# vnminin/phylomap

Measured on NVIDIA B200. Metric: sampled branch-site histories/sec (4-state, 10k-tip tree), higher is better.
Workload: dtype f32

## Files before the change

phylomap_b200/csrc/pm_host.cu:

```cuda
#include <cuda_runtime.h>

#include <algorithm>
#include <chrono>
#include <cmath>
#include <cstdarg>
#include <cstdio>
#include <cstdlib>
#include <cstring>
#include <map>
#include <memory>
#include <mutex>
#include <string>
#include <type_traits>
#include <vector>

#include "../../include/phylomap_b200.h"
#include "pm_launch.cuh"
#include "pm_setup_kernels.cuh"
#include "pm_loglik.cuh"
#include "pm_exp.cuh"
#include "pm_nccl.hpp"
#include "pm_rates.hpp"
#include "pm_tree.hpp"

// ... 316 lines not shown
  p.gx = (S + 127) / 128;
  long long ny = (148LL * 16 * 6 + p.gx - 1) / p.gx;
  ny = std::max(1LL, std::min<long long>(ny, (E + 15) / 16));
  ny = std::min<long long>(ny, 65535);
  ny = std::max<long long>(ny, (E + 2047) / 2048);
  ny = std::max<long long>(ny, (E + ((1LL << 32) - 1) / S - 1) / std::max<long long>(1, ((1LL << 32) - 1) / S));
  const double G = (double)(1 << rec_shift);
  for (;;) {
    p.chunk = (int)((E + ny - 1) / ny);
    ny = (E + p.chunk - 1) / p.chunk;
    long long cap_max = 0;
    p.cap_off.assign(ny + 1, 0);
    for (long long c = 0; c < ny; c++) {
      const int b0 = (int)c * p.chunk, b1 = std::min(E, b0 + p.chunk);
      double len = 0;
      long long init_records = 0;
      for (int e = b0; e < b1; e++) {
        len += (double)elen[e];
        const long long m0 = moff[e + 1] - moff[e];
        if (exact || m0 >= 2) init_records += m0;
      }
      long long cap;
      if (no_paths) cap = 4;
      else if (path_capacity > 0) cap = (long long)path_capacity * (b1 - b0) * (long long)G;
      else if (exact) {
        const int jumps = poisson_cap(1.5 * Omega * len + 1.0, 1e-18);
        cap = std::max<long long>((long long)(b1 - b0) + jumps, init_records);
      } else {
        std::vector<double> lams;
        long long init3 = 0;
        for (int e = b0; e < b1; e++) {
          lams.push_back(1.5 * Omega * (double)elen[e]);
          const long long m0 = moff[e + 1] - moff[e];
          if (m0 >= 3) init3 += m0;
        }
        double lam_sum = 0, lam_max = 0;
        for (double l : lams) { lam_sum += l; lam_max = std::max(lam_max, l); }
        const long long simple = (long long)poisson_cap(G * lam_sum, 1e-18) + 2LL * (b1 - b0) * (long long)G;
        long long stat = simple;
        if (lam_max < 200.0) stat = std::min(stat, chernoff_records_cap(lams, 1e-18, G));
        cap = std::max<long long>(stat, init3 * (long long)G) + 4;
      }
      if (cap > (1 << 28)) { if (rec_shift) cap = 1 << 28; else fail(PM_ERR_CAPACITY, "path capacity of a branch chunk too large"); }
      cap = (cap + 3) & ~3;
      cap_max = std::max(cap_max, cap);
      p.cap_off[c + 1] = p.cap_off[c] + (int)cap;
    }
    if (exact || no_paths || cap_max <= 65535) break;
    if (rec_shift) { p.fits = false; break; }
    if (p.chunk <= 1 || ny >= 65535) fail(PM_ERR_CAPACITY, "a branch needs more than 65 535 path records per site");
    ny = std::min<long long>(std::min<long long>(2 * ny, E), 65535);
  }
  p.ny = ny;
  return p;
}

struct CladeCode {
  pm::host::CladeSchedule cs;
  std::vector<int> e16, top;
  std::vector<int> d16;
  std::vector<long long> tips;
};
CladeCode encode_clade_schedule(const pm::host::Schedule& sch, long long S, long long TS, long long rowPL, bool redraw_tips) {
  const int T = sch.T;
  CladeCode c;
  pm::host::CladeSchedule& cs = c.cs;
  const int clade_max = (T - 1 < 512) ? std::max(8, (T - 1) / 8) : std::max(8, std::min(512, (T - 1) / 64));
  pm::host::build_clade_schedule(sch, 8, clade_max, cs);
  const int n1 = cs.warp_off.back();
  c.e16.assign((size_t)PM_CLADE_ENTRY_INTS * (n1 + 17), 0);
  auto put64 = [](int* dst, long long v) { dst[0] = (int)(unsigned)(v & 0xffffffffLL); dst[1] = (int)(v >> 32); };
  for (int i = 0; i < n1; i++) {
    const int* en = &cs.entries[(size_t)8 * i];
    int* o = &c.e16[(size_t)PM_CLADE_ENTRY_INTS * i];
    const int pn = en[0], a = en[1], ea = en[2], b = en[3], eb = en[4];
    int fl = en[5] & 3;
    const int x = (en[5] & 4) ? a : (en[5] & 8) ? b : -1;
    if (a < T) fl |= 16;
    if (b < T) fl |= 32;
    put64(o + 0, (long long)(pn - T) * rowPL);
    put64(o + 2, x >= 0 ? (long long)(x - T) * rowPL : -1LL);
    put64(o + 4, (long long)ea * S * 4);
    put64(o + 6, (long long)eb * S * 4);
    put64(o + 8, a < T ? (long long)a * TS : -1LL);
    put64(o + 10, b < T ? (long long)b * TS : -1LL);
    o[12] = fl;
  }
  c.top.assign(cs.entries.begin() + (size_t)8 * n1, cs.entries.end());
  for (int& v : cs.top_off) v -= n1;
  const int n2 = cs.down_warp_off.back();
  c.d16.assign((size_t)16 * (n2 + 17), 0);
  for (int i = 0; i < n2; i++) {
    const int* en = &cs.down_seq[(size_t)4 * i];
    int* o = &c.d16[(size_t)16 * i];
    put64(o + 0, (long long)(en[0] - T) * rowPL);
    put64(o + 2, (long long)en[2] * S * 4);
    put64(o + 4, (long long)en[0] * S);
    put64(o + 6, en[3] ? -1LL : (long long)en[1] * S);
  }
  if (redraw_tips)
    for (int v = 0; v < T; v++) {
      const int e = sch.parent_edge[v];
      c.tips.push_back((long long)sch.e_parent[e] * S); c.tips.push_back((long long)e * S * 4);
    }
  return c;
}

struct SmallOrder {
  std::vector<int> down;
  std::vector<int> border;
};
template <typename Real>
SmallOrder small_draw_order(const pm::host::Schedule& sch, const pm::host::CladeSchedule& cs, const std::vector<Real>& elen) {
  const int T = sch.T, E = (int)elen.size();
  SmallOrder so;
  std::vector<uint32_t> key(2 * (size_t)T - 1, 0u);
  for (int i = 0; i < (int)cs.down_top.size() / 4; i++) key[cs.down_top[(size_t)4 * i]] = 0x80000000u | (uint32_t)i;
  for (int i = 0; i < cs.down_warp_off.back(); i++) key[cs.down_seq[(size_t)4 * i]] = (uint32_t)i;
  for (int v = 0; v < T; v++) key[v] = 0x40000000u | (uint32_t)v;
  const int nd = (int)sch.down_entries.size() / 3;
  so.down.assign((size_t)4 * std::max(nd, 1), 0);
  for (int i = 0; i < nd; i++) {
    const int* en = &sch.down_entries[(size_t)3 * i];
    so.down[(size_t)4 * i] = en[0]; so.down[(size_t)4 * i + 1] = en[1]; so.down[(size_t)4 * i + 2] = en[2]; so.down[(size_t)4 * i + 3] = (int)key[en[0]];
  }
  std::vector<int> sorted(E);
  for (int e = 0; e < E; e++) sorted[e] = e;
  std::stable_sort(sorted.begin(), sorted.end(), [&](int x, int y) { return elen[x] > elen[y]; });
  if (E <= 256) {
    so.border.assign(256, -1);
    for (int k = 0; k < E; k++) so.border[(size_t)(k % 8) * 32 + k / 8] = sorted[k];
  } else so.border = sorted;
  return so;
}

struct WorkItems {
  std::vector<long long> off;
  std::vector<int> g;
  std::vector<int> hint;
};
template <typename Real>
WorkItems build_work_items(const std::vector<Real>& elen, double Omega, long long S) {
  const int E = (int)elen.size();
  const long long Wl = (S + 31) / 32;
  WorkItems w;
  w.off.assign(E + 1, 0);
  w.g.resize(E);
  for (int e = 0; e < E; e++) {
    const double lam = Omega * (double)elen[e];
    const double h = std::max(1e-6, 1.0 - std::exp(-lam) * (1.0 + lam));
    long long g = (long long)std::ceil(96.0 / (32.0 * h));
    g = std::max(1LL, std::min<long long>(std::min<long long>(g, 32), Wl));
    w.g[e] = (int)g;
    w.off[e + 1] = w.off[e] + (Wl + g - 1) / g;
  }
  w.hint.resize((size_t)(w.off[E] >> 6) + 1);
  for (long long i = 0, e = 0; i < (long long)w.hint.size(); i++) {
    while (e + 1 < E && w.off[e + 1] <= (i << 6)) e++;
    w.hint[i] = (int)e;
  }
  return w;
}

template <typename Real>
struct TreeDev {
  pm::host::Schedule sch;
  long long S = 0, TS = 0;
  DevBuf cl_entries, cl_warp_off, cl_top_entries, cl_top_off, cd_top, cd_top_off, cd_entries, cd_warp_off, cd_tips;
  DevBuf up_entries, up_off, down_entries, down_off, e_parent, e_child, e_len, maps_off, maps_len, cap_off;
  DevBuf tipcode, node_state, meta, PL, rec_len[2], rec_st[2], dw_partial, hard_ballot, wk_off, wk_g, wk_hint, wk_item, rec_cursor, shape;
  long long wk_total = 0, dw_rows = 0;
  int hard_blocks = 0;
  int pl_slots = 0;
  int slots_per_sm = 0;
  DevBuf slot_busy;
  long long pl_sites = 0;
  int rec_shift = 0;
  bool small_ok = false;
  bool small_two = false;
  int small_chunks = 0;
  DevBuf small_down, small_part, small_cnt, small_root, small_prof, small_border;
  DevBuf tip_stage;
  int small_cap = 0;
  int small_order_n = 0;
  long long rec_groups = 0;
  DevBuf e_len_d, TP, ll_partial;
  std::vector<int> cap_off_h;
  pm::ChainParams<Real> P;
  dim3 paths_grid;
  int chunk = 0;
  long long nblocks = 0;
};

template <typename Real>
struct ChainT : pm_chain {
  Variant V;
  int n = 0, ntrees = 0, N_total = 0, iters_done = 0, W = 0, WR = 0, ncols = 0;
  pm::host::NcclApi::Comm nccl = nullptr;
  int NS = 0;
  bool exact = false;
  double* Q = nullptr;
  double* B = nullptr;
  std::vector<double> pid, prior;
  double Omega = 0;
  pm_options opt;
  cudaStream_t stream = nullptr;
  bool own_stream = false;
  std::vector<std::unique_ptr<TreeDev<Real>>> trees;
  int jcap = 0;
  DevBuf model, cnt, root_out, err_flag, rows, tab_off, tab_u, q_dev;
  double* q_h = nullptr;
  std::vector<double> own_B;
  std::vector<double> eig_L, eig_R, eig_d;
  DevBuf eig_dev;
  Real* model_h = nullptr;
  double* rows_h = nullptr;
  double* rows_h_dev = nullptr;
  unsigned* err_h = nullptr;
  std::vector<double> scale_prev, rate_prev;
  pm::host::MersenneR mt{0};
  std::unique_ptr<pm::host::ReplaySource> replay;
  size_t smem_prune = 0, smem_nodes = 0, smem_paths = 0;
  int rows_cap = 0;
  int debug_kernel = 0;
  struct Timed { cudaEvent_t a, b; int k; };
  std::vector<Timed> timed;
  DevBuf ctl, phase_ns;
  uint32_t* ctl_h = nullptr;
  cudaGraphExec_t sweep_graph = nullptr;
  void* graph_rows = nullptr;
  bool capturing = false;
  int launches_per_sweep = 0;
  Switches sw;

  ~ChainT() override {
    cudaSetDevice(opt.device);
    cudaDeviceSynchronize();
    for (auto& t : timed) { cudaEventDestroy(t.a); cudaEventDestroy(t.b); }
    if (model_h) cudaFreeHost(model_h);
    if (rows_h) cudaFreeHost(rows_h);
    if (err_h) cudaFreeHost(err_h);
    if (q_h) cudaFreeHost(q_h);
    if (ctl_h) cudaFreeHost(ctl_h);
    for (auto& t : trees) if (t && t->small_prof.p) {
      long long h[12];
      if (cudaMemcpy(h, t->small_prof.p, sizeof h, cudaMemcpyDeviceToHost) == cudaSuccess)
        fprintf(stderr, "[phylomap_b200] k_small_chain block 0 (%d + %d levels), cycles over %d sweeps: prune %lld, node draws %lld, paths %lld, row %lld; paths per warp:"
                        " %lld %lld %lld %lld %lld %lld %lld %lld\n", (int)t->sch.up_off.size() - 1, (int)t->sch.down_off.size() - 1, iters_done, h[0], h[1], h[2], h[3], h[4], h[5], h[6], h[7], h[8], h[9], h[10], h[11]);
    }
    if (sweep_graph) cudaGraphExecDestroy(sweep_graph);
    if (own_stream && stream) cudaStreamDestroy(stream);
  }

  pm::host::UniformSource& host_rng() { return replay ? static_cast<pm::host::UniformSource&>(*replay) : mt; }

  size_t model_elems() const { return (size_t)2 * n * n + 5 * n; }
  size_t model_stride() const { return (model_elems() + 3) & ~(size_t)3; }

  void stage_model(bool first) {
    std::vector<double> Bd((size_t)n * n), Bs((size_t)n * n);
    for (int i = 0; i < n; i++)
      for (int j = 0; j < n; j++) {
        const double v = B[i + (size_t)j * n];
        Bd[(size_t)i * n + j] = v;
        Bs[(size_t)i * n + j] = (V.sparse && !(v > 1e-7)) ? 0.0 : v;
      }
    std::vector<double> scale_new(n);
    for (int s = 0; s < n; s++) scale_new[s] = 1.0 / (Omega + Q[s + (size_t)s * n]);
    std::vector<double> rate_new(n);
    for (int s = 0; s < n; s++) rate_new[s] = Omega + Q[s + (size_t)s * n];
    if (first) { scale_prev = scale_new; rate_prev = rate_new; }
    Real* m = model_h;
    for (size_t i = 0; i < (size_t)n * n; i++) { m[i] = (Real)Bd[i]; m[(size_t)n * n + i] = (Real)Bs[i]; }
    Real* v = m + 2 * (size_t)n * n;
    for (int s = 0; s < n; s++) {
      v[s] = (Real)pid[s]; v[n + s] = (Real)scale_prev[s]; v[2 * n + s] = (Real)scale_new[s];
      v[3 * n + s] = (Real)rate_prev[s]; v[4 * n + s] = (Real)rate_new[s];
    }
    scale_prev = scale_new; rate_prev = rate_new;
    Real* pw = m + model_stride();
    std::vector<double> cur((size_t)n * n, 0.0), nxt((size_t)n * n);
    for (int i = 0; i < n; i++) cur[(size_t)i * n + i] = 1.0;
    for (int j = 0; j < jcap; j++) {
      for (size_t i = 0; i < (size_t)n * n; i++) pw[(size_t)j * n * n + i] = (Real)cur[i];
      if (j + 1 < jcap) {
        for (int r = 0; r < n; r++)
          for (int c = 0; c < n; c++) {
            double acc = 0;
            for (int l = 0; l < n; l++) acc = acc + Bs[(size_t)r * n + l] * cur[(size_t)l * n + c];
            nxt[(size_t)r * n + c] = acc;
          }
        cur.swap(nxt);
      }
    }
    CK(cudaMemcpyAsync(model.p, m, (model_stride() + (size_t)jcap * n * n) * sizeof(Real), cudaMemcpyHostToDevice, stream));
  }

  template <typename F>
  auto with_ns(F&& f) const {
    if (NS == 2) return f(std::integral_constant<int, 2>{});
    if (NS == 4) return f(std::integral_constant<int, 4>{});
    return f(std::integral_constant<int, 0>{});
  }
  template <typename F>
  auto with_ns_exact(F&& f) const {
    if constexpr (std::is_same_v<Real, double>)
      if (exact) return with_ns([&](auto ns) { return f(ns, std::true_type{}); });
    return with_ns([&](auto ns) { return f(ns, std::false_type{}); });
  }

  template <int NSc, bool EX>
  void launch_sweep_t(TreeDev<Real>& t, uint32_t iter, double* row) {
    if (!EX && use_small(t)) { launch_small(t, iter, 1, row); launches_per_sweep = t.S == 1 ? 1 : 2; return; }
    const uint32_t* ctl_d = capturing ? ctl.as<uint32_t>() : nullptr;
    {
      pm::ChainParams<Real> P = t.P;
      P.ctl = ctl_d;
      const int gx = (int)((t.S + 31) / 32);
      if (t.pl_slots) {
        begin_timed(4);
        pm::Sweep<Real, NSc, EX>::prune_nodes(P, gx, smem_nodes, stream, iter, 0, 3, t.slots_per_sm ? t.slot_busy.template as<int>() : nullptr,
                                              t.slots_per_sm, timing ? phase_ns.as<unsigned long long>() : nullptr);
        end_timed();
      } else {
        begin_timed(0);
        pm::Sweep<Real, NSc, EX>::prune(P, gx, smem_prune, stream);
        end_timed();
        begin_timed(1);
        pm::Sweep<Real, NSc, EX>::nodes(P, gx, smem_nodes, stream, iter);
        end_timed();
      }
    }
    begin_timed(2);
    if (!EX) CK(cudaMemsetAsync(t.rec_cursor.p, 0, t.rec_cursor.bytes, stream));
    {
      pm::ChainParams<Real> P = t.P;
      P.ctl = ctl_d;
      pm::Sweep<Real, NSc, EX>::paths(P, t.paths_grid, smem_paths, stream, iter, (iter == 0 && !capturing) ? 1 : 0, t.chunk, t.hard_blocks);
    }
    end_timed();
    begin_timed(3);
    pm::k_reduce<<<1, 256, 0, stream>>>(t.dw_partial.template as<double>(), t.dw_rows, n, cnt.as<unsigned long long>(),
                                        root_out.as<int>(), row, 0, err_flag.as<unsigned>(), W, capturing ? ctl.as<uint32_t>() : nullptr, WR);
    end_timed();
    launches_per_sweep = (t.pl_slots ? 1 : 2) + (exact ? 2 : (iter == 0 && !capturing) ? 3 : 4);
    if (!capturing) launches += launches_per_sweep;
  }
  bool use_small(const TreeDev<Real>& t) const { return t.small_ok && !timing && !sw.debug_sync && !capturing; }
  void launch_small(TreeDev<Real>& t, uint32_t iter0, int nsweeps, double* rows_d) {
    const long long S = t.S;
    pm::SmallOut o;
    o.down = reinterpret_cast<const int4*>(t.small_down.p); o.down_off = t.down_off.template as<int>();
    o.n_down_levels = (int)t.sch.down_off.size() - 1; o.n_chunks = t.small_chunks;
    o.br_order = t.small_border.template as<int>(); o.n_order = t.small_order_n;
    o.part = nullptr; o.cnt = nullptr; o.root = nullptr; o.rows = nullptr; o.row_stride = WR; o.err_slot = W;
    o.prof = nullptr;
    if (sw.small_prof) {
      if (!t.small_prof.p) { t.small_prof.alloc(12 * sizeof(long long)); CK(cudaMemsetAsync(t.small_prof.p, 0, t.small_prof.bytes, stream)); }
      o.prof = t.small_prof.template as<long long>();
    }
    auto launch = [&](uint32_t it0, int nb) {
      with_ns([&](auto ns) { pm::Sweep<Real, decltype(ns)::value, false>::small_chain(t.P, (int)S, stream, it0, nb, o, t.small_two); });
    };
    if (S == 1) {
      o.rows = rows_d;
      launch(iter0, nsweeps);
      launches += 1;
      return;
    }
    const int batch = (int)std::max<long long>(1, std::min<long long>(nsweeps, (64LL << 20) / (S * n * (long long)sizeof(double))));
    if (t.small_cap < batch) {
      t.small_part.alloc((size_t)batch * S * n * sizeof(double));
      t.small_cnt.alloc((size_t)batch * n * n * sizeof(unsigned long long));
      t.small_root.alloc((size_t)batch * sizeof(int));
      t.small_cap = batch;
      CK(cudaMemsetAsync(t.small_cnt.p, 0, t.small_cnt.bytes, stream));
      CK(cudaMemsetAsync(t.small_root.p, 0, t.small_root.bytes, stream));
    }
    o.part = t.small_part.template as<double>(); o.cnt = t.small_cnt.template as<unsigned long long>(); o.root = t.small_root.template as<int>();
    for (int b0 = 0; b0 < nsweeps; b0 += batch) {
      const int nb = std::min(batch, nsweeps - b0);
      launch(iter0 + (uint32_t)b0, nb);
      pm::k_small_reduce<<<nb, 128, 0, stream>>>(o.part, o.cnt, o.root, S, n, rows_d + (size_t)b0 * WR, WR, err_flag.as<unsigned>(), W);
      launches += 2;
    }
  }
  void launch_loglik(TreeDev<Real>& t, double* row) {
    for (int i = 0; i < n; i++) for (int j = 0; j < n; j++) q_h[(size_t)i * n + j] = Q[i + (size_t)j * n];
    CK(cudaMemcpyAsync(q_dev.p, q_h, (size_t)n * n * sizeof(double), cudaMemcpyHostToDevice, stream));
    const int E = t.sch.E;
    pm::k_transprob<Real><<<(E + 127) / 128, 128, 0, stream>>>(q_dev.as<double>(), t.e_len_d.template as<double>(), E, n,
                                                              t.TP.template as<Real>());
    const int gx = (int)((t.S + 31) / 32);
    with_ns([&](auto ns) {
      pm::k_loglik<Real, decltype(ns)::value><<<gx, 256, 0, stream>>>(t.P, t.TP.template as<Real>(), t.ll_partial.template as<double>());
    });
    pm::k_reduce_ll<<<1, 256, 0, stream>>>(t.ll_partial.template as<double>(), gx, row + n + n * n + 1);
    launches += 3;
  }

  template <int NSc, bool EX>
  void launch_prune_t(TreeDev<Real>& t, long long only_site) {
    const long long nb = (t.S + 31) / 32;
    if (t.pl_slots) {
      if (only_site >= 0) pm::Sweep<Real, NSc, EX>::prune_nodes(t.P, 1, smem_nodes, stream, 0u, only_site / 32, 1, nullptr, 0, nullptr);
      else pm::Sweep<Real, NSc, EX>::prune_nodes(t.P, (int)nb, smem_nodes, stream, 0u, 0, 1, t.slots_per_sm ? t.slot_busy.template as<int>() : nullptr,
                                                 t.slots_per_sm, nullptr);
    } else pm::Sweep<Real, NSc, EX>::prune(t.P, (int)nb, smem_prune, stream);
    launches++;
  }

  void launch_sweep(TreeDev<Real>& t, uint32_t iter, double* row) {
    with_ns_exact([&](auto ns, auto ex) { launch_sweep_t<decltype(ns)::value, decltype(ex)::value>(t, iter, row); });
  }
  void launch_prune(TreeDev<Real>& t, long long only_site = -1) {
    with_ns_exact([&](auto ns, auto ex) { launch_prune_t<decltype(ns)::value, decltype(ex)::value>(t, only_site); });
  }

  void begin_timed(int k) {
    debug_kernel = k;
    if (!timing) return;
    Timed t; t.k = k;
    CK(cudaEventCreate(&t.a)); CK(cudaEventCreate(&t.b));
    CK(cudaEventRecord(t.a, stream));
    timed.push_back(t);
  }
  void end_timed() {
    if (timing) CK(cudaEventRecord(timed.back().b, stream));
    if (sw.debug_sync) {
      try { check_device_errors(); }
      catch (Fail& f) { f.msg += " [raised by sweep kernel #" + std::to_string(debug_kernel) + ": 0 prune, 1 nodes, 2 paths, 3 reduce]"; throw; }
    }
  }
  void collect_timed() {
    double fused = 0;
    for (auto& t : timed) {
      float ms = 0;
      cudaEventElapsedTime(&ms, t.a, t.b);
      if (t.k == 4) fused += ms; else kernel_ms[t.k] += ms;
      cudaEventDestroy(t.a); cudaEventDestroy(t.b);
    }
    timed.clear();
    if (fused > 0) {
      unsigned long long ns[2] = {0, 0};
      cudaMemcpy(ns, phase_ns.p, sizeof ns, cudaMemcpyDeviceToHost);
      cudaMemset(phase_ns.p, 0, sizeof ns);
      const double tot = (double)ns[0] + (double)ns[1];
      const double share = tot > 0 ? (double)ns[0] / tot : 0.5;
      kernel_ms[0] += fused * share;
      kernel_ms[1] += fused * (1.0 - share);
    }
  }

  void check_device_errors() {
    CK(cudaMemcpyAsync(err_h, err_flag.p, sizeof(unsigned), cudaMemcpyDeviceToHost, stream));
    CK(cudaStreamSynchronize(stream));
    const unsigned f = *err_h;
    if (!f) return;
    if (f & PM_DE_BAD_STATE) fail(PM_ERR_ARG, "tip states must lie in 1..n");
    if (f & PM_DE_SAMPLE_NA) fail(PM_ERR_SAMPLE, "NAs not allowed in probability");
    if (f & PM_DE_SAMPLE_NEG) fail(PM_ERR_SAMPLE, "Negative probabilities not allowed");
    if (f & PM_DE_SAMPLE_ZERO)
      fail(PM_ERR_SAMPLE, opt.precision == PM_F32 ? "Not enough positive probabilities (FP32 partial likelihoods span ~1e-45: on large trees with "
                                                      "one-piece branches this can be an underflow; precision f64 has the reference's range)"
                                                    : "Not enough positive probabilities");
    if (f & PM_DE_REPLAY) fail(PM_ERR_REPLAY, "replay table exhausted");
    if (f & PM_DE_JUMP_LIMIT)
      fail(PM_ERR_CAPACITY, "a branch carries more than 63 state changes at one site: the deterministic mode holds at most 64 runs "
                            "per path (the production arithmetic has no such limit)");
    if (f & PM_DE_PATH_CAP) fail(PM_ERR_CAPACITY, "the run records of a branch chunk overflowed; raise pm_options.path_capacity");
    if (f & PM_DE_M_OVERFLOW) fail(PM_ERR_CAPACITY, "more than 65535 pieces on one branch");
    fail(PM_ERR_CUDA, "inconsistent chain state (device flag %u)", f);
  }

  void create(int variant, const pm_tree* tr, int ntr, int n_, double* Q_, const double* pid_, double* B_, double Om,
              const double* prior_, int nprior, int Ntot, const pm_options* o) {
    V = variant_of(variant);
    n = n_; ntrees = ntr; N_total = Ntot; Q = Q_; B = B_; Omega = Om;
    opt = *o;
    sw = read_switches();
    PhaseTrace trace{sw.trace};
    std::vector<pm::host::Schedule> schedules = validate(variant, tr, pid_, prior_, nprior);
    trace.mark("validation + schedules");
    const int sms = open_device();
    trace.mark("device queries + stream");
    err_flag.alloc(sizeof(unsigned));
    CK(cudaMemsetAsync(err_flag.p, 0, err_flag.bytes, stream));
    cudaStream_t aux = nullptr;
    cudaEvent_t ev_a = nullptr, ev_b = nullptr;
    struct AuxGuard {
      cudaStream_t& s; cudaEvent_t& a; cudaEvent_t& b;
      ~AuxGuard() { if (s) { cudaStreamSynchronize(s); cudaStreamDestroy(s); } if (a) cudaEventDestroy(a); if (b) cudaEventDestroy(b); }
    } aux_guard{aux, ev_a, ev_b};
    CK(cudaStreamCreateWithFlags(&aux, cudaStreamNonBlocking));
    CK(cudaEventCreateWithFlags(&ev_a, cudaEventDisableTiming));
    CK(cudaEventCreateWithFlags(&ev_b, cudaEventDisableTiming));
    CK(cudaEventRecord(ev_a, stream));
    CK(cudaStreamWaitEvent(aux, ev_a, 0));
    double tmax = 0;
    for (int ti = 0; ti < ntr; ti++) trees.push_back(create_tree(tr[ti], ti, std::move(schedules[ti]), sms, aux, tmax, trace));

    alloc_model_and_host_buffers(tmax);
    if (opt.rng == PM_RNG_TABLE) upload_replay_table();
    mt.reseed((uint32_t)opt.seed);
    trace.mark("pinned buffers, replay table");
    const int np_fast = exact ? 0 : ((NS == 2 || NS == 4) ? std::min(PM_SMEM_POW, jcap) : 0);
    smem_prune = ((size_t)n * n + (size_t)np_fast * n * n) * sizeof(Real);
    smem_nodes = ((size_t)n * n + 3 * n + (size_t)np_fast * n * n) * sizeof(Real);
    smem_paths = (size_t)4 * n * sizeof(double) + ((size_t)n * n + ((n * n) & 1)) * sizeof(unsigned) +
                 ((size_t)2 * n * n + 5 * n + (size_t)np_fast * n * n) * sizeof(Real);

    for (int ti = 0; ti < ntr; ti++) {
      TreeDev<Real>& t = *trees[ti];
      fill_params(t, ti);
      const pm::ChainParams<Real>& P = t.P;
      if (!V.exp && !V.llonly)
        pm::k_init_meta<Real><<<dim3((unsigned)((t.S + 255) / 256), (unsigned)std::min(P.E, 65535)), 256, 0, stream>>>(P.maps_off, P.maps_len, t.S, P.E, P.meta,
                                                                                                                         P.e_len, exact ? nullptr : P.shape);
      trace.mark("set-up kernels issued");
      CK(cudaGetLastError());
    }
    CK(cudaEventRecord(ev_b, aux));
    CK(cudaStreamWaitEvent(stream, ev_b, 0));
    stage_model(true);
    if (V.exp) {
      std::vector<double> eg;
      eg.insert(eg.end(), eig_L.begin(), eig_L.end());
      eg.insert(eg.end(), eig_R.begin(), eig_R.end());
      eg.insert(eg.end(), eig_d.begin(), eig_d.end());
      upload(eig_dev, eg, stream);
      TreeDev<Real>& t = *trees[0];
      const int E = t.sch.E;
      const double* g = eig_dev.as<double>();
      pm::k_transprob_eig<Real><<<(E + 127) / 128, 128, 0, stream>>>(g, g + (size_t)n * n, g + (size_t)2 * n * n,
                                                                    t.e_len_d.template as<double>(), E, n, t.TP.template as<Real>());
      CK(cudaGetLastError());
    }
    check_device_errors();
    for (auto& t : trees) t->tip_stage.alloc(0);
    trace.mark("tip states: H2D + transpose, init kernels, sync");
  }

  std::vector<pm::host::Schedule> validate(int variant, const pm_tree* tr, const double* pid_, const double* prior_, int nprior) {
    const int ntr = ntrees;
    if (n < 2 || n > PM_NMAX) fail(PM_ERR_ARG, "number of states must be in 2..%d", PM_NMAX);
    if (!V.multi && ntr != 1) fail(PM_ERR_ARG, "this sampler takes exactly one tree");
    if (ntr < 1) fail(PM_ERR_ARG, "no trees");
    if (N_total < 0) fail(PM_ERR_ARG, "N must be non-negative");
    if (V.hidden && (n < 4 || (n & 1))) fail(PM_ERR_ARG, "hidden-rate samplers need an even number of states >= 4");
    if (V.two_state && n != 2) fail(PM_ERR_ARG, "this sampler is 2-state only");
    if (V.dic && n > PM_DIC_NMAX) fail(PM_ERR_ARG, "the DIC samplers support at most %d states", PM_DIC_NMAX);
    const int need_prior = V.two_state ? 4 : variant == PM_V_KSMT ? 8 : V.hidden ? 6 : 0;
    if (nprior < need_prior || (need_prior && !prior_)) fail(PM_ERR_ARG, "prior needs %d values", need_prior);
    if (need_prior) prior.assign(prior_, prior_ + nprior);
    pid.assign(pid_, pid_ + n);
    exact = opt.mode == PM_MODE_DETERMINISTIC;
    if (exact && opt.precision != PM_F64) fail(PM_ERR_ARG, "deterministic mode computes in FP64");
    if (exact && V.exp) fail(PM_ERR_ARG, "the direct sampler (maketreelistEXP) runs in production arithmetic only");
    if (opt.rng == PM_RNG_TABLE && (!opt.tab_off || !opt.tab_u)) fail(PM_ERR_ARG, "replay table missing");
    if (opt.rng == PM_RNG_TABLE && !exact) fail(PM_ERR_ARG, "the replay table feeds the deterministic mode only");
    if (opt.rng == PM_RNG_TABLE && (opt.site_offset != 0 || opt.allreduce || opt.nccl_world > 1)) fail(PM_ERR_ARG, "replay runs are single-process");
    if (opt.allreduce && !opt.cuda_stream)
      fail(PM_ERR_ARG, "an allreduce callback needs pm_options.cuda_stream: the collective must be ordered on the stream the chain launches on");
    if (opt.allreduce && opt.nccl_world > 1) fail(PM_ERR_ARG, "give either an allreduce callback or an NCCL clique, not both");
    if (opt.nccl_world > 1 && (!opt.nccl_id || opt.nccl_rank < 0 || opt.nccl_rank >= opt.nccl_world)) fail(PM_ERR_ARG, "bad NCCL clique (nccl_id / nccl_rank / nccl_world)");
    NS = (n == 2) ? 2 : (n == 4) ? 4 : 0;
    W = n + n * n + 1 + (V.dic ? 1 : 0);
    WR = W + 1;
    ncols = ncols_of(variant, n);

    if (!(Omega > 0)) fail(PM_ERR_ARG, "Omega must be positive");
    std::vector<pm::host::Schedule> schedules(ntr);
    for (int ti = 0; ti < ntr; ti++) {
      const pm_tree& x = tr[ti];
      if (x.n_tips != tr[0].n_tips || x.n_edges != tr[0].n_edges) fail(PM_ERR_ARG, "all trees must have the same number of tips");
      if (x.n_sites < 1 || x.n_sites != tr[0].n_sites) fail(PM_ERR_ARG, "n_sites must be >= 1 and equal across trees");
      if (x.n_sites >= (1LL << 31)) fail(PM_ERR_ARG, "at most 2^31 - 1 sites per process");
      if (!x.edge || !x.nen || !x.nodelist || !x.maps_off || !x.maps_len) fail(PM_ERR_ARG, "tree %d: missing field", ti);
      if (!x.states && !x.states_u8) fail(PM_ERR_ARG, "tree %d: states missing", ti);
      try {
        pm::host::build_schedule(x.n_tips, x.n_edges, x.edge, x.nen, x.nodelist, x.root, V.redraw_tips, schedules[ti]);
      } catch (const std::string& msg) { fail(PM_ERR_ARG, "tree %d: %s", ti, msg.c_str()); }
      if (x.maps_off[0] != 0) fail(PM_ERR_ARG, "tree %d: maps_off[0] must be 0", ti);
      for (int e = 0; e < x.n_edges; e++) {
        const long long a = x.maps_off[e], b = x.maps_off[e + 1];
        if (b <= a) fail(PM_ERR_ARG, "tree %d: branch %d has no segments", ti, e + 1);
        if (b - a > 65535) fail(PM_ERR_ARG, "tree %d: branch %d has more than 65535 segments", ti, e + 1);
        for (long long p = a; p < b; p++) {
          if (!(x.maps_len[p] >= 0)) fail(PM_ERR_ARG, "tree %d: negative or NA segment length", ti);
          if (x.maps_state && (x.maps_state[p] < 1 || x.maps_state[p] > n)) fail(PM_ERR_ARG, "tree %d: mapnames out of range", ti);
        }
      }
    }
    return schedules;
  }

  int open_device() {
    int ndev = 0;
    if (cudaGetDeviceCount(&ndev) != cudaSuccess || ndev <= 0) fail(PM_ERR_CUDA, "no CUDA device (there is no CPU fallback)");
    if (opt.device < 0 || opt.device >= ndev) fail(PM_ERR_CUDA, "device %d not present", opt.device);
    CK(cudaSetDevice(opt.device));
    int major = 0, minor = 0, sms = 0;
    CK(cudaDeviceGetAttribute(&major, cudaDevAttrComputeCapabilityMajor, opt.device));
    CK(cudaDeviceGetAttribute(&minor, cudaDevAttrComputeCapabilityMinor, opt.device));
    CK(cudaDeviceGetAttribute(&sms, cudaDevAttrMultiProcessorCount, opt.device));
    if (major != 10) fail(PM_ERR_CUDA, "device %d is sm_%d%d; this library is built for sm_100a only", opt.device, major, minor);
    if (opt.cuda_stream) stream = (cudaStream_t)opt.cuda_stream;
    else { CK(cudaStreamCreateWithFlags(&stream, cudaStreamNonBlocking)); own_stream = true; }
    return sms;
  }

  std::unique_ptr<TreeDev<Real>> create_tree(const pm_tree& x, int ti, pm::host::Schedule&& sch, int sms, cudaStream_t aux,
                                             double& tmax, PhaseTrace& trace) {
    std::unique_ptr<TreeDev<Real>> tp(new TreeDev<Real>());
    TreeDev<Real>& t = *tp;
    t.sch = std::move(sch);
    t.S = x.n_sites;
    t.TS = (t.S + 15) / 16 * 16;
    const int E = x.n_edges, T = x.n_tips;
    const long long S = t.S;
    const bool no_paths = V.exp || V.llonly;
    upload_tips(t, x, aux);
    std::vector<long long> moff(x.maps_off, x.maps_off + E + 1);
    std::vector<Real> elen(E);
    for (int e = 0; e < E; e++) {
      double tot = 0;
      for (long long p = moff[e]; p < moff[e + 1]; p++) tot = tot + x.maps_len[p];
      elen[e] = (Real)tot;
      tmax = std::max(tmax, tot);
    }
    std::vector<double> mlen(x.maps_len, x.maps_len + moff[E]);

    const size_t small_smem = with_ns([&](auto ns) { return pm::Sweep<Real, decltype(ns)::value, false>::small_smem(T); });
    const SmallChoice small = choose_small_kernel(!exact && (NS == 2 || NS == 4) && !no_paths && opt.rng != PM_RNG_TABLE, elen,
                                                  Omega, T, S, sms, small_smem, sw);
    t.small_ok = small.ok;
    t.small_two = small.two;
    const bool pooled_ok = !t.small_ok && !exact && !no_paths && sw.rec_pool;
    RecordPlan rp = plan_records(pooled_ok ? 5 : 0, elen, moff, S, Omega, exact, no_paths, opt.path_capacity);
    if (!rp.fits) rp = plan_records(0, elen, moff, S, Omega, exact, no_paths, opt.path_capacity);
    t.rec_shift = rp.rec_shift;
    t.rec_groups = (S + (1LL << t.rec_shift) - 1) >> t.rec_shift;
    t.chunk = rp.chunk;
    t.paths_grid = dim3((unsigned)rp.gx, (unsigned)rp.ny, 1);
    t.nblocks = rp.gx * rp.ny;
    t.small_chunks = (int)rp.ny;
    t.cap_off_h = std::move(rp.cap_off);
    trace.mark("record capacities");

    plan_partials_slots(t, sms);
    upload(t.up_entries, t.sch.up_entries, stream);
    upload(t.up_off, t.sch.up_off, stream);
    if (!exact && (NS == 2 || NS == 4)) {
      CladeCode cc = encode_clade_schedule(t.sch, S, t.TS, (long long)t.pl_sites * n * (long long)sizeof(Real), V.redraw_tips);
      upload(t.cl_entries, cc.e16, stream);
      upload(t.cl_warp_off, cc.cs.warp_off, stream);
      upload(t.cl_top_entries, cc.top, stream);
      upload(t.cl_top_off, cc.cs.top_off, stream);
      upload(t.cd_entries, cc.d16, stream);
      upload(t.cd_warp_off, cc.cs.down_warp_off, stream);
      upload(t.cd_top, cc.cs.down_top, stream);
      upload(t.cd_top_off, cc.cs.down_top_off, stream);
      upload(t.cd_tips, cc.tips, stream);
      t.P.n_cl_top_levels = (int)cc.cs.top_off.size() - 1;
      t.P.n_cd_top_levels = (int)cc.cs.down_top_off.size() - 1;
      t.P.n_cd_tips = (int)cc.tips.size() / 2;
      if (t.small_ok) {
        const SmallOrder so = small_draw_order(t.sch, cc.cs, elen);
        upload(t.small_down, so.down, stream);
        upload(t.small_border, so.border, stream);
        t.small_order_n = (int)so.border.size();
      }
    }
    upload(t.down_entries, t.sch.down_entries, stream);
    upload(t.down_off, t.sch.down_off, stream);
    upload(t.e_parent, t.sch.e_parent, stream);
    upload(t.e_child, t.sch.e_child, stream);
    upload(t.e_len, elen, stream);
    if (V.dic || V.exp) {
      std::vector<double> eld(E);
      for (int e = 0; e < E; e++) eld[e] = x.edge_length ? x.edge_length[e] : (double)elen[e];
      if (x.edge_length) for (int e = 0; e < E; e++) if (!(eld[e] >= 0)) fail(PM_ERR_ARG, "tree %d: negative or NA edge.length", ti);
      upload(t.e_len_d, eld, stream);
      t.TP.alloc((size_t)E * n * n * sizeof(Real));
      t.ll_partial.alloc((size_t)((S + 31) / 32) * sizeof(double));
    }
    trace.mark("clade schedules + uploads");
    alloc_path_state(t, moff, mlen, elen, sms);
    trace.mark("device buffers");
    return tp;
  }

  void upload_tips(TreeDev<Real>& t, const pm_tree& x, cudaStream_t aux) {
    const int T = x.n_tips;
    t.tipcode.alloc((size_t)T * t.TS);
    CK(cudaMemsetAsync(t.tipcode.p, 0, t.tipcode.bytes, aux));
    t.node_state.alloc((size_t)(2 * T - 1) * t.S);
    CK(cudaMemsetAsync(t.node_state.p, 0, t.node_state.bytes, aux));
    const size_t esz = x.states_u8 ? 1 : 4;
    long long rows_per = std::max<long long>(32, (256LL << 20) / ((long long)T * (long long)esz));
    rows_per = std::min<long long>(rows_per, std::min<long long>(t.S, 32LL * 65535));
    t.tip_stage.alloc((size_t)rows_per * T * esz);
    for (long long s0 = 0; s0 < t.S; s0 += rows_per) {
      const int ns = (int)std::min<long long>(rows_per, t.S - s0);
      const void* src = x.states_u8 ? (const void*)(x.states_u8 + s0 * T) : (const void*)(x.states + s0 * T);
      CK(cudaMemcpyAsync(t.tip_stage.p, src, (size_t)ns * T * esz, cudaMemcpyHostToDevice, aux));
      dim3 g((T + 31) / 32, (ns + 31) / 32), b(32, 8);
      if (x.states_u8)
        pm::k_init_tips<uint8_t><<<g, b, 0, aux>>>(t.tip_stage.template as<uint8_t>(), ns, s0, t.S, t.TS, T, n, V.parity_tips,
                                                     t.tipcode.template as<uint8_t>(), t.node_state.template as<uint8_t>(), err_flag.as<unsigned>());
      else
        pm::k_init_tips<int32_t><<<g, b, 0, aux>>>(t.tip_stage.template as<int32_t>(), ns, s0, t.S, t.TS, T, n, V.parity_tips,
                                                     t.tipcode.template as<uint8_t>(), t.node_state.template as<uint8_t>(), err_flag.as<unsigned>());
    }
    CK(cudaGetLastError());
  }

  void plan_partials_slots(TreeDev<Real>& t, int sms) {
    t.pl_slots = 0;
    t.pl_sites = t.S;
    if (exact || !(NS == 2 || NS == 4) || V.dic || V.exp || V.llonly || !sw.fused) return;
    const size_t smem_lo = ((size_t)n * n + 3 * n) * sizeof(Real);
    const int per_sm = with_ns([&](auto ns) { return pm::Sweep<Real, decltype(ns)::value, false>::fused_blocks_per_sm(smem_lo); });
    if (per_sm < 1) fail(PM_ERR_CUDA, "cudaOccupancyMaxActiveBlocksPerMultiprocessor failed for the fused prune + node-draw kernel");
    t.slots_per_sm = per_sm;
    t.pl_slots = sm_id_range(opt.device, sms) * per_sm;
    t.pl_sites = 32LL * t.pl_slots;
    if (t.pl_sites >= ((t.S + 31) / 32) * 32) {
      t.pl_slots = (int)((t.S + 31) / 32); t.pl_sites = 32LL * t.pl_slots; t.slots_per_sm = 0;
    } else {
      t.slot_busy.alloc((size_t)t.pl_slots * sizeof(int));
      CK(cudaMemsetAsync(t.slot_busy.p, 0, t.slot_busy.bytes, stream));
    }
  }

  void alloc_path_state(TreeDev<Real>& t, const std::vector<long long>& moff, const std::vector<double>& mlen,
                        const std::vector<Real>& elen, int sms) {
    const int E = t.sch.E, T = t.sch.T;
    const long long S = t.S, R = t.cap_off_h.back();
    const bool no_paths = V.exp || V.llonly;
    upload(t.maps_off, moff, stream);
    upload(t.maps_len, mlen, stream);
    upload(t.cap_off, t.cap_off_h, stream);
    if (!no_paths) t.meta.alloc((size_t)E * S * sizeof(uint32_t));
    t.PL.alloc((size_t)(T - 1) * t.pl_sites * n * sizeof(Real));
    for (int b = 0; b < 2 && !no_paths; b++) {
      t.rec_len[b].alloc((size_t)R * t.rec_groups * sizeof(Real));
      t.rec_st[b].alloc((size_t)R * t.rec_groups);
    }
    if (!exact && !no_paths) {
      const long long Wl = (S + 31) / 32;
      t.hard_ballot.alloc((size_t)E * Wl * sizeof(uint32_t));
      const WorkItems w = build_work_items(elen, Omega, S);
      t.wk_total = w.off.back();
      upload(t.wk_hint, w.hint, stream);
      upload(t.wk_off, w.off, stream);
      upload(t.wk_g, w.g, stream);
      t.wk_item.alloc((size_t)std::max<long long>(t.wk_total, 1) * sizeof(unsigned long long));
      pm::k_build_items<<<(unsigned)((t.wk_total + 255) / 256), 256, 0, stream>>>(t.wk_off.template as<long long>(), t.wk_g.template as<int>(), E, Wl,
                                                                                 t.wk_total, t.wk_item.template as<unsigned long long>());
      t.rec_cursor.alloc((size_t)t.small_chunks * t.rec_groups * sizeof(int));
      t.shape.alloc((size_t)E * S * sizeof(uint16_t));
      t.hard_blocks = (int)std::max<long long>(1, std::min<long long>(sms * 4LL, (t.wk_total + 3) / 4));
    }
    t.dw_rows = t.nblocks + 3 * t.hard_blocks;
    t.dw_partial.alloc((size_t)t.dw_rows * n * sizeof(double));
    CK(cudaMemsetAsync(t.dw_partial.p, 0, t.dw_partial.bytes, stream));
    dev_bytes += t.tipcode.bytes + t.node_state.bytes + t.meta.bytes + t.PL.bytes + 2 * (t.rec_len[0].bytes + t.rec_st[0].bytes) +
                 t.dw_partial.bytes + t.hard_ballot.bytes + t.rec_cursor.bytes + t.shape.bytes + t.wk_item.bytes;
  }

  void alloc_model_and_host_buffers(double tmax) {
    jcap = opt.power_capacity > 0 ? opt.power_capacity : 64;
    if (V.exp) jcap = 302;
    else if (opt.power_capacity <= 0) {
      const double lam = Omega * tmax;
      const double want = lam + 10 * std::sqrt(lam) + 24;
      jcap = (int)std::min(16384.0, std::max(64.0, want));
    }
    if (jcap < 2) jcap = 2;
    model.alloc((model_stride() + (size_t)jcap * n * n) * sizeof(Real));
    CK(cudaMallocHost((void**)&model_h, (model_stride() + (size_t)jcap * n * n) * sizeof(Real)));
    memset(model_h, 0, (model_stride() + (size_t)jcap * n * n) * sizeof(Real));
    CK(cudaMallocHost((void**)&rows_h, (size_t)ntrees * WR * sizeof(double)));
    if (cudaHostGetDevicePointer((void**)&rows_h_dev, rows_h, 0) != cudaSuccess) { rows_h_dev = nullptr; (void)cudaGetLastError(); }
    if (opt.nccl_world > 1) nccl = clique(opt.nccl_id, opt.nccl_world, opt.nccl_rank);
    CK(cudaMallocHost((void**)&err_h, sizeof(unsigned)));
    CK(cudaMallocHost((void**)&ctl_h, 2 * sizeof(uint32_t)));
    ctl.alloc(2 * sizeof(uint32_t));
    phase_ns.alloc(2 * sizeof(unsigned long long));
    CK(cudaMemsetAsync(phase_ns.p, 0, phase_ns.bytes, stream));
    if (V.dic) { CK(cudaMallocHost((void**)&q_h, (size_t)n * n * sizeof(double))); q_dev.alloc((size_t)n * n * sizeof(double)); }
    cnt.alloc((size_t)n * n * sizeof(unsigned long long));
    root_out.alloc(sizeof(int));
    CK(cudaMemsetAsync(cnt.p, 0, cnt.bytes, stream));
    CK(cudaMemsetAsync(root_out.p, 0, root_out.bytes, stream));
  }

  int replay_slots_per_iter() const { return (2 * trees[0]->sch.T - 1) + 2 * trees[0]->sch.E; }
  void upload_replay_table() {
    const long long nslots = (long long)ntrees * trees[0]->S * N_total * replay_slots_per_iter();
    std::vector<long long> off(nslots + 1);
    for (long long i = 0; i <= nslots; i++) off[i] = opt.tab_off[i];
    std::vector<double> u(opt.tab_u, opt.tab_u + off[nslots]);
    upload(tab_off, off, stream);
    upload(tab_u, u, stream);
    if (opt.host_tab) replay.reset(new pm::host::ReplaySource(opt.host_tab, opt.host_tab_n));
  }

  void fill_params(TreeDev<Real>& t, int ti) {
    pm::ChainParams<Real>& P = t.P;
    const int T = t.sch.T, E = t.sch.E, spi = replay_slots_per_iter();
    P.n = n; P.T = T; P.E = E; P.S = t.S;
    P.cap_off = t.cap_off.template as<int>();
    P.hard_ballot = t.hard_ballot.template as<uint32_t>(); P.W = (int)((t.S + 31) / 32);
    P.wk_off = t.wk_off.template as<long long>(); P.wk_g = t.wk_g.template as<int>(); P.wk_total = t.wk_total;
    P.wk_hint = t.wk_hint.template as<int>(); P.wk_item = t.wk_item.template as<unsigned long long>();
    P.rec_cursor = t.rec_cursor.template as<int>(); P.chunk = t.chunk; P.easy_blocks = t.nblocks;
    P.shape = t.shape.template as<uint16_t>();
    P.model = model.as<Real>(); P.ppow = model.as<Real>() + model_stride(); P.jcap = jcap;
    P.up_entries = t.up_entries.template as<int>(); P.up_off = t.up_off.template as<int>();
    P.n_up_levels = (int)t.sch.up_off.size() - 1;
    P.cl_entries = t.cl_entries.template as<int>(); P.cl_warp_off = t.cl_warp_off.template as<int>();
    P.cl_top_entries = t.cl_top_entries.template as<int>(); P.cl_top_off = t.cl_top_off.template as<int>();
    P.cd_top = t.cd_top.template as<int>(); P.cd_top_off = t.cd_top_off.template as<int>();
    P.cd_entries = t.cd_entries.template as<int>(); P.cd_warp_off = t.cd_warp_off.template as<int>();
    P.cd_tips = t.cd_tips.template as<long long>();
    P.down_entries = t.down_entries.template as<int>(); P.down_off = t.down_off.template as<int>();
    P.n_down_levels = (int)t.sch.down_off.size() - 1;
    P.e_parent = t.e_parent.template as<int>(); P.e_child = t.e_child.template as<int>();
    P.e_len = t.e_len.template as<Real>();
    P.maps_off = t.maps_off.template as<long long>(); P.maps_len = t.maps_len.template as<double>();
    P.root = t.sch.root;
    P.tipcode = t.tipcode.template as<uint8_t>(); P.TS = t.TS; P.node_state = t.node_state.template as<uint8_t>();
    P.meta = t.meta.template as<uint32_t>(); P.PL = t.PL.template as<Real>();
    P.tile_base = 0; P.pl_S = t.pl_sites; P.rec_shift = t.rec_shift; P.rec_groups = t.rec_groups; P.ctl = nullptr;
    for (int b = 0; b < 2; b++) { P.rec_len[b] = t.rec_len[b].template as<Real>(); P.rec_st[b] = t.rec_st[b].template as<uint8_t>(); }
    P.normalize = V.normalize || !exact; P.full_counts = V.full_counts; P.parity_tips = V.parity_tips;
    P.dw_partial = t.dw_partial.template as<double>(); P.cnt = cnt.as<unsigned long long>();
    P.root_out = root_out.as<int>(); P.err_flag = err_flag.as<unsigned>();
    const uint64_t key = opt.seed + (uint64_t)ti * 0x9E3779B97F4A7C15ull;
    P.rng.k0 = (uint32_t)key; P.rng.k1 = (uint32_t)(key >> 32);
    for (int r = 0; r < 10; r++) { P.rng.rk[2 * r] = P.rng.k0 + (uint32_t)r * 0x9E3779B9u; P.rng.rk[2 * r + 1] = P.rng.k1 + (uint32_t)r * 0xBB67AE85u; }
    P.rng.site0 = (uint32_t)opt.site_offset;
    P.rng.tab_off = opt.rng == PM_RNG_TABLE ? (const int64_t*)tab_off.p : nullptr;
    P.rng.tab_u = opt.rng == PM_RNG_TABLE ? tab_u.as<double>() : nullptr;
    P.rng.tab_site_stride = (int64_t)N_total * spi;
    P.rng.tab_base = (int64_t)ti * t.S * N_total * spi;
    P.rng.slots_per_iter = spi; P.rng.n_nodes = 2 * T - 1;
  }

  void reduce_over_ranks(double* buf, int count) {
    if (nccl) {
      auto& api = pm::host::NcclApi::get();
      const int rc = api.AllReduce(buf, buf, (size_t)count, pm::host::NcclApi::kDouble, pm::host::NcclApi::kSum, nccl, stream);
      if (rc != 0) fail(PM_ERR_CUDA, "ncclAllReduce failed: %s", api.error(rc).c_str());
    } else if (opt.allreduce) {
      if (opt.allreduce(opt.allreduce_ctx, buf, count) != 0) fail(PM_ERR_CUDA, "allreduce callback failed");
    }
  }
  void check_row_errors(const double* rows_host, int nrows) {
    bool any = false;
    for (int i = 0; i < nrows; i++) any = any || rows_host[(size_t)i * WR + W] != 0.0;
    if (!any) return;
    check_device_errors();
    fail(PM_ERR_CUDA, "another rank reported a device error in this sweep; all ranks stop together");
  }

  void ensure_rows(int count) {
    const int need = std::max(count, 1) * ntrees;
    if (need <= rows_cap) return;
    rows.alloc((size_t)need * WR * sizeof(double));
    rows_cap = need;
  }

  void write_fixed_row(const double* r, double* out, int64_t ld, int i) {
    for (int s = 0; s < n; s++) out[i + (int64_t)s * ld] = r[s];
    for (int a = 0; a < n; a++)
      for (int b = 0; b < n; b++) {
        if (a == b) continue;
        const int col = n + a * (n - 1) + b - (a < b ? 1 : 0);
        out[i + (int64_t)col * ld] = r[n + a * n + b];
      }
  }

  void launch_exp_iteration(TreeDev<Real>& t, uint32_t iter, double* row) {
    const int gx = (int)((t.S + 31) / 32);
    Real* TP = t.TP.template as<Real>();
    double* llp = t.ll_partial.template as<double>();
    const size_t smem_b = (size_t)4 * n * sizeof(double) + ((size_t)n * n + ((n * n) & 1)) * sizeof(unsigned) + (size_t)n * n * sizeof(Real);
    const double* el = t.e_len_d.template as<double>();
    with_ns([&](auto ns) {
      constexpr int NSc = decltype(ns)::value;
      begin_timed(0);
      pm::k_loglik<Real, NSc><<<gx, 256, 0, stream>>>(t.P, TP, llp);
      end_timed();
      begin_timed(1);
      pm::k_exp_nodes<Real, NSc><<<gx, 256, 0, stream>>>(t.P, TP, iter);
      end_timed();
      begin_timed(2);
      pm::k_exp_branches<Real, NSc><<<t.paths_grid, 128, smem_b, stream>>>(t.P, TP, el, (Real)Omega, iter, t.chunk);
      end_timed();
    });
    begin_timed(3);
    pm::k_reduce<<<1, 256, 0, stream>>>(t.dw_partial.template as<double>(), t.dw_rows, n, cnt.as<unsigned long long>(),
                                        root_out.as<int>(), row, 0, err_flag.as<unsigned>(), W);
    end_timed();
    launches += 4;
  }

  void run(int count, double* out, int64_t ld) override {
    if (count < 0 || iters_done + count > N_total) fail(PM_ERR_ARG, "cannot run %d more iterations (%d of %d done)", count, iters_done, N_total);
    if (count == 0) return;
    if (ld < count) fail(PM_ERR_ARG, "leading dimension smaller than the number of rows");
    CK(cudaSetDevice(opt.device));
    if (!V.rates) {
      ensure_rows(count);
      TreeDev<Real>& t = *trees[0];
      const bool small = (double)t.S * t.sch.E <= (double)(1 << 22);
      const bool one_launch = !V.exp && !exact && use_small(t);
      const bool use_graph = !one_launch && !V.exp && !timing && !sw.debug_sync && count > 1 && (sw.graph == 1 || (sw.graph != 0 && small));
      if (one_launch) launch_small(t, (uint32_t)iters_done, count, rows.as<double>());
      for (int i = 0; i < count && !one_launch; i++) {
        if (V.exp) launch_exp_iteration(t, (uint32_t)(iters_done + i), rows.as<double>() + (size_t)i * WR);
        else if (use_graph && i > 0) {
          if (i == 1) {
            if (sweep_graph && graph_rows != rows.p) { cudaGraphExecDestroy(sweep_graph); sweep_graph = nullptr; }
            if (!sweep_graph) {
              cudaGraph_t g = nullptr;
              CK(cudaStreamBeginCapture(stream, cudaStreamCaptureModeRelaxed));
              capturing = true;
              try { launch_sweep(t, 1u, rows.as<double>()); } catch (...) { capturing = false; cudaStreamEndCapture(stream, &g); if (g) cudaGraphDestroy(g); throw; }
              capturing = false;
              CK(cudaStreamEndCapture(stream, &g));
              const cudaError_t ge = cudaGraphInstantiate(&sweep_graph, g, 0);
              cudaGraphDestroy(g);
              if (ge != cudaSuccess) fail(PM_ERR_CUDA, "cudaGraphInstantiate failed: %s", cudaGetErrorString(ge));
              graph_rows = rows.p;
            }
            ctl_h[0] = (uint32_t)(iters_done + 1); ctl_h[1] = 1u;
            CK(cudaMemcpyAsync(ctl.p, ctl_h, 2 * sizeof(uint32_t), cudaMemcpyHostToDevice, stream));
          }
          CK(cudaGraphLaunch(sweep_graph, stream));
          launches += launches_per_sweep;
        }
        else launch_sweep(t, (uint32_t)(iters_done + i), rows.as<double>() + (size_t)i * WR);
        if (opt.progress) { printf("%i \r", iters_done + i); }
      }
      CK(cudaGetLastError());
      reduce_over_ranks(rows.as<double>(), count * WR);
      std::vector<double> h((size_t)count * WR);
      CK(cudaMemcpyAsync(h.data(), rows.p, h.size() * sizeof(double), cudaMemcpyDeviceToHost, stream));
      CK(cudaStreamSynchronize(stream));
      check_row_errors(h.data(), count);
      collect_timed();
      for (int i = 0; i < count; i++) write_fixed_row(&h[(size_t)i * WR], out, ld, i);
      iters_done += count;
      return;
    }

    ensure_rows(1);
    pm::host::RateModel rm{n, Q, B, Omega, prior.data()};
    const size_t nparam = V.hidden ? (size_t)2 + 3 * (n / 2 - 1) : 2;
    if (rate_proposed.size() != nparam) { rate_proposed.assign(nparam, 0); rate_accepted.assign(nparam, 0); }
    rm.proposed = rate_proposed.data(); rm.accepted = rate_accepted.data();
    pm::host::UniformSource& g = host_rng();
    std::vector<double> row(ncols);
    std::vector<std::vector<double>> jodt(ntrees, std::vector<double>(ncols, 0.0));
    for (int i = 0; i < count; i++) {
      const int it = iters_done;
      if (V.multi && it == 0) (void)g.next();
      bool host_rows = rows_h_dev != nullptr && !nccl && !opt.allreduce && !V.dic;
      for (int j = 0; j < ntrees; j++) host_rows = host_rows && use_small(*trees[j]);
      double* const row0 = host_rows ? rows_h_dev : rows.as<double>();
      for (int j = 0; j < ntrees; j++) launch_sweep(*trees[j], (uint32_t)it, row0 + (size_t)j * WR);
      if (V.dic) launch_loglik(*trees[0], rows.as<double>());
      CK(cudaGetLastError());
      cudaEvent_t ca = nullptr, cb = nullptr;
      if (timing) { CK(cudaEventCreate(&ca)); CK(cudaEventCreate(&cb)); CK(cudaEventRecord(ca, stream)); }
      reduce_over_ranks(rows.as<double>(), ntrees * WR);
      if (timing) CK(cudaEventRecord(cb, stream));
      if (!host_rows) CK(cudaMemcpyAsync(rows_h, rows.p, (size_t)ntrees * WR * sizeof(double), cudaMemcpyDeviceToHost, stream));
      CK(cudaStreamSynchronize(stream));
      if (timing) { float ms = 0; cudaEventElapsedTime(&ms, ca, cb); comm_ms += ms; cudaEventDestroy(ca); cudaEventDestroy(cb); }
      const auto host_t0 = std::chrono::steady_clock::now();
      check_row_errors(rows_h, ntrees);
      for (int j = 0; j < ntrees; j++) {
        std::fill(jodt[j].begin(), jodt[j].end(), 0.0);
        const double* r = rows_h + (size_t)j * WR;
        for (int c = 0; c < n + n * n; c++) jodt[j][c] = r[c];
        if (V.hidden) rm.record_hidden(jodt[j].data()); else rm.record_two_state(jodt[j].data());
        if (V.dic) { jodt[j][ncols - 2] = r[n + n * n]; jodt[j][ncols - 1] = r[n + n * n + 1]; }
        else jodt[j][ncols - 1] = r[n + n * n];
      }
      int pick = 0;
      if (V.multi) {
        const double u = g.next();
        double cum = 0;
        for (pick = 0; pick < ntrees; pick++) { cum += 1.0 / ntrees; if (u < cum) break; }
        if (pick >= ntrees) pick = ntrees - 1;
        jodt[pick][ncols - 1] = pick;
      }
      const double* st = jodt[pick].data();
      for (int c = 0; c < ncols; c++) out[i + (int64_t)c * ld] = st[c];
      if (V.hidden) rm.hidden_rates(st, g, V.multi); else rm.two_state(st, g, V.multi);
      if (g.exhausted()) fail(PM_ERR_REPLAY, "host replay table exhausted");
      iters_done++;
      stage_model(false);
      if (timing) host_update_ms += std::chrono::duration<double, std::milli>(std::chrono::steady_clock::now() - host_t0).count();
      if (opt.progress) { printf("%i \r", it); }
    }
    CK(cudaStreamSynchronize(stream));
    collect_timed();
  }

  float time_prune(int tree, int reps) override {
    if (tree < 0 || tree >= ntrees || reps < 1) fail(PM_ERR_ARG, "bad arguments");
    CK(cudaSetDevice(opt.device));
    cudaEvent_t a, b;
    CK(cudaEventCreate(&a)); CK(cudaEventCreate(&b));
    launch_prune(*trees[tree]);
    CK(cudaEventRecord(a, stream));
    for (int r = 0; r < reps; r++) launch_prune(*trees[tree]);
    CK(cudaEventRecord(b, stream));
    CK(cudaEventSynchronize(b));
    float ms = 0;
    CK(cudaEventElapsedTime(&ms, a, b));
    cudaEventDestroy(a); cudaEventDestroy(b);
    CK(cudaGetLastError());
    return ms / reps;
  }

  void node_states(int tree, int32_t* out) override {
    TreeDev<Real>& t = *trees.at(tree);
    const int NN = 2 * t.sch.T - 1;
    std::vector<uint8_t> h((size_t)NN * t.S);
    CK(cudaMemcpy(h.data(), t.node_state.p, h.size(), cudaMemcpyDeviceToHost));
    for (long long s = 0; s < t.S; s++) for (int v = 0; v < NN; v++) out[s * NN + v] = h[(size_t)v * t.S + s];
  }
  void piece_counts(int tree, int32_t* out) override {
    TreeDev<Real>& t = *trees.at(tree);
    const int E = t.sch.E;
    std::vector<uint32_t> h((size_t)E * t.S);
    CK(cudaMemcpy(h.data(), t.meta.p, h.size() * 4, cudaMemcpyDeviceToHost));
    for (long long s = 0; s < t.S; s++) for (int e = 0; e < E; e++) out[s * E + e] = (int)(h[(size_t)e * t.S + s] & 0xffffu);
  }
  int path(int tree, int64_t site, int e, double* len, int32_t* st, int cap) override {
    TreeDev<Real>& t = *trees.at(tree);
    if (site < 0 || site >= t.S || e < 0 || e >= t.sch.E) fail(PM_ERR_ARG, "bad site / branch");
    uint32_t m = 0;
    CK(cudaMemcpy(&m, t.meta.template as<uint32_t>() + (size_t)e * t.S + site, 4, cudaMemcpyDeviceToHost));
    if (iters_done == 0) fail(PM_ERR_ARG, "no sweep done yet");
    const int c = e / t.chunk, b0 = c * t.chunk;
    const int cap_c = t.cap_off_h[c + 1] - t.cap_off_h[c];
    const int buf = (iters_done - 1) & 1;
    auto records = [&](long long pos, int count) {
      const size_t base = (size_t)t.cap_off_h[c] * t.rec_groups + (size_t)(site >> t.rec_shift) * cap_c + pos;
      for (int k = 0; k < count && k < cap; k++) {
        Real L; uint8_t s;
        CK(cudaMemcpy(&L, t.rec_len[buf].template as<Real>() + base + k, sizeof(Real), cudaMemcpyDeviceToHost));
        CK(cudaMemcpy(&s, t.rec_st[buf].template as<uint8_t>() + base + k, 1, cudaMemcpyDeviceToHost));
        len[k] = (double)L; st[k] = s;
      }
    };
    if (exact) {
      const int nj = (m >> 16) & 0xff;
      long long pos = 0;
      for (int e2 = b0; e2 < e; e2++) {
        uint32_t m2 = 0;
        CK(cudaMemcpy(&m2, t.meta.template as<uint32_t>() + (size_t)e2 * t.S + site, 4, cudaMemcpyDeviceToHost));
        pos += ((m2 >> 16) & 0xff) + 1;
      }
      records(pos, nj + 1);
      return nj + 1;
    }
    uint16_t shp = 0;
    CK(cudaMemcpy(&shp, t.shape.template as<uint16_t>() + (size_t)e * t.S + site, 2, cudaMemcpyDeviceToHost));
    int nj = shp & 0x3f;
    const int s0 = (shp >> 6) & 0x1f, s1 = (shp >> 11) & 0x1f;
    const uint32_t q = m >> 16;
    Real Le;
    CK(cudaMemcpy(&Le, t.e_len.template as<Real>() + e, sizeof(Real), cudaMemcpyDeviceToHost));
    if (nj == 0) {
      if (cap > 0) { len[0] = (double)Le; st[0] = s0; }
      return 1;
    }
    if (nj == 1) {
      const Real p1 = (Real)q * (Le * (Real)(1.0 / 65536.0));
      if (cap > 0) { len[0] = (double)p1; st[0] = s0; }
      if (cap > 1) { len[1] = (double)(Le - p1); st[1] = s1; }
      return 2;
    }
    long long pos = (long long)q;
    if (nj == 63) {
      Real cntv;
      CK(cudaMemcpy(&cntv, t.rec_len[buf].template as<Real>() + (size_t)t.cap_off_h[c] * t.rec_groups + (size_t)(site >> t.rec_shift) * cap_c + pos, sizeof(Real),
                    cudaMemcpyDeviceToHost));
      nj = (int)cntv - 1;
      pos += 1;
    }
    records(pos, nj + 1);
    return nj + 1;
  }
  static constexpr uint32_t PM_STATE_FORMAT = 6;
  struct StateHeader {
    char magic[8];
    int32_t variant, n, ntrees, precision, mode, T, E, iters_done, jcap, reserved;
    int64_t S, site_offset, total_bytes;
    uint64_t seed;
  };
  std::vector<DevBuf*> state_buffers() {
    std::vector<DevBuf*> v{&model};
    for (auto& t : trees) {
      v.push_back(&t->node_state); v.push_back(&t->meta); v.push_back(&t->shape);
      for (int b = 0; b < 2; b++) { v.push_back(&t->rec_len[b]); v.push_back(&t->rec_st[b]); }
    }
    return v;
  }
  size_t host_state_bytes() const { return sizeof(StateHeader) + 625 * sizeof(uint32_t) + ((size_t)2 * n * n + 2 * n) * sizeof(double); }
  int64_t state_bytes() override {
    size_t tot = host_state_bytes();
    for (DevBuf* b : state_buffers()) tot += (b->bytes + 15) & ~(size_t)15;
    return (int64_t)tot;
  }
  StateHeader make_header() {
    StateHeader h;
    memset(&h, 0, sizeof h);
    memcpy(h.magic, "PMB200S", 8);
    h.variant = V.id; h.n = n; h.ntrees = ntrees; h.precision = opt.precision; h.mode = opt.mode;
    h.T = trees[0]->sch.T; h.E = trees[0]->sch.E; h.iters_done = iters_done; h.jcap = jcap;
    h.S = trees[0]->S; h.site_offset = opt.site_offset; h.total_bytes = state_bytes(); h.seed = opt.seed;
    uint32_t hsh = 2166136261u;
    auto mix = [&](uint32_t v) { hsh = (hsh ^ v) * 16777619u; };
    mix(PM_STATE_FORMAT); mix(PM_META(1, 2)); mix((uint32_t)PM_SHAPE(1, 2, 3)); mix(PM_LAMBDA_INV); mix(PM_LOCAL_PATH_MAX); mix(PM_SMEM_POW);
    for (auto& t : trees) { mix((uint32_t)t->chunk); mix((uint32_t)t->rec_shift); for (int c : t->cap_off_h) mix((uint32_t)c); }
    h.reserved = (int32_t)((PM_STATE_FORMAT << 24) | (hsh & 0xffffffu));
    return h;
  }
  void export_state(void* buf, int64_t bytes) override {
    if (opt.rng == PM_RNG_TABLE) fail(PM_ERR_ARG, "replay-table runs cannot be checkpointed");
    if (!buf || bytes < state_bytes()) fail(PM_ERR_ARG, "state buffer too small (%lld bytes needed)", (long long)state_bytes());
    CK(cudaSetDevice(opt.device));
    CK(cudaStreamSynchronize(stream));
    unsigned char* p = (unsigned char*)buf;
    const StateHeader h = make_header();
    memcpy(p, &h, sizeof h); p += sizeof h;
    uint32_t w[625]; mt.save(w);
    memcpy(p, w, sizeof w); p += sizeof w;
    memcpy(p, Q, (size_t)n * n * sizeof(double)); p += (size_t)n * n * sizeof(double);
    memcpy(p, B, (size_t)n * n * sizeof(double)); p += (size_t)n * n * sizeof(double);
    memcpy(p, scale_prev.data(), n * sizeof(double)); p += n * sizeof(double);
    memcpy(p, rate_prev.data(), n * sizeof(double)); p += n * sizeof(double);
    for (DevBuf* b : state_buffers()) {
      if (b->bytes) CK(cudaMemcpyAsync(p, b->p, b->bytes, cudaMemcpyDeviceToHost, stream));
      p += (b->bytes + 15) & ~(size_t)15;
    }
    CK(cudaStreamSynchronize(stream));
  }
  void import_state(const void* buf, int64_t bytes) override {
    if (opt.rng == PM_RNG_TABLE) fail(PM_ERR_ARG, "replay-table runs cannot be checkpointed");
    if (!buf || bytes < (int64_t)sizeof(StateHeader)) fail(PM_ERR_ARG, "not a chain state");
    const unsigned char* p = (const unsigned char*)buf;
    StateHeader h; memcpy(&h, p, sizeof h); p += sizeof h;
    const StateHeader me = make_header();
    if (memcmp(h.magic, me.magic, 8) != 0) fail(PM_ERR_ARG, "not a chain state");
    if (h.variant != me.variant || h.n != me.n || h.ntrees != me.ntrees || h.precision != me.precision || h.mode != me.mode ||
        h.T != me.T || h.E != me.E || h.S != me.S || h.site_offset != me.site_offset || h.jcap != me.jcap || h.seed != me.seed ||
        h.total_bytes != me.total_bytes)
      fail(PM_ERR_ARG, "the state was exported by a chain of a different shape, sampler, precision, seed or site block");
    if (h.reserved != me.reserved)
      fail(PM_ERR_ARG, "the state was exported under another state format or buffer layout (format %d here, %d in the blob)",
           (int)PM_STATE_FORMAT, (int)((uint32_t)h.reserved >> 24));
    if (bytes < h.total_bytes) fail(PM_ERR_ARG, "truncated chain state");
    if (h.iters_done < 0 || h.iters_done > N_total) fail(PM_ERR_ARG, "the state has %d iterations done, this chain was created for %d", h.iters_done, N_total);
    CK(cudaSetDevice(opt.device));
    CK(cudaStreamSynchronize(stream));
    uint32_t w[625]; memcpy(w, p, sizeof w); p += sizeof w;
    if (w[624] > 624u) fail(PM_ERR_ARG, "corrupt chain state");
    mt.load(w);
    memcpy(Q, p, (size_t)n * n * sizeof(double)); p += (size_t)n * n * sizeof(double);
    memcpy(B, p, (size_t)n * n * sizeof(double)); p += (size_t)n * n * sizeof(double);
    memcpy(scale_prev.data(), p, n * sizeof(double)); p += n * sizeof(double);
    memcpy(rate_prev.data(), p, n * sizeof(double)); p += n * sizeof(double);
    for (DevBuf* b : state_buffers()) {
      if (b->bytes) CK(cudaMemcpyAsync(b->p, p, b->bytes, cudaMemcpyHostToDevice, stream));
      p += (b->bytes + 15) & ~(size_t)15;
    }
    CK(cudaStreamSynchronize(stream));
    iters_done = h.iters_done;
  }

  double loglik() override {
    if (!V.dic) fail(PM_ERR_ARG, "this chain was not created with a log-likelihood column");
    CK(cudaSetDevice(opt.device));
    ensure_rows(1);
    double* row = rows.as<double>();
    launch_loglik(*trees[0], row);
    CK(cudaGetLastError());
    double* cell = row + n + n * n + 1;
    reduce_over_ranks(cell, 1);
    CK(cudaMemcpyAsync(rows_h, cell, sizeof(double), cudaMemcpyDeviceToHost, stream));
    check_device_errors();
    return rows_h[0];
  }
  void partials(int tree, int64_t site, double* out) override {
    TreeDev<Real>& t = *trees.at(tree);
    const int T = t.sch.T;
    if (site < 0 || site >= t.S) fail(PM_ERR_ARG, "bad site");
    CK(cudaSetDevice(opt.device));
    launch_prune(t, site);
    CK(cudaStreamSynchronize(stream));
    const long long col = t.pl_slots ? site % 32 : site;
    std::fill(out, out + (size_t)(2 * T - 1) * n, 0.0);
    std::vector<Real> v(n);
    for (int i = 0; i < T - 1; i++) {
      CK(cudaMemcpy(v.data(), t.PL.template as<Real>() + ((size_t)i * t.pl_sites + col) * n, n * sizeof(Real), cudaMemcpyDeviceToHost));
      for (int j = 0; j < n; j++) out[(size_t)(T + i) * n + j] = (double)v[j];
    }
  }
};

struct EigenIn { const double* lefts; const double* rights; const double* d; };

template <typename Real>
void prepare_exp(ChainT<Real>& c, int n, const double* Q, const EigenIn& eg, double*& B, double& Omega) {
  double mn = Q[0];
  for (int i = 1; i < n; i++) mn = std::min(mn, Q[i + (size_t)i * n]);
  Omega = -mn;
  c.own_B.assign((size_t)n * n, 0.0);
  for (int i = 0; i < n; i++) for (int j = 0; j < n; j++) c.own_B[i + (size_t)j * n] = (i == j ? 1.0 : 0.0) + Q[i + (size_t)j * n] / Omega;
  B = c.own_B.data();
  c.eig_L.resize((size_t)n * n); c.eig_R.resize((size_t)n * n); c.eig_d.resize(n);
  for (int i = 0; i < n; i++) {
    c.eig_d[i] = eg.d[i + (size_t)i * n];
    for (int j = 0; j < n; j++) { c.eig_L[(size_t)i * n + j] = eg.lefts[i + (size_t)j * n]; c.eig_R[(size_t)i * n + j] = eg.rights[i + (size_t)j * n]; }
  }
}

pm_chain* make_chain(int variant, const pm_tree* trees, int ntrees, int n, double* Q, const double* pid, double* B,
                     double Omega, const double* prior, int nprior, int N_total, const pm_options* opt,
                     const EigenIn* eg = nullptr, bool internal = false) {
  pm_options def;
  if (!opt) { pm_default_options(&def); opt = &def; }
  if (!trees || !Q || !pid || (!B && variant != PM_V_EXP)) fail(PM_ERR_ARG, "null argument");
  if (variant == PM_V_EXP && (!eg || !eg->lefts || !eg->rights || !eg->d)) fail(PM_ERR_ARG, "the direct sampler needs the eigendecomposition of Q");
  if (variant == PM_V_EXP && (n < 2 || n > PM_NMAX)) fail(PM_ERR_ARG, "number of states must be in 2..%d", PM_NMAX);
  if ((variant < PM_V_PLAIN || variant > PM_V_EXP) && !internal) fail(PM_ERR_ARG, "unknown variant");
  if (opt->precision == PM_F32) {
    std::unique_ptr<ChainT<float>> c(new ChainT<float>());
    if (variant == PM_V_EXP) prepare_exp(*c, n, Q, *eg, B, Omega);
    c->create(variant, trees, ntrees, n, Q, pid, B, Omega, prior, nprior, N_total, opt);
    return c.release();
  }
  std::unique_ptr<ChainT<double>> c(new ChainT<double>());
  if (variant == PM_V_EXP) prepare_exp(*c, n, Q, *eg, B, Omega);
  c->create(variant, trees, ntrees, n, Q, pid, B, Omega, prior, nprior, N_total, opt);
  return c.release();
}

void run_site_block(int variant, const pm_tree* x, int n, double* Q, const double* pid, double* B, double Omega, int N,
                    const pm_options* opt, const EigenIn* eg, long long s0, long long count, double* out) {
  pm_tree t = *x;
  t.n_sites = count;
  if (x->states_u8) t.states_u8 = x->states_u8 + s0 * (long long)x->n_tips;
  if (x->states) t.states = x->states + s0 * (long long)x->n_tips;
  pm_options o = *opt;
  o.site_offset = opt->site_offset + s0;
  std::unique_ptr<pm_chain> c(make_chain(variant, &t, 1, n, Q, pid, B, Omega, nullptr, 0, N, &o, eg));
  c->run(N, out, N);
}

int one_call(int variant, const pm_tree* trees, int ntrees, int n, double* Q, const double* pid, double* B, double Omega,
             int N, const double* prior, int nprior, const pm_options* opt, double* out, char* err, size_t errlen,
             const EigenIn* eg = nullptr) {
  return guarded(err, errlen, [&] {
    if (!out && N > 0) fail(PM_ERR_ARG, "null output");
    pm_options def;
    if (!opt) { pm_default_options(&def); opt = &def; }
    const bool fixed_q = variant == PM_V_PLAIN || variant == PM_V_SPARSE || variant == PM_V_BIGTREE || variant == PM_V_EXP;
    const bool single_process = !opt->allreduce && opt->nccl_world <= 1;
    long long tile = read_switches().site_tile;
    if (!fixed_q || !trees || ntrees != 1 || opt->rng == PM_RNG_TABLE || trees[0].n_sites < 2) tile = 0;
    const long long S = trees ? trees[0].n_sites : 0;
    for (;;) {
      const long long ts = (tile > 0 && tile < S) ? tile : S;
      try {
        if (ts >= S) {
          std::unique_ptr<pm_chain> c(make_chain(variant, trees, ntrees, n, Q, pid, B, Omega, prior, nprior, N, opt, eg));
          c->run(N, out, N);
        } else {
          const int nc = ncols_of(variant, n);
          std::vector<double> part((size_t)N * nc), acc((size_t)N * nc, 0.0);
          for (long long s0 = 0; s0 < S; s0 += ts) {
            run_site_block(variant, trees, n, Q, pid, B, Omega, N, opt, eg, s0, std::min(ts, S - s0), part.data());
            for (size_t i = 0; i < acc.size(); i++) acc[i] += part[i];
          }
          std::copy(acc.begin(), acc.end(), out);
        }
        return;
      } catch (const Fail& f) {
        const bool oom = f.code == PM_ERR_CUDA && f.msg.find("cudaMalloc") != std::string::npos;
        if (!oom || !fixed_q || !single_process || ts < 64 || ntrees != 1 || opt->rng == PM_RNG_TABLE) throw;
        cudaGetLastError();
        pool().release();
        tile = (ts + 1) / 2;
      }
    }
  });
}

}

extern "C" {

void pm_default_options(pm_options* o) {
  memset(o, 0, sizeof *o);
  o->precision = PM_F64;
  o->mode = PM_MODE_PRODUCTION;
  o->rng = PM_RNG_PHILOX;
  o->seed = 1;
}

int32_t pm_ncols(int32_t variant, int32_t n) { return ncols_of(variant, n); }

int pm_maketreelistMCMC(const pm_tree* x, int32_t n, double* Q, const double* pid, double* B, double Omega, int32_t N,
                        const pm_options* opt, double* out, char* err, size_t errlen) {
  return one_call(PM_V_PLAIN, x, 1, n, Q, pid, B, Omega, N, nullptr, 0, opt, out, err, errlen);
}
int pm_SPARSEmaketreelistMCMC(const pm_tree* x, int32_t n, double* Q, const double* pid, double* B, double Omega,
                              int32_t N, const pm_options* opt, double* out, char* err, size_t errlen) {
  return one_call(PM_V_SPARSE, x, 1, n, Q, pid, B, Omega, N, nullptr, 0, opt, out, err, errlen);
}
int pm_maketreelistMCMC_bigtree(const pm_tree* x, int32_t n, double* Q, const double* pid, double* B, double Omega,
                                int32_t N, const pm_options* opt, double* out, char* err, size_t errlen) {
  return one_call(PM_V_BIGTREE, x, 1, n, Q, pid, B, Omega, N, nullptr, 0, opt, out, err, errlen);
}
int pm_maketreelistMCMCbf(const pm_tree* x, int32_t n, double* Q, const double* pid, double* B, double Omega, int32_t N,
                          const double* prior, int32_t nprior, const pm_options* opt, double* out, char* err,
                          size_t errlen) {
  return one_call(PM_V_BF, x, 1, n, Q, pid, B, Omega, N, prior, nprior, opt, out, err, errlen);
}
int pm_maketreelistMCMCks(const pm_tree* x, int32_t n, double* Q, const double* pid, double* B, double Omega, int32_t N,
                          const double* prior, int32_t nprior, const pm_options* opt, double* out, char* err,
                          size_t errlen) {
  return one_call(PM_V_KS, x, 1, n, Q, pid, B, Omega, N, prior, nprior, opt, out, err, errlen);
}
int pm_maketreelistMCMCmt(const pm_tree* trees, int32_t ntrees, int32_t n, double* Q, const double* pid, double* B,
                          double Omega, int32_t N, const double* prior, int32_t nprior, const pm_options* opt,
                          double* out, char* err, size_t errlen) {
  return one_call(PM_V_MT, trees, ntrees, n, Q, pid, B, Omega, N, prior, nprior, opt, out, err, errlen);
}
int pm_maketreelistMCMCksmt(const pm_tree* trees, int32_t ntrees, int32_t n, double* Q, const double* pid, double* B,
                            double Omega, int32_t N, const double* prior, int32_t nprior, const pm_options* opt,
                            double* out, char* err, size_t errlen) {
  return one_call(PM_V_KSMT, trees, ntrees, n, Q, pid, B, Omega, N, prior, nprior, opt, out, err, errlen);
}

int pm_maketreelistEXP(const pm_tree* x, int32_t n, double* Q, const double* pid, int32_t N, const double* lefts,
                       const double* rights, const double* d, const pm_options* opt, double* out, char* err, size_t errlen) {
  EigenIn eg{lefts, rights, d};
  return one_call(PM_V_EXP, x, 1, n, Q, pid, nullptr, 0.0, N, nullptr, 0, opt, out, err, errlen, &eg);
}

int pm_maketreelistMCMC2sDICt(const pm_tree* x, int32_t n, double* Q, const double* pid, double* B, double Omega, int32_t N,
                              const double* prior, int32_t nprior, const pm_options* opt, double* out, char* err,
                              size_t errlen) {
  return one_call(PM_V_DIC2S, x, 1, n, Q, pid, B, Omega, N, prior, nprior, opt, out, err, errlen);
}
int pm_maketreelistMCMCksDICt(const pm_tree* x, int32_t n, double* Q, const double* pid, double* B, double Omega, int32_t N,
                              const double* prior, int32_t nprior, const pm_options* opt, double* out, char* err,
                              size_t errlen) {
  return one_call(PM_V_DICKS, x, 1, n, Q, pid, B, Omega, N, prior, nprior, opt, out, err, errlen);
}

int pm_loglik(const pm_tree* x, int32_t n, const double* Q, const double* pid, int32_t parity_tips, const pm_options* opt,
              double* out, char* err, size_t errlen) {
  return guarded(err, errlen, [&] {
    if (!x || !Q || !pid || !out) fail(PM_ERR_ARG, "null argument");
    if (n < 2 || n > PM_DIC_NMAX) fail(PM_ERR_ARG, "number of states must be in 2..%d", PM_DIC_NMAX);
    if (parity_tips && (n & 1)) fail(PM_ERR_ARG, "parity tip partials need an even number of states");
    std::vector<double> q(Q, Q + (size_t)n * n), b((size_t)n * n, 0.0);
    double om = 0;
    for (int i = 0; i < n; i++) om = std::max(om, 2 * std::fabs(q[i + (size_t)i * n]));
    if (!(om > 0)) om = 1;
    for (int i = 0; i < n; i++) for (int j = 0; j < n; j++) b[i + (size_t)j * n] = (i == j ? 1.0 : 0.0) + q[i + (size_t)j * n] / om;
    std::unique_ptr<pm_chain> c(make_chain(parity_tips ? V_LOGLIK_PARITY : V_LOGLIK, x, 1, n, q.data(), pid, b.data(), om, nullptr, 0, 0,
                                           opt, nullptr, true));
    *out = c->loglik();
  });
}

int pm_debug_clade_schedule(const int32_t* edge, int32_t n_edges, int32_t n_tips, const int32_t* nen, const int32_t* nodelist,
                            int32_t root, int32_t nwarps, int32_t clade_max, int64_t* stats, char* err, size_t errlen) {
  return guarded(err, errlen, [&] {
    if (!edge || !nen || !nodelist || !stats || nwarps < 1) fail(PM_ERR_ARG, "bad argument");
    pm::host::Schedule sch;
    try { pm::host::build_schedule(n_tips, n_edges, edge, nen, nodelist, root, false, sch); }
    catch (const std::string& msg) { fail(PM_ERR_ARG, "%s", msg.c_str()); }
    pm::host::CladeSchedule cs;
    pm::host::build_clade_schedule(sch, nwarps, clade_max, cs);
    const int T = n_tips, NN = 2 * T - 1;
    std::vector<int> owner(NN, -2), posn(NN, -1);
    const int n1 = cs.warp_off[nwarps];
    long long lo = 1LL << 60, hi = 0, nprev = 0;
    for (int w = 0; w < nwarps; w++) {
      lo = std::min<long long>(lo, cs.warp_off[w + 1] - cs.warp_off[w]);
      hi = std::max<long long>(hi, cs.warp_off[w + 1] - cs.warp_off[w]);
      int prev = -1;
      for (int i = cs.warp_off[w]; i < cs.warp_off[w + 1]; i++) {
        const int* en = &cs.entries[(size_t)8 * i];
        const int v = en[0], fl = en[5];
        if (v < T || v >= NN || owner[v] != -2) fail(PM_ERR_ARG, "node %d scheduled twice or out of range", v);
        const int kids[2] = {en[1], en[3]};
        for (int c = 0; c < 2; c++) {
          const int k = kids[c], isprev = fl & (c ? 2 : 1), isload = fl & (c ? 8 : 4);
          if (k < T) { if (isprev || isload) fail(PM_ERR_ARG, "tip child of %d flagged", v); continue; }
          if (owner[k] != w) fail(PM_ERR_ARG, "child %d of %d is not an earlier node of the same warp", k, v);
          if (isprev ? (k != prev) : (!isload || posn[k] >= i - 1)) fail(PM_ERR_ARG, "flags of node %d", v);
          if (isprev) nprev++;
        }
        if ((fl & 4) && (fl & 8)) fail(PM_ERR_ARG, "node %d would load both children", v);
        owner[v] = w; posn[v] = i; prev = v;
      }
    }
    const int ntop = (int)cs.entries.size() / 8 - n1;
    for (size_t l = 0; l + 1 < cs.top_off.size(); l++)
      for (int i = cs.top_off[l]; i < cs.top_off[l + 1]; i++) {
        const int* en = &cs.entries[(size_t)8 * i];
        const int v = en[0];
        if (v < T || v >= NN || owner[v] != -2) fail(PM_ERR_ARG, "top node %d scheduled twice", v);
        const int kids[2] = {en[1], en[3]};
        for (int k : kids) if (k >= T && (owner[k] == -2 || (owner[k] == -1 && posn[k] >= cs.top_off[l]))) fail(PM_ERR_ARG, "top node %d before its child %d", v, k);
        owner[v] = -1; posn[v] = i;
      }
    for (int v = T; v < NN; v++) if (owner[v] == -2) fail(PM_ERR_ARG, "node %d never scheduled", v);
    std::vector<int> seen(NN, 0);
    seen[sch.root] = 1;
    for (size_t l = 0; l + 1 < cs.down_top_off.size(); l++) {
      for (int i = cs.down_top_off[l]; i < cs.down_top_off[l + 1]; i++) {
        const int* en = &cs.down_top[(size_t)4 * i];
        if (seen[en[0]] || !seen[en[1]] || seen[en[1]] > (int)l + 1) fail(PM_ERR_ARG, "top-down order of node %d", en[0]);
      }
      for (int i = cs.down_top_off[l]; i < cs.down_top_off[l + 1]; i++) seen[cs.down_top[(size_t)4 * i]] = (int)l + 2;
    }
    for (int w = 0; w < nwarps; w++) {
      int prev = -1;
      for (int i = cs.down_warp_off[w]; i < cs.down_warp_off[w + 1]; i++) {
        const int* en = &cs.down_seq[(size_t)4 * i];
        if (seen[en[0]] || !seen[en[1]]) fail(PM_ERR_ARG, "pre-order of node %d", en[0]);
        if (en[3] && en[1] != prev) fail(PM_ERR_ARG, "parent-is-previous flag of node %d", en[0]);
        if (sch.e_child[en[2]] != en[0] || sch.e_parent[en[2]] != en[1]) fail(PM_ERR_ARG, "edge of node %d", en[0]);
        seen[en[0]] = 1 << 20; prev = en[0];
      }
    }
    for (int v = T; v < NN; v++) if (!seen[v]) fail(PM_ERR_ARG, "node %d never drawn", v);
    stats[0] = n1; stats[1] = ntop; stats[2] = (long long)cs.top_off.size() - 1; stats[3] = lo; stats[4] = hi; stats[5] = nprev;
    stats[6] = cs.down_warp_off[nwarps]; stats[7] = (long long)cs.down_top.size() / 4;
  });
}

int pm_tree_order(const int32_t* edge, int32_t n_edges, int32_t n_tips, int32_t* nen, int32_t* nodelist, int32_t* root,
                  char* err, size_t errlen) {
  return guarded(err, errlen, [&] {
    if (!edge || !nen || !nodelist || !root) fail(PM_ERR_ARG, "null argument");
    pm::host::tree_order(edge, n_edges, n_tips, nen, nodelist, root);
  });
}

int pm_chain_create(int32_t variant, const pm_tree* trees, int32_t ntrees, int32_t n, double* Q, const double* pid,
                    double* B, double Omega, const double* prior, int32_t nprior, int32_t N_total, const pm_options* opt,
                    pm_chain** out, char* err, size_t errlen) {
  return guarded(err, errlen, [&] {
    if (!out) fail(PM_ERR_ARG, "null output");
    *out = make_chain(variant, trees, ntrees, n, Q, pid, B, Omega, prior, nprior, N_total, opt);
  });
}
int pm_chain_run(pm_chain* c, int32_t count, double* out, int64_t ld, char* err, size_t errlen) {
  return guarded(err, errlen, [&] {
    if (!c || (!out && count > 0)) fail(PM_ERR_ARG, "null argument");
    c->run(count, out, ld);
  });
}
int64_t pm_chain_state_bytes(pm_chain* c) { return c ? c->state_bytes() : 0; }
int pm_chain_export_state(pm_chain* c, void* buf, int64_t bytes, char* err, size_t errlen) {
  return guarded(err, errlen, [&] {
    if (!c) fail(PM_ERR_ARG, "null argument");
    c->export_state(buf, bytes);
  });
}
int pm_chain_import_state(pm_chain* c, const void* buf, int64_t bytes, char* err, size_t errlen) {
  return guarded(err, errlen, [&] {
    if (!c) fail(PM_ERR_ARG, "null argument");
    c->import_state(buf, bytes);
  });
}
int pm_chain_time_prune(pm_chain* c, int32_t tree, int32_t reps, float* ms_per_pass, char* err, size_t errlen) {
  return guarded(err, errlen, [&] {
    if (!c || !ms_per_pass) fail(PM_ERR_ARG, "null argument");
    *ms_per_pass = c->time_prune(tree, reps);
  });
}
void pm_chain_kernel_times(pm_chain* c, double ms[4], int64_t* launches) {
  for (int i = 0; i < 4; i++) ms[i] = c->kernel_ms[i];
  if (launches) *launches = c->launches;
}
void pm_chain_enable_timing(pm_chain* c, int32_t on) { c->timing = on != 0; }
void pm_chain_overheads(pm_chain* c, double ms[2]) { ms[0] = c->comm_ms; ms[1] = c->host_update_ms; }
int pm_chain_get_node_states(pm_chain* c, int32_t tree, int32_t* out) {
  return guarded(nullptr, 0, [&] { c->node_states(tree, out); });
}
int pm_chain_get_piece_counts(pm_chain* c, int32_t tree, int32_t* out) {
  return guarded(nullptr, 0, [&] { c->piece_counts(tree, out); });
}
int pm_chain_get_path(pm_chain* c, int32_t tree, int64_t site, int32_t e, double* len, int32_t* st, int32_t cap) {
  int r = -1;
// ... 53 lines not shown
```

phylomap_b200/csrc/pm_kernels.cuh:

```cuda
#pragma once
#include <type_traits>
#include "pm_device.cuh"

namespace pm {

template <typename Real>
struct ChainParams {
  int n, T, E;
  const int* cap_off;
  long long S;
  const Real* model;
  const Real* ppow;
  int jcap;
  const int* up_entries; const int* up_off; int n_up_levels;
  int* rec_cursor;
  const int* cl_entries; const int* cl_warp_off; const int* cl_top_entries; const int* cl_top_off; int n_cl_top_levels;
  const int* cd_top; const int* cd_top_off; int n_cd_top_levels; const int* cd_entries; const int* cd_warp_off;
  const long long* cd_tips; int n_cd_tips;
  const int* down_entries; const int* down_off; int n_down_levels;
  const int* e_parent; const int* e_child; const Real* e_len;
  const long long* maps_off; const double* maps_len;
  int root;
  const uint8_t* tipcode; long long TS;
  uint8_t* node_state; uint32_t* meta; Real* PL;
  long long tile_base, pl_S;
  int rec_shift; long long rec_groups;
  const uint32_t* ctl;
  uint32_t* hard_ballot; int W;
  const long long* wk_off; const int* wk_g; long long wk_total;
  const int* wk_hint;
  const unsigned long long* wk_item;
  int chunk;
  long long easy_blocks;
  uint16_t* shape;
  Real* rec_len[2]; uint8_t* rec_st[2];
  int normalize, full_counts, parity_tips;
  double* dw_partial; unsigned long long* cnt; int* root_out;
  unsigned* err_flag;
  RngDesc rng;
};

template <typename Real, int NC>
__device__ __forceinline__ void tip_partial(int code, int n, bool parity, Real* v) {
#pragma unroll
  for (int j = 0; j < n; j++) v[j] = parity ? (Real)((j & 1) != code) : (Real)(j == code);
}

template <typename Real, int NC, bool EXACT>
__device__ __forceinline__ void apply_power(const ChainParams<Real>& P, const Real* sBs, const Real* sPow, int npow_s, int n,
                                            int k, Real* v) {
  if (k <= 0) return;
  if (!EXACT) {
    if (k < npow_s) { matvec<Real, NC, false>(sPow + k * n * n, n, v); return; }
    if (k < P.jcap) { matvec<Real, NC, false>(P.ppow + (size_t)k * n * n, n, v); return; }
  }
  for (int r = 0; r < k; r++) matvec<Real, NC, EXACT>(sBs, n, v);
}

template <typename Real>
__device__ __forceinline__ void load_model_smem(const ChainParams<Real>& P, int n, Real* sB, Real* sBs, Real* sVec ,
                                                Real* sPow, int npow_s) {
  for (int i = threadIdx.x; i < n * n; i += blockDim.x) { if (sB) sB[i] = P.model[i]; sBs[i] = P.model[n * n + i]; }
  if (sVec) for (int i = threadIdx.x; i < 3 * n; i += blockDim.x) sVec[i] = P.model[2 * n * n + i];
  for (int i = threadIdx.x; i < npow_s * n * n; i += blockDim.x) sPow[i] = P.ppow[i];
}

template <int NS, bool EXACT> __host__ __device__ constexpr int smem_pow_count() { return (!EXACT && NS > 0 && NS <= 4) ? PM_SMEM_POW : 0; }

template <typename Real, int NS, bool EXACT>
__global__ void __launch_bounds__(256) k_prune(ChainParams<Real> P) {
  constexpr int NC = NS > 0 ? NS : PM_NMAX;
  const int n = NS > 0 ? NS : P.n;
  extern __shared__ __align__(16) unsigned char smem_raw[];
  Real* sBs = reinterpret_cast<Real*>(smem_raw);
  Real* sPow = sBs + n * n;
  const int npow_s = min(smem_pow_count<NS, EXACT>(), P.jcap);
  load_model_smem<Real>(P, n, nullptr, sBs, nullptr, sPow, npow_s);
  __syncthreads();
  const int lane = threadIdx.x & 31, warp = threadIdx.x >> 5, nw = blockDim.x >> 5;
  const long long S = P.S;
  const long long site = (long long)blockIdx.x * 32 + lane;
  const bool active = site < S;
  const bool parity = P.parity_tips != 0;
  for (int l = 0; l < P.n_up_levels; l++) {
    const int beg = __ldg(P.up_off + l), end = __ldg(P.up_off + l + 1);
    for (int idx = beg + warp; idx < end; idx += nw) {
      const int* en = P.up_entries + 5 * idx;
      const int pn = __ldg(en), a = __ldg(en + 1), ea = __ldg(en + 2), b = __ldg(en + 3), eb = __ldg(en + 4);
      if (active) {
        const int ka = (int)(P.meta[(long long)ea * S + site] & 0xffffu) - 1;
        const int kb = (int)(P.meta[(long long)eb * S + site] & 0xffffu) - 1;
        Real va[NC], vb[NC];
        if (a < P.T) tip_partial<Real, NC>(P.tipcode[(long long)a * P.TS + site], n, parity, va);
        else VecIO<Real, NS>::load(P.PL + ((long long)(a - P.T) * S + site) * n, n, va);
        if (b < P.T) tip_partial<Real, NC>(P.tipcode[(long long)b * P.TS + site], n, parity, vb);
        else VecIO<Real, NS>::load(P.PL + ((long long)(b - P.T) * S + site) * n, n, vb);
        apply_power<Real, NC, EXACT>(P, sBs, sPow, npow_s, n, kb, vb);
        apply_power<Real, NC, EXACT>(P, sBs, sPow, npow_s, n, ka, va);
        Real out[NC];
#pragma unroll
        for (int j = 0; j < n; j++) out[j] = Ar<Real, EXACT>::mul(vb[j], va[j]);
        if (P.normalize) {
          if (EXACT) {
            Real a1 = 0, a2 = 0;
#pragma unroll
            for (int j = 0; j < n; j++) { if (j & 1) a2 = Ar<Real, true>::add(a2, out[j]); else a1 = Ar<Real, true>::add(a1, out[j]); }
            const Real s = Ar<Real, true>::add(a1, a2);
#pragma unroll
            for (int j = 0; j < n; j++) out[j] = Ar<Real, true>::div(out[j], s);
          } else {
            Real s = 0;
#pragma unroll
            for (int j = 0; j < n; j++) s += out[j];
            const Real inv = s > (Real)0 ? (Real)1 / s : (Real)0;
#pragma unroll
            for (int j = 0; j < n; j++) out[j] *= inv;
          }
        }
        VecIO<Real, NS>::store(P.PL + ((long long)(pn - P.T) * S + site) * n, n, out);
      }
    }
    __syncthreads();
  }
}

template <typename Real, int NS>
__device__ __forceinline__ void pow_times(const ChainParams<Real>& P, const Real* sPow, int npow_s, int k, Real* v) {
  if (k < npow_s) {
    const Real* M = sPow + k * NS * NS;
    Real y[NS];
#pragma unroll
    for (int i = 0; i < NS; i++) {
      Real acc = 0;
#pragma unroll
      for (int j = 0; j < NS; j++) acc += M[i * NS + j] * v[j];
      y[i] = acc;
    }
#pragma unroll
    for (int i = 0; i < NS; i++) v[i] = y[i];
  } else if (k < P.jcap) {
    matvec<Real, NS, false>(P.ppow + (size_t)k * NS * NS, NS, v);
  } else {
    for (int r = 0; r < k; r++) matvec<Real, NS, false>(sPow + NS * NS, NS, v);
  }
}

template <typename Real> __device__ __forceinline__ Real fast_rcp(Real x) { return (Real)1 / x; }
template <> __device__ __forceinline__ float fast_rcp<float>(float x) {
  float r; asm("rcp.approx.ftz.f32 %0, %1;" : "=f"(r) : "f"(x)); return r;
}

template <typename Real, int NS>
struct PruneNode {
  int pn; uint32_t ma, mb;
  int ca, cb;
  Real va[NS], vb[NS];
};

__device__ __forceinline__ void cp_async4(unsigned dst, const void* gsrc, bool pred) {
  const int sz = pred ? 4 : 0;
  asm volatile("cp.async.ca.shared.global [%0], [%1], 4, %2;" ::"r"(dst), "l"(gsrc), "r"(sz) : "memory");
}
__device__ __forceinline__ void cp_async4(unsigned dst, const void* gsrc) {
  asm volatile("cp.async.ca.shared.global [%0], [%1], 4;" ::"r"(dst), "l"(gsrc) : "memory");
}
__device__ __forceinline__ void cp_async16(unsigned dst, const void* gsrc) {
  asm volatile("cp.async.ca.shared.global [%0], [%1], 16;" ::"r"(dst), "l"(gsrc) : "memory");
}
__device__ __forceinline__ void cp_async_commit() { asm volatile("cp.async.commit_group;" ::: "memory"); }
template <int N> __device__ __forceinline__ void cp_async_wait() { asm volatile("cp.async.wait_group %0;" ::"n"(N) : "memory"); }
__device__ __forceinline__ int lds_u16(unsigned a) { unsigned short v; asm volatile("ld.shared.u16 %0, [%1];" : "=h"(v) : "r"(a)); return (int)v; }
__device__ __forceinline__ int lds_u8(unsigned a) { unsigned v; asm volatile("ld.shared.u8 %0, [%1];" : "=r"(v) : "r"(a)); return (int)v; }
__device__ __forceinline__ int4 lds_v4(unsigned a) {
  int4 v; asm volatile("ld.shared.v4.s32 {%0,%1,%2,%3}, [%4];" : "=r"(v.x), "=r"(v.y), "=r"(v.z), "=r"(v.w) : "r"(a)); return v;
}
template <typename Real, int NS> __device__ __forceinline__ void lds_vec(unsigned a, Real* v);
template <> __device__ __forceinline__ void lds_vec<float, 4>(unsigned a, float* v) {
  asm volatile("ld.shared.v4.f32 {%0,%1,%2,%3}, [%4];" : "=f"(v[0]), "=f"(v[1]), "=f"(v[2]), "=f"(v[3]) : "r"(a));
}
template <> __device__ __forceinline__ void lds_vec<float, 2>(unsigned a, float* v) {
  asm volatile("ld.shared.v2.f32 {%0,%1}, [%2];" : "=f"(v[0]), "=f"(v[1]) : "r"(a));
}
template <> __device__ __forceinline__ void lds_vec<double, 2>(unsigned a, double* v) {
  asm volatile("ld.shared.v2.f64 {%0,%1}, [%2];" : "=d"(v[0]), "=d"(v[1]) : "r"(a));
}
template <> __device__ __forceinline__ void lds_vec<double, 4>(unsigned a, double* v) {
  asm volatile("ld.shared.v2.f64 {%0,%1}, [%2];" : "=d"(v[0]), "=d"(v[1]) : "r"(a));
  asm volatile("ld.shared.v2.f64 {%0,%1}, [%2];" : "=d"(v[2]), "=d"(v[3]) : "r"(a + 16));
}
__device__ __forceinline__ int lds_s32(unsigned a) { int v; asm volatile("ld.shared.s32 %0, [%1];" : "=r"(v) : "r"(a)); return v; }

#define PM_CLADE_SLOT 384
#define PM_CLADE_ENTRY_INTS 16

template <typename Real, int NS, int DEPTH>
__device__ __forceinline__ void prune_clade_block(const ChainParams<Real>& P, const long long site0, const long long pl0) {
  extern __shared__ __align__(16) unsigned char smem_raw[];
  Real* sPow = reinterpret_cast<Real*>(smem_raw + PM_CLADE_SLOT * 8 * DEPTH);
  Real* sPowT = sPow + PM_SMEM_POW * NS * NS;
  const int npow_s = min(PM_SMEM_POW, P.jcap);
  for (int i = threadIdx.x; i < npow_s * NS * NS; i += blockDim.x) {
    const Real v = P.ppow[i];
    sPow[i] = v;
    const int k = i / (NS * NS), r = (i / NS) % NS, c = i % NS;
    sPowT[k * NS * NS + c * NS + r] = v;
  }
  __syncthreads();
  const int lane = threadIdx.x & 31, warp = threadIdx.x >> 5, nw = blockDim.x >> 5;
  const long long S = P.S;
  const long long site_raw = site0 + lane;
  const bool active = site_raw < S;
  const long long site = active ? site_raw : S - 1;
  const bool parity = P.parity_tips != 0;
  const int T = P.T;
  const uint32_t* __restrict__ meta = P.meta + site;
  const uint8_t* __restrict__ tip = P.tipcode + site;
  Real* PLs = P.PL + (pl0 + (site - site0)) * NS;
  const long long rowPL = P.pl_S * NS;

  auto contribution = [&](int k, int code, Real* v) {
    if (code >= 0 && !parity && k < npow_s) {
      VecIO<Real, NS>::load(sPowT + k * NS * NS + code * NS, NS, v);
    } else {
      if (code >= 0) tip_partial<Real, NS>(code, NS, parity, v);
      pow_times<Real, NS>(P, sPow, npow_s, k, v);
    }
  };
  auto product = [&](const Real* va, const Real* vb, Real* out) {
    Real sum = 0;
#pragma unroll
    for (int j = 0; j < NS; j++) { out[j] = vb[j] * va[j]; sum += out[j]; }
    if (sizeof(Real) == 4 && !(sum > (Real)1e-30)) {
      double d[NS], ds = 0;
#pragma unroll
      for (int j = 0; j < NS; j++) { d[j] = (double)vb[j] * (double)va[j]; ds += d[j]; }
      const double di = ds > 0 ? 1.0 / ds : 0.0;
#pragma unroll
      for (int j = 0; j < NS; j++) out[j] = (Real)(d[j] * di);
      return;
    }
    const Real inv = sum > (Real)0 ? fast_rcp<Real>(sum) : (Real)0;
#pragma unroll
    for (int j = 0; j < NS; j++) out[j] *= inv;
  };

  {
    const int i0 = __ldg(P.cl_warp_off + warp), i1 = __ldg(P.cl_warp_off + warp + 1);
    unsigned ring = (unsigned)__cvta_generic_to_shared(smem_raw) + warp * (DEPTH * PM_CLADE_SLOT);
    asm volatile("" : "+r"(ring));
    char* const plb = reinterpret_cast<char*>(PLs);
    const char* const mtb = reinterpret_cast<const char*>(meta);
    const char* const tpb = reinterpret_cast<const char*>(P.tipcode) + site0 + 4 * (lane & 7);
    const bool tip_in = site0 + 4 * (lane & 7) < S;
    const int4* ep = reinterpret_cast<const int4*>(P.cl_entries) + 4 * (long long)i0;
    unsigned long long plb_u = reinterpret_cast<unsigned long long>(plb), mtb_u = reinterpret_cast<unsigned long long>(mtb),
                       tpb_u = reinterpret_cast<unsigned long long>(tpb);
    int act = active ? 1 : 0;
    asm volatile("" : "+l"(plb_u), "+l"(mtb_u), "+l"(tpb_u), "+r"(act));
    auto off64 = [](int lo, int hi) { return (long long)(((unsigned long long)(unsigned)hi << 32) | (unsigned)lo); };
    const bool role_b = (lane >> 3) == 1, role_nxt = lane >= 21, role_ent = lane >= 16;
    unsigned long long cbase = role_ent ? (unsigned long long)(role_nxt ? (long long)DEPTH * 64 + 16 + 4 * (lane - 21)
                                                                        : (lane == 20 ? 48 : 4 * (lane - 16)))
                                        : tpb_u;
    unsigned dst_off = lane >= 29 ? 340 + 4 * (lane - 29) : role_nxt ? 352 + 4 * (lane - 21) : 256 + 4 * lane;
    int lrole = ((lane < 29 && (role_ent || tip_in)) ? 1 : 0) | (role_nxt ? 2 : 0) | (role_b ? 4 : 0) | (role_ent ? 8 : 0);
    unsigned lane4 = 4 * lane;
    unsigned fast_pow = ((!parity || NS == 4) && npow_s == PM_SMEM_POW) ? (unsigned)PM_SMEM_POW : 0u;
    int lane_v = lane;
    asm volatile("" : "+l"(cbase), "+r"(dst_off), "+r"(lrole), "+r"(lane4), "+r"(fast_pow), "+r"(lane_v));
    auto issue = [&](unsigned slot, const int4* e, const int4& q1, const int4& q2, bool more) {
      cp_async4(slot + lane4, reinterpret_cast<const char*>(mtb_u) + off64(q1.x, q1.y));
      cp_async4(slot + 128 + lane4, reinterpret_cast<const char*>(mtb_u) + off64(q1.z, q1.w));
      const long long tipoff = (lrole & 4) ? off64(q2.z, q2.w) : off64(q2.x, q2.y);
      const long long X = (lrole & 8) ? reinterpret_cast<long long>(e) : tipoff;
      const bool on = (lrole & 1) && X >= 0 && (more || !(lrole & 2));
      cp_async4(slot + dst_off, reinterpret_cast<const char*>(cbase + (unsigned long long)(X >= 0 ? X : 0LL)), on);
    };
#pragma unroll 1
    for (int u = 0; u < DEPTH; u++) {
      if (i0 + u < i1) { issue(ring + u * PM_CLADE_SLOT, ep, __ldg(ep + 1), __ldg(ep + 2), i0 + u + DEPTH < i1); ep += 4; }
      cp_async_commit();
    }
    Real prev[NS], xA[NS], xB[NS];
#pragma unroll
    for (int j = 0; j < NS; j++) { prev[j] = 0; xA[j] = 0; xB[j] = 0; }
    long long pnA = 0, pnB = 0;
    int flA = 0, flB = 0;
    if (i0 < i1) {
      cp_async_wait<DEPTH - 1>();
      __syncwarp();
      const int4 h = lds_v4(ring + 320);
      pnA = off64(h.x, h.y);
      flA = lds_s32(ring + 336);
    }
    unsigned slot = ring;
    unsigned ring_end = ring + DEPTH * PM_CLADE_SLOT;
    asm volatile("" : "+r"(ring_end));
    auto tip_column = [&](int k, int code, Real* v) {
      if (!parity) { VecIO<Real, NS>::load(sPowT + (k * NS + code) * NS, NS, v); return; }
      Real c0[NS], c1[NS];
      const int j0 = 1 - code;
      VecIO<Real, NS>::load(sPowT + (k * NS + j0) * NS, NS, c0);
      VecIO<Real, NS>::load(sPowT + (k * NS + (j0 + 2 < NS ? j0 + 2 : j0)) * NS, NS, c1);
#pragma unroll
      for (int j = 0; j < NS; j++) v[j] = c0[j] + c1[j];
    };
    auto step = [&](int idx, long long pn_off, int fl, const Real* xcur, long long& pn_off_n, int& fl_n, Real* xnext) {
      const unsigned slot_n = (slot + PM_CLADE_SLOT == ring_end) ? ring : slot + PM_CLADE_SLOT;
      cp_async_wait<DEPTH - 2>();
      __syncwarp();
      if (idx + 1 < i1) {
        const int4 h = lds_v4(slot_n + 320);
        fl_n = lds_s32(slot_n + 336);
        pn_off_n = off64(h.x, h.y);
        if (h.w >= 0) VecIO<Real, NS>::load(reinterpret_cast<const Real*>(plb_u + (unsigned long long)off64(h.z, h.w)), NS, xnext);
      }
      const int ma = lds_u16(slot + lane4), mb = lds_u16(slot + 128 + lane4);
      Real va[NS], vb[NS];
      const bool fast = __all_sync(0xffffffffu, ((unsigned)(ma - 1) | (unsigned)(mb - 1)) < fast_pow);
      if (fast) {
        if (fl & 16) tip_column(ma - 1, lds_u8(slot + 256 + lane_v), va);
        else {
          const Real* Ma = sPow + (ma - 1) * NS * NS;
          Real src[NS];
#pragma unroll
          for (int j = 0; j < NS; j++) src[j] = (fl & 1) ? prev[j] : xcur[j];
#pragma unroll
          for (int r = 0; r < NS; r++) {
            Real row[NS];
            VecIO<Real, NS>::load(Ma + r * NS, NS, row);
            Real acc = 0;
#pragma unroll
            for (int c = 0; c < NS; c++) acc += row[c] * src[c];
            va[r] = acc;
          }
        }
        if (fl & 32) tip_column(mb - 1, lds_u8(slot + 288 + lane_v), vb);
        else {
          const Real* Mb = sPow + (mb - 1) * NS * NS;
          Real src[NS];
#pragma unroll
          for (int j = 0; j < NS; j++) src[j] = (fl & 2) ? prev[j] : xcur[j];
#pragma unroll
          for (int r = 0; r < NS; r++) {
            Real row[NS];
            VecIO<Real, NS>::load(Mb + r * NS, NS, row);
            Real acc = 0;
#pragma unroll
            for (int c = 0; c < NS; c++) acc += row[c] * src[c];
            vb[r] = acc;
          }
        }
      } else {
        const int ca = (fl & 16) ? lds_u8(slot + 256 + lane_v) : -1, cb = (fl & 32) ? lds_u8(slot + 288 + lane_v) : -1;
#pragma unroll
        for (int j = 0; j < NS; j++) {
          va[j] = (fl & 1) ? prev[j] : xcur[j];
          vb[j] = (fl & 2) ? prev[j] : xcur[j];
        }
        contribution(mb - 1, cb, vb);
        contribution(ma - 1, ca, va);
      }
      product(va, vb, prev);
      if (act) VecIO<Real, NS>::store(reinterpret_cast<Real*>(plb_u + (unsigned long long)pn_off), NS, prev);
      __syncwarp();
      if (idx + DEPTH < i1) {
        const int4 q1 = lds_v4(slot + 352), q2 = lds_v4(slot + 368);
        __syncwarp();
        issue(slot, ep, q1, q2, idx + 2 * DEPTH < i1);
        ep += 4;
      }
      cp_async_commit();
      slot = slot_n;
    };
#pragma unroll 1
    for (int idx = i0; idx < i1; idx += 2) {
      step(idx, pnA, flA, xA, pnB, flB, xB);
      if (idx + 1 < i1) step(idx + 1, pnB, flB, xB, pnA, flA, xA);
    }
    cp_async_wait<0>();
  }
  __syncthreads();

  const int4* __restrict__ ent = reinterpret_cast<const int4*>(P.cl_top_entries);
  auto load = [&](PruneNode<Real, NS>& nd, int id) {
    const int4 e0 = __ldg(ent + 2 * id), e1 = __ldg(ent + 2 * id + 1);
    nd.pn = e0.x;
    nd.ma = meta[(long long)e0.z * S];
    nd.mb = meta[(long long)e1.x * S];
    nd.ca = -1; nd.cb = -1;
    if (e0.y < T) nd.ca = tip[(long long)e0.y * P.TS];
    else VecIO<Real, NS>::load(PLs + (long long)(e0.y - T) * rowPL, NS, nd.va);
    if (e0.w < T) nd.cb = tip[(long long)e0.w * P.TS];
    else VecIO<Real, NS>::load(PLs + (long long)(e0.w - T) * rowPL, NS, nd.vb);
  };
  auto compute = [&](PruneNode<Real, NS>& nd) {
    contribution((int)(nd.mb & 0xffffu) - 1, nd.cb, nd.vb);
    contribution((int)(nd.ma & 0xffffu) - 1, nd.ca, nd.va);
    Real out[NS];
    product(nd.va, nd.vb, out);
    if (active) VecIO<Real, NS>::store(PLs + (long long)(nd.pn - T) * rowPL, NS, out);
  };
  PruneNode<Real, NS> A, B;
  for (int l = 0; l < P.n_cl_top_levels; l++) {
    const int beg = __ldg(P.cl_top_off + l), end = __ldg(P.cl_top_off + l + 1);
    int idx = beg + warp;
    if (idx < end) load(A, idx);
    while (idx < end) {
      if (idx + nw < end) load(B, idx + nw);
      compute(A);
      idx += nw;
      if (idx >= end) break;
      if (idx + nw < end) load(A, idx + nw);
      compute(B);
      idx += nw;
    }
    __syncthreads();
  }
}

template <typename Real, int NS, int DEPTH, int MINB>
__global__ void __launch_bounds__(256, MINB) k_prune_clade(ChainParams<Real> P) {
  prune_clade_block<Real, NS, DEPTH>(P, P.tile_base + (long long)blockIdx.x * 32, (long long)blockIdx.x * 32);
}

template <typename Real, int NS, bool EXACT>
__global__ void __launch_bounds__(256) k_nodes(ChainParams<Real> P, uint32_t iter) {
  if (P.ctl) iter = P.ctl[0];
  constexpr int NC = NS > 0 ? NS : PM_NMAX;
  typedef typename StreamSel<Real, EXACT>::type Stream;
  const int n = NS > 0 ? NS : P.n;
  extern __shared__ __align__(16) unsigned char smem_raw[];
  Real* sBs = reinterpret_cast<Real*>(smem_raw);
  Real* sVec = sBs + n * n;
  Real* sPow = sVec + 3 * n;
  const int npow_s = min(smem_pow_count<NS, EXACT>(), P.jcap);
  load_model_smem<Real>(P, n, nullptr, sBs, sVec, sPow, npow_s);
  __syncthreads();
  const int lane = threadIdx.x & 31, warp = threadIdx.x >> 5, nw = blockDim.x >> 5;
  const long long S = P.S;
  const long long site = (long long)blockIdx.x * 32 + lane;
  const bool active = site < S;
  const bool parity = P.parity_tips != 0;
  if (warp == 0 && active) {
    Real w[NC], pl[NC];
    VecIO<Real, NS>::load(P.PL + ((long long)(P.root - P.T) * S + site) * n, n, pl);
#pragma unroll
    for (int j = 0; j < n; j++) w[j] = Ar<Real, EXACT>::mul(sVec[j], pl[j]);
    Stream g; g.open(P.rng, (uint32_t)site, iter, K_NODE, (uint32_t)P.root, P.err_flag);
    const int s = categorical<Real, NC, EXACT>(w, n, g.next(), P.err_flag);
    P.node_state[(long long)P.root * S + site] = (uint8_t)s;
    if (P.rng.site0 + (uint32_t)site == 0u) *P.root_out = s;
  }
  __syncthreads();
  for (int l = 0; l < P.n_down_levels; l++) {
    const int beg = __ldg(P.down_off + l), end = __ldg(P.down_off + l + 1);
    for (int idx = beg + warp; idx < end; idx += nw) {
      const int* en = P.down_entries + 3 * idx;
      const int v = __ldg(en), pn = __ldg(en + 1), e = __ldg(en + 2);
      if (active) {
        const int ps = P.node_state[(long long)pn * S + site];
        const int k = (int)(P.meta[(long long)e * S + site] & 0xffffu) - 1;
        Real w[NC], pl[NC];
        bool done = false;
        if (!EXACT && k > 0) {
          const Real* M = (k < npow_s) ? (sPow + k * n * n) : (k < P.jcap ? P.ppow + (size_t)k * n * n : nullptr);
          if (M) {
#pragma unroll
            for (int j = 0; j < n; j++) w[j] = M[ps * n + j];
            done = true;
          }
        }
        if (!done) {
#pragma unroll
          for (int j = 0; j < n; j++) w[j] = (Real)(j == ps);
          for (int r = 0; r < k; r++) matvec_t<Real, NC, EXACT>(sBs, n, w);
        }
        if (v < P.T) tip_partial<Real, NC>(P.tipcode[(long long)v * P.TS + site], n, parity, pl);
        else VecIO<Real, NS>::load(P.PL + ((long long)(v - P.T) * S + site) * n, n, pl);
#pragma unroll
        for (int j = 0; j < n; j++) w[j] = Ar<Real, EXACT>::mul(w[j], pl[j]);
        Stream g; g.open(P.rng, (uint32_t)site, iter, K_NODE, (uint32_t)v, P.err_flag);
        const int s = categorical<Real, NC, EXACT>(w, n, g.next(), P.err_flag);
        P.node_state[(long long)v * S + site] = (uint8_t)s;
      }
    }
    __syncthreads();
  }
}

template <typename Real> __device__ __forceinline__ Real u01_from_word(uint32_t x);
template <> __device__ __forceinline__ float u01_from_word<float>(uint32_t x) { return ((float)(x >> 8) + 0.5f) * (1.0f / 16777216.0f); }
template <> __device__ __forceinline__ double u01_from_word<double>(uint32_t x) { return ((double)x + 0.5) * (1.0 / 4294967296.0); }

template <typename Real, int NS, bool EXACT>
__global__ void __launch_bounds__(128) k_paths(ChainParams<Real> P, uint32_t iter, int first, int chunk) {
  if (P.ctl) { iter = P.ctl[0]; first = iter == 0u; }
  constexpr int NC = NS > 0 ? NS : PM_NMAX;
  typedef typename StreamSel<Real, EXACT>::type Stream;
  typedef ExpDev<Real, EXACT> Exp;
  typedef Ar<Real, EXACT> A;
  typedef Ar<Real, true> AX;
  typedef typename std::conditional<EXACT, double, Real>::type Acc;
  const int n = NS > 0 ? NS : P.n;
  extern __shared__ __align__(16) unsigned char smem_raw[];
  double* s_dw = reinterpret_cast<double*>(smem_raw);
  unsigned* s_cnt = reinterpret_cast<unsigned*>(s_dw + 4 * n);
  Real* sB = reinterpret_cast<Real*>(s_cnt + n * n + ((n * n) & 1));
  Real* sBs = sB + n * n;
  Real* sVec = sBs + n * n;
  Real* sPow = sVec + 3 * n;
  const int npow_s = min(smem_pow_count<NS, EXACT>(), P.jcap);
  load_model_smem<Real>(P, n, sB, sBs, sVec, sPow, npow_s);
  for (int i = threadIdx.x; i < n * n; i += blockDim.x) s_cnt[i] = 0;
  for (int i = threadIdx.x; i < 4 * n; i += blockDim.x) s_dw[i] = 0.0;
  __syncthreads();
  const Real* s_scale_old = sVec + n;
  const Real* s_scale_new = sVec + 2 * n;
  const long long S = P.S;
  const long long site = (long long)blockIdx.x * blockDim.x + threadIdx.x;
  const bool active = site < S;
  const int e0 = blockIdx.y * chunk, e1 = min(P.E, e0 + chunk);
  const int cap0 = __ldg(P.cap_off + blockIdx.y), cap_c = __ldg(P.cap_off + blockIdx.y + 1) - cap0;
  const long long abase = (long long)cap0 * S + (active ? site : 0) * (long long)cap_c;
  const Real* __restrict__ rd_len = P.rec_len[(iter & 1u) ^ 1u] + abase;
  const uint8_t* __restrict__ rd_st = P.rec_st[(iter & 1u) ^ 1u] + abase;
  Real* __restrict__ wr_len = P.rec_len[iter & 1u] + abase;
  uint8_t* __restrict__ wr_st = P.rec_st[iter & 1u] + abase;
  int rd = 0, wr = 0;
  const bool full = P.full_counts != 0;
  Acc Racc[NS > 0 ? NS : 1];
#pragma unroll
  for (int j = 0; j < (NS > 0 ? NS : 1); j++) Racc[j] = 0;
  unsigned errbits = 0;

  if (active) for (int e = e0; e < e1; e++) {
    const long long pe = (long long)e * S + site;
    const uint32_t mt = P.meta[pe];
    const int m = (int)(mt & 0xffffu), nj = (int)((mt >> 16) & 0xffu), s0 = (int)(mt >> 24);
    const int ps = P.node_state[(long long)__ldg(P.e_parent + e) * S + site];
    const int cs = P.node_state[(long long)__ldg(P.e_child + e) * S + site];
    int nout = 0, newm = 0, sfirst = 0;
    Stream gnew; gnew.open(P.rng, (uint32_t)site, iter, K_BREXP, (uint32_t)e, P.err_flag);

    auto emit = [&](Real L, int s, bool final_run) {
      if (nout == 0) sfirst = s;
      const bool skip = (!EXACT) && final_run && nout == 0;
      if (!skip) {
        if (wr < cap_c && nout < PM_LOCAL_PATH_MAX) { wr_len[wr] = L; wr_st[wr] = (uint8_t)s; wr++; }
        else errbits |= (nout >= PM_LOCAL_PATH_MAX) ? PM_DE_JUMP_LIMIT : PM_DE_PATH_CAP;
      }
      if (NS > 0) {
#pragma unroll
        for (int j = 0; j < (NS > 0 ? NS : 1); j++) Racc[j] += (s == j) ? (Acc)L : (Acc)0;
      } else atomicAdd(&s_dw[s], (double)L);
      const Real sc = s_scale_new[s];
      if (isfinite(sc) && sc > (Real)0) {
        Real tot = 0;
        for (;;) {
          const Real g = AX::mul(sc, Exp::draw(gnew));
          const Real t2 = AX::add(tot, g);
          if (t2 < L) { tot = t2; newm++; if (newm > 70000) break; } else break;
        }
      }
      newm++;
      nout++;
    };

    if (!EXACT && !first && nj == 0 && (m == 1 || (m == 2 && ps == cs))) {
      if (full && m == 2) atomicAdd(&s_cnt[ps * n + cs], 1u);
      emit(__ldg(P.e_len + e), cs, true);
    } else {
      Real in_len[PM_LOCAL_PATH_MAX]; uint8_t in_st[PM_LOCAL_PATH_MAX];
      int nin = 0;
      if (!first) {
        if (!EXACT && nj == 0) { nin = 1; in_len[0] = __ldg(P.e_len + e); in_st[0] = (uint8_t)s0; }
        else {
          nin = min(nj + 1, PM_LOCAL_PATH_MAX);
          for (int c = 0; c < nin; c++) { const int q = min(rd + c, cap_c - 1); in_len[c] = rd_len[q]; in_st[c] = rd_st[q]; }
          rd += nj + 1;
        }
      }
      Stream gold;
      gold.open(P.rng, (uint32_t)site, first ? iter : iter - 1u, K_BREXP, (uint32_t)e, P.err_flag);
      Stream gst; gst.open(P.rng, (uint32_t)site, iter, K_BRSTATE, (uint32_t)e, P.err_flag);
      int j = 0; Real tot = 0; long long cp = first ? P.maps_off[e] : 0;
      auto next_piece = [&]() -> Real {
        if (first) return (Real)P.maps_len[cp++];
        if (j >= nin) { errbits |= PM_DE_INCONSISTENT; return (Real)0; }
        const Real L = in_len[j];
        const Real sc = s_scale_old[in_st[j]];
        if (isfinite(sc) && sc > (Real)0) {
          const Real g = AX::mul(sc, Exp::draw(gold));
          const Real t2 = AX::add(tot, g);
          if (t2 < L) { tot = t2; return g; }
        }
        const Real r = AX::sub(L, tot);
        j++; tot = 0;
        return r;
      };
      int cur_state = (m == 1) ? cs : ps;
      Real cur_len = next_piece();
      int prev = cur_state;
      for (int p = 1; p < m; p++) {
        int st;
        if (p == m - 1) st = cs;
        else {
          const int jd = m - p - 1;
          Real w[NC];
          const Real* M = (jd < npow_s) ? (sPow + jd * n * n) : (jd < P.jcap ? P.ppow + (size_t)jd * n * n : nullptr);
          if (M) {
#pragma unroll
            for (int c = 0; c < n; c++) w[c] = M[c * n + cs];
          } else {
#pragma unroll
            for (int c = 0; c < n; c++) w[c] = (Real)(c == cs);
            for (int r = 0; r < jd; r++) matvec<Real, NC, EXACT>(sBs, n, w);
          }
#pragma unroll
          for (int c = 0; c < n; c++) w[c] = A::mul(sB[prev * n + c], w[c]);
          st = categorical<Real, NC, EXACT>(w, n, gst.next(), P.err_flag);
        }
        const Real len = next_piece();
        if (full) atomicAdd(&s_cnt[prev * n + st], 1u);
        if (st == cur_state) cur_len = A::add(cur_len, len);
        else {
          emit(cur_len, cur_state, false);
          if (!full) atomicAdd(&s_cnt[cur_state * n + st], 1u);
          cur_state = st; cur_len = len;
        }
        prev = st;
      }
      if (!EXACT && nout == 0) cur_len = __ldg(P.e_len + e);
      emit(cur_len, cur_state, true);
    }
    if (newm > 65535) { errbits |= PM_DE_M_OVERFLOW; newm = 65535; }
    if (nout > PM_LOCAL_PATH_MAX) nout = PM_LOCAL_PATH_MAX;
    P.meta[pe] = (uint32_t)newm | ((uint32_t)(nout - 1) << 16) | ((uint32_t)sfirst << 24);
  }
  if (errbits) atomicOr(P.err_flag, errbits);

  if (NS > 0) {
    const int lane = threadIdx.x & 31, warp = threadIdx.x >> 5;
#pragma unroll
    for (int j = 0; j < (NS > 0 ? NS : 1); j++) {
      double v = (double)Racc[j];
#pragma unroll
      for (int o = 16; o > 0; o >>= 1) v += __shfl_down_sync(0xffffffffu, v, o);
      if (lane == 0) s_dw[warp * n + j] = v;
    }
  }
  __syncthreads();
  const long long blk = (long long)blockIdx.y * gridDim.x + blockIdx.x;
  if ((int)threadIdx.x < n) {
    double v;
    if (NS > 0) { v = 0; for (int w = 0; w < (int)(blockDim.x >> 5); w++) v += s_dw[w * n + threadIdx.x]; }
    else v = s_dw[threadIdx.x];
    P.dw_partial[blk * n + threadIdx.x] = v;
  }
  for (int i = threadIdx.x; i < n * n; i += blockDim.x) if (s_cnt[i]) atomicAdd(&P.cnt[i], (unsigned long long)s_cnt[i]);
}

template <typename Real, int NS>
__device__ __forceinline__ int draw_node_state(const ChainParams<Real>& P, const Real* sBs, const Real* sPow, int npow_s, int k, int ps,
                                               const Real* pl, uint32_t word) {
  Real w[NS];
  if (k < npow_s) VecIO<Real, NS>::load(sPow + (k * NS + ps) * NS, NS, w);
  else if (k < P.jcap) {
#pragma unroll
    for (int j = 0; j < NS; j++) w[j] = P.ppow[(size_t)k * NS * NS + ps * NS + j];
  } else {
#pragma unroll
    for (int j = 0; j < NS; j++) w[j] = (Real)(j == ps);
    for (int r = 0; r < k; r++) matvec_t<Real, NS, false>(sBs, NS, w);
  }
#pragma unroll
  for (int j = 0; j < NS; j++) w[j] *= pl[j];
  Real c[NS];
  c[0] = w[0];
#pragma unroll
  for (int j = 1; j < NS; j++) c[j] = c[j - 1] + w[j];
  const Real tot = c[NS - 1];
  if (!(tot > (Real)0) || !isfinite(tot)) { atomicOr(P.err_flag, tot > (Real)0 ? PM_DE_SAMPLE_NA : PM_DE_SAMPLE_ZERO); return 0; }
  const Real t = u01_from_word<Real>(word) * tot;
  int pick = 0;
#pragma unroll
  for (int j = 0; j < NS - 1; j++) pick += (t >= c[j]) ? 1 : 0;
  if (!(t < tot)) {
#pragma unroll
    for (int j = 0; j < NS; j++) if (w[j] > (Real)0) pick = j;
  }
  return pick;
}

template <typename Real>
__device__ __forceinline__ int draw_parity_tip4(const ChainParams<Real>& P, const Real* sBs, const Real* sPow, int npow_s, int k, int ps,
                                                int code, uint32_t word) {
  Real w[4];
  if (k < npow_s) VecIO<Real, 4>::load(sPow + (k * 4 + ps) * 4, 4, w);
  else if (k < P.jcap) {
#pragma unroll
    for (int j = 0; j < 4; j++) w[j] = P.ppow[(size_t)k * 16 + ps * 4 + j];
  } else {
#pragma unroll
    for (int j = 0; j < 4; j++) w[j] = (Real)(j == ps);
    for (int r = 0; r < k; r++) matvec_t<Real, 4, false>(sBs, 4, w);
  }
  const Real ra = code ? w[0] : w[1], rb = code ? w[2] : w[3];
  const Real tot = ra + rb;
  if (!(tot > (Real)0) || !isfinite(tot)) { atomicOr(P.err_flag, tot > (Real)0 ? PM_DE_SAMPLE_NA : PM_DE_SAMPLE_ZERO); return 0; }
  const Real t = u01_from_word<Real>(word) * tot;
  const int a = 1 - code;
  int pick = (t < ra) ? a : a + 2;
  if (!(t < tot)) pick = (rb > (Real)0) ? a + 2 : a;
  return pick;
}
template <typename Real, int NS>
__device__ __forceinline__ int draw_tip_state(const ChainParams<Real>& P, const Real* sBs, const Real* sPow, int npow_s, int k, int ps, int code,
                                              bool parity, uint32_t word) {
  if (NS == 4 && parity) return draw_parity_tip4<Real>(P, sBs, sPow, npow_s, k, ps, code, word);
  Real pl[NS];
  tip_partial<Real, NS>(code, NS, parity, pl);
  return draw_node_state<Real, NS>(P, sBs, sPow, npow_s, k, ps, pl, word);
}

template <typename Real, int NS, int DEPTH>
__device__ __forceinline__ void nodes_clade_block(const ChainParams<Real>& P, const uint32_t iter, const long long site0, const long long pl0) {
  constexpr int PB = NS * (int)sizeof(Real);
  constexpr int PLB = 32 * PB;
  constexpr int SLOT = PLB + 160;
  extern __shared__ __align__(16) unsigned char smem_raw[];
  Real* sBs = reinterpret_cast<Real*>(smem_raw + SLOT * 8 * DEPTH);
  Real* sVec = sBs + NS * NS;
  Real* sPow = sVec + 3 * NS;
  const int npow_s = min(PM_SMEM_POW, P.jcap);
  load_model_smem<Real>(P, NS, nullptr, sBs, sVec, sPow, npow_s);
  __syncthreads();
  const int lane = threadIdx.x & 31, warp = threadIdx.x >> 5, nw = blockDim.x >> 5;
  const long long S = P.S;
  const long long site_raw = site0 + lane;
  const bool active = site_raw < S;
  const long long site = active ? site_raw : S - 1;
  const long long lsite = pl0 + (site - site0);
  const bool parity = P.parity_tips != 0;
  const int T = P.T;
  const uint32_t gsite = P.rng.site0 + (uint32_t)site;
  const uint32_t kslot = make_slot(K_NODEGRP, 0u);
  uint8_t* const nst = P.node_state + site;
  if (warp == 0) {
    Real w[NS], pl[NS];
    VecIO<Real, NS>::load(P.PL + ((long long)(P.root - T) * P.pl_S + lsite) * NS, NS, pl);
#pragma unroll
    for (int j = 0; j < NS; j++) w[j] = sVec[j] * pl[j];
    uint32_t o[4];
    philox4x32_10_rk(0xffffffffu, kslot, iter, gsite, P.rng.rk, o);
    const int s = categorical<Real, NS, false>(w, NS, u01_from_word<Real>(o[0]), P.err_flag);
    if (active) {
      nst[(long long)P.root * S] = (uint8_t)s;
      if (gsite == 0u) *P.root_out = s;
    }
  }
  __syncthreads();
  for (int l = 0; l < P.n_cd_top_levels; l++) {
    const int beg = __ldg(P.cd_top_off + l), end = __ldg(P.cd_top_off + l + 1);
    for (int idx = beg + warp; idx < end; idx += nw) {
      const int4 en = __ldg(reinterpret_cast<const int4*>(P.cd_top) + idx);
      const int ps = nst[(long long)en.y * S];
      const int k = (int)(P.meta[(long long)en.z * S + site] & 0xffffu) - 1;
      Real pl[NS];
      VecIO<Real, NS>::load(P.PL + ((long long)(en.x - T) * P.pl_S + lsite) * NS, NS, pl);
      uint32_t o[4];
      philox4x32_10_rk(0x80000000u + (uint32_t)idx, kslot, iter, gsite, P.rng.rk, o);
      const int s = draw_node_state<Real, NS>(P, sBs, sPow, npow_s, k, ps, pl, o[0]);
      if (active) nst[(long long)en.x * S] = (uint8_t)s;
    }
    __syncthreads();
  }
  {
    const int i0 = __ldg(P.cd_warp_off + warp), i1 = __ldg(P.cd_warp_off + warp + 1);
    unsigned ring = (unsigned)__cvta_generic_to_shared(smem_raw) + warp * (DEPTH * SLOT);
    asm volatile("" : "+r"(ring));
    unsigned long long plb_u = reinterpret_cast<unsigned long long>(P.PL + lsite * NS),
                       mtb_u = reinterpret_cast<unsigned long long>(P.meta + site),
                       nsb_u = reinterpret_cast<unsigned long long>(nst);
    int act = active ? 1 : 0;
    unsigned lane4 = 4 * lane, lanePB = PB * lane;
    unsigned long long hsrc = lane < 4 ? 16 + 4 * lane : (unsigned long long)DEPTH * 64 + 4 * (lane - 4);
    unsigned hdst = PLB + 128 + 4 * lane;
    asm volatile("" : "+l"(plb_u), "+l"(mtb_u), "+l"(nsb_u), "+r"(act), "+r"(lane4), "+r"(lanePB), "+l"(hsrc), "+r"(hdst));
    auto off64 = [](int lo, int hi) { return (long long)(((unsigned long long)(unsigned)hi << 32) | (unsigned)lo); };
    const int4* ep = reinterpret_cast<const int4*>(P.cd_entries) + 4 * (long long)i0;
    auto issue = [&](unsigned slot, const int4* e, const int4& q0, bool more) {
      const char* src = reinterpret_cast<const char*>(plb_u) + off64(q0.x, q0.y);
      if (PB == 8) asm volatile("cp.async.ca.shared.global [%0], [%1], 8;" ::"r"(slot + lanePB), "l"(src) : "memory");
      else {
        cp_async16(slot + lanePB, src);
        if (PB == 32) cp_async16(slot + lanePB + 16, src + 16);
      }
      cp_async4(slot + PLB + lane4, reinterpret_cast<const char*>(mtb_u) + off64(q0.z, q0.w));
      if (lane < 8) cp_async4(slot + hdst, reinterpret_cast<const char*>(e) + hsrc, lane < 4 || more);
    };
#pragma unroll 1
    for (int u = 0; u < DEPTH; u++) {
      if (i0 + u < i1) { issue(ring + u * SLOT, ep, __ldg(ep), i0 + u + DEPTH < i1); ep += 4; }
      cp_async_commit();
    }
    long long vA = 0, vB = 0, pA = -1, pB = -1;
    int psA = 0, psB = 0;
    if (i0 < i1) {
      cp_async_wait<DEPTH - 1>();
      __syncwarp();
      const int4 h = lds_v4(ring + PLB + 128);
      vA = off64(h.x, h.y); pA = off64(h.z, h.w);
      if (pA >= 0) psA = *reinterpret_cast<const uint8_t*>(nsb_u + (unsigned long long)pA);
    }
    unsigned slot = ring;
    unsigned ring_end = ring + DEPTH * SLOT;
    asm volatile("" : "+r"(ring_end));
    int sprev = 0;
    uint32_t o[4] = {0, 0, 0, 0};
    auto step = [&](int idx, long long v_off, long long p_off, int ps_mem, long long& v_off_n, long long& p_off_n, int& ps_mem_n) {
      const unsigned slot_n = (slot + SLOT == ring_end) ? ring : slot + SLOT;
      cp_async_wait<DEPTH - 2>();
      __syncwarp();
      if (idx + 1 < i1) {
        const int4 h = lds_v4(slot_n + PLB + 128);
        v_off_n = off64(h.x, h.y); p_off_n = off64(h.z, h.w);
        if (h.w >= 0) ps_mem_n = *reinterpret_cast<const uint8_t*>(nsb_u + (unsigned long long)p_off_n);
      }
      if ((idx & 3) == 0 || idx == i0) philox4x32_10_rk((uint32_t)idx >> 2, kslot, iter, gsite, P.rng.rk, o);
      const uint32_t word = (idx & 3) == 0 ? o[0] : (idx & 3) == 1 ? o[1] : (idx & 3) == 2 ? o[2] : o[3];
      Real pl[NS];
      lds_vec<Real, NS>(slot + lanePB, pl);
      const int k = lds_u16(slot + PLB + lane4) - 1;
      const int ps = p_off < 0 ? sprev : ps_mem;
      const int sn = draw_node_state<Real, NS>(P, sBs, sPow, npow_s, k, ps, pl, word);
      if (act) *reinterpret_cast<uint8_t*>(nsb_u + (unsigned long long)v_off) = (uint8_t)sn;
      sprev = sn;
      __syncwarp();
      if (idx + DEPTH < i1) {
        const int4 q0 = lds_v4(slot + PLB + 144);
        __syncwarp();
        issue(slot, ep, q0, idx + 2 * DEPTH < i1);
        ep += 4;
      }
      cp_async_commit();
      slot = slot_n;
    };
#pragma unroll 1
    for (int idx = i0; idx < i1; idx += 2) {
      step(idx, vA, pA, psA, vB, pB, psB);
      if (idx + 1 < i1) step(idx + 1, vB, pB, psB, vA, pA, psA);
    }
    cp_async_wait<0>();
  }
  if (P.n_cd_tips > 0) {
    __syncthreads();
    const int ntip = P.n_cd_tips, ngrp = (ntip + 3) >> 2;
    const uint8_t* const tipb = P.tipcode + site;
    const char* const mtb = reinterpret_cast<const char*>(P.meta + site);
    struct TipLoad { int ps, k, cd; };
    auto load = [&](int grp, TipLoad (&L)[4]) {
#pragma unroll
      for (int q = 0; q < 4; q++) {
        const int v = min(4 * grp + q, ntip - 1);
        const longlong2 en = __ldg(reinterpret_cast<const longlong2*>(P.cd_tips) + v);
        L[q].ps = nst[en.x];
        L[q].k = (int)(*reinterpret_cast<const uint32_t*>(mtb + en.y) & 0xffffu) - 1;
        L[q].cd = tipb[(long long)v * P.TS];
      }
    };
    auto draw = [&](int grp, const TipLoad (&L)[4]) {
      uint32_t o[4];
      philox4x32_10_rk(0x40000000u + (uint32_t)grp, kslot, iter, gsite, P.rng.rk, o);
#pragma unroll
      for (int q = 0; q < 4; q++) {
        if (4 * grp + q < ntip) {
          const uint32_t word = q == 0 ? o[0] : q == 1 ? o[1] : q == 2 ? o[2] : o[3];
          const int sn = draw_tip_state<Real, NS>(P, sBs, sPow, npow_s, L[q].k, L[q].ps, L[q].cd, parity, word);
          if (active) nst[(long long)(4 * grp + q) * S] = (uint8_t)sn;
        }
      }
    };
    TipLoad A[4], B[4];
    int grp = warp;
    if (grp < ngrp) load(grp, A);
    while (grp < ngrp) {
      if (grp + nw < ngrp) load(grp + nw, B);
      draw(grp, A);
      grp += nw;
      if (grp >= ngrp) break;
      if (grp + nw < ngrp) load(grp + nw, A);
      draw(grp, B);
      grp += nw;
    }
  }
}

template <typename Real, int NS, int DEPTH, int MINB>
__global__ void __launch_bounds__(256, MINB) k_nodes_clade(ChainParams<Real> P, uint32_t iter) {
  if (P.ctl) iter = P.ctl[0];
  nodes_clade_block<Real, NS, DEPTH>(P, iter, P.tile_base + (long long)blockIdx.x * 32, (long long)blockIdx.x * 32);
}

__device__ __forceinline__ unsigned long long global_ns() { unsigned long long t; asm volatile("mov.u64 %0, %%globaltimer;" : "=l"(t)); return t; }
__device__ __forceinline__ unsigned sm_id() { unsigned v; asm volatile("mov.u32 %0, %%smid;" : "=r"(v)); return v; }

template <typename Real, int NS, int DEPTH, int MINB>
__global__ void __launch_bounds__(256, MINB) k_prune_nodes_clade(ChainParams<Real> P, uint32_t iter, long long b0, int phases, int* slot_busy,
                                                                 int slots_per_sm, unsigned long long* phase_ns) {
  if (P.ctl) iter = P.ctl[0];
  __shared__ unsigned long long s_t[2];
  __shared__ int s_slot;
  if (threadIdx.x == 0) {
    int slot = (int)blockIdx.x;
    if (slot_busy) {
      const int base = (int)sm_id() * slots_per_sm;
      int k = 0;
      while (atomicCAS(slot_busy + base + k, 0, 1) != 0) k = (k + 1 == slots_per_sm) ? 0 : k + 1;
      slot = base + k;
    }
    s_slot = slot;
    if (phase_ns) s_t[0] = global_ns();
  }
  __syncthreads();
  const int slot = s_slot;
  const long long site0 = (b0 + blockIdx.x) * 32, pl0 = (long long)slot * 32;
  prune_clade_block<Real, NS, DEPTH>(P, site0, pl0);
  __syncthreads();
  if (phases & 2) {
    if (phase_ns && threadIdx.x == 0) s_t[1] = global_ns();
    nodes_clade_block<Real, NS, DEPTH>(P, iter, site0, pl0);
    __syncthreads();
    if (phase_ns && threadIdx.x == 0) {
      const unsigned long long t2 = global_ns();
      atomicAdd(phase_ns, s_t[1] - s_t[0]);
      atomicAdd(phase_ns + 1, t2 - s_t[1]);
    }
  }
  if (threadIdx.x == 0 && slot_busy) atomicExch(slot_busy + slot, 0);
}

#define PM_META(m, q) ((uint32_t)(m) | ((uint32_t)(q) << 16))

template <typename Real>
__device__ __forceinline__ bool rate_ok(Real r) { return isfinite(r) && r > (Real)0; }

__device__ __forceinline__ float lds_real(unsigned a, float) { float v; asm volatile("ld.shared.f32 %0, [%1];" : "=f"(v) : "r"(a)); return v; }
__device__ __forceinline__ double lds_real(unsigned a, double) { double v; asm volatile("ld.shared.f64 %0, [%1];" : "=d"(v) : "r"(a)); return v; }
__device__ __forceinline__ unsigned smem_addr(const void* p) { return (unsigned)__cvta_generic_to_shared(p); }

template <typename Real, int NS>
struct EasySmem {
  int cnt, rate, acc, sum, topo;
  __host__ __device__ static int up16(int x) { return (x + 15) & ~15; }
  __host__ __device__ explicit EasySmem(int n) {
    cnt = up16(4 * n * (int)sizeof(double));
    rate = up16(cnt + n * n * (int)sizeof(unsigned));
    acc = up16(rate + n * (int)sizeof(Real));
    sum = acc + (NS > 0 ? NS * 128 * (int)sizeof(Real) : 0);
    topo = sum + (NS > 0 ? NS * 128 * (int)sizeof(double) : 0);
  }
  __host__ __device__ int len(int chunk) const { return topo + chunk * 8; }
  __host__ __device__ size_t bytes(int chunk) const { return (size_t)len(chunk) + (size_t)chunk * sizeof(Real); }
};
__device__ __forceinline__ void lds_v2s32(unsigned a, int& x, int& y) { asm volatile("ld.shared.v2.s32 {%0,%1}, [%2];" : "=r"(x), "=r"(y) : "r"(a)); }
__device__ __forceinline__ void red_shared_inc_if(bool p, unsigned a) {
  asm volatile("{\n\t.reg .pred q;\n\tsetp.ne.b32 q, %1, 0;\n\t@q red.shared.add.u32 [%0], 1;\n\t}" ::"r"(a), "r"((unsigned)p) : "memory");
}
__device__ __forceinline__ void sts_add_if(bool p, unsigned a, float x) {
  asm volatile("{\n\t.reg .pred q;\n\t.reg .f32 v;\n\tsetp.ne.b32 q, %2, 0;\n\t@q ld.shared.f32 v, [%0];\n\t@q add.rn.f32 v, v, %1;\n\t"
               "@q st.shared.f32 [%0], v;\n\t}" ::"r"(a), "f"(x), "r"((unsigned)p));
}
__device__ __forceinline__ void sts_add_if(bool p, unsigned a, double x) {
  asm volatile("{\n\t.reg .pred q;\n\t.reg .f64 v;\n\tsetp.ne.b32 q, %2, 0;\n\t@q ld.shared.f64 v, [%0];\n\t@q add.rn.f64 v, v, %1;\n\t"
               "@q st.shared.f64 [%0], v;\n\t}" ::"r"(a), "d"(x), "r"((unsigned)p));
}
__device__ __forceinline__ void sts_real(unsigned a, float x) { asm volatile("st.shared.f32 [%0], %1;" ::"r"(a), "f"(x)); }
__device__ __forceinline__ void sts_real(unsigned a, double x) { asm volatile("st.shared.f64 [%0], %1;" ::"r"(a), "d"(x)); }
__device__ __forceinline__ uint32_t ldg_u32(const uint32_t* a) { uint32_t v; asm volatile("ld.global.u32 %0, [%1];" : "=r"(v) : "l"(a)); return v; }
__device__ __forceinline__ int ldg_u8(const uint8_t* a) { uint32_t v; asm volatile("ld.global.u8 %0, [%1];" : "=r"(v) : "l"(a)); return (int)v; }
__device__ __forceinline__ void stg_u32_if(bool p, uint32_t* a, uint32_t x) {
  asm volatile("{\n\t.reg .pred q;\n\tsetp.ne.b32 q, %2, 0;\n\t@q st.global.u32 [%0], %1;\n\t}" ::"l"(a), "r"(x), "r"((unsigned)p));
}
__device__ __forceinline__ void stg_u16_if(bool p, uint16_t* a, uint16_t x) {
  asm volatile("{\n\t.reg .pred q;\n\tsetp.ne.b32 q, %2, 0;\n\t@q st.global.u16 [%0], %1;\n\t}" ::"l"(a), "h"(x), "r"((unsigned)p));
}

template <typename Real, int NS>
__global__ void __launch_bounds__(128, (sizeof(Real) == 8 ? 6 : 8)) k_paths_easy(ChainParams<Real> P, uint32_t iter, int chunk) {
  if (P.ctl) iter = P.ctl[0];
  constexpr int NR = NS > 0 ? NS : 1;
  typedef Pin<Real> PN;
  const int n = NS > 0 ? NS : P.n;
  extern __shared__ __align__(16) unsigned char smem_raw[];
  const EasySmem<Real, NS> lay(n);
  double* s_dw = reinterpret_cast<double*>(smem_raw);
  unsigned* s_cnt = reinterpret_cast<unsigned*>(smem_raw + lay.cnt);
  Real* s_rate = reinterpret_cast<Real*>(smem_raw + lay.rate);
  Real* s_acc = reinterpret_cast<Real*>(smem_raw + lay.acc);
  double* s_sum = reinterpret_cast<double*>(smem_raw + lay.sum);
  int2* s_topo = reinterpret_cast<int2*>(smem_raw + lay.topo);
  Real* s_len = reinterpret_cast<Real*>(smem_raw + lay.len(chunk));
  const int e0 = blockIdx.y * chunk, e1 = min(P.E, e0 + chunk);
  for (int i = threadIdx.x; i < n * n; i += blockDim.x) s_cnt[i] = 0;
  for (int i = threadIdx.x; i < n; i += blockDim.x) {
    const Real r = P.model[2 * n * n + 4 * n + i];
    s_rate[i] = rate_ok(r) ? r : (Real)0;
  }
  for (int i = threadIdx.x; i < 4 * n; i += blockDim.x) s_dw[i] = 0.0;
  if (NS > 0) for (int j = 0; j < NS; j++) { s_acc[j * 128 + threadIdx.x] = 0; s_sum[j * 128 + threadIdx.x] = 0.0; }
  for (int i = threadIdx.x; i < e1 - e0; i += blockDim.x) {
    s_topo[i] = make_int2(P.e_parent[e0 + i], P.e_child[e0 + i]);
    s_len[i] = P.e_len[e0 + i];
  }
  __syncthreads();
  unsigned a_base = smem_addr(smem_raw);
  asm volatile("" : "+r"(a_base));
  const unsigned a_cnt = a_base + (unsigned)lay.cnt, a_rate = a_base + (unsigned)lay.rate, a_topo = a_base + (unsigned)lay.topo,
                 a_len = a_base + (unsigned)lay.len(chunk);
  const unsigned a_acc = a_base + (unsigned)lay.acc + (unsigned)sizeof(Real) * threadIdx.x,
                 a_sum = a_base + (unsigned)lay.sum + (unsigned)sizeof(double) * threadIdx.x;
  const long long S = P.S;
  uint32_t Su = (uint32_t)S;
  const long long site_raw = (long long)blockIdx.x * blockDim.x + threadIdx.x;
  const long long site = site_raw < S ? site_raw : S - 1;
  const bool full = P.full_counts != 0;
  const long long wglob = site_raw >> 5;
  uint32_t* __restrict__ bal_b = P.hard_ballot + (long long)e0 * P.W + wglob;
  unsigned bal_writer = (threadIdx.x & 31) == 0 && wglob < (long long)P.W;
  uint32_t Wu = (uint32_t)P.W;
  uint32_t* __restrict__ meta_b = P.meta + (long long)e0 * S + site;
  uint16_t* __restrict__ shape_b = P.shape + (long long)e0 * S + site;
  uint32_t row = 0, rowf = 0, rowb = 0;
  const uint8_t* __restrict__ nstate = P.node_state + site;
  if (sizeof(Real) == 4) asm volatile("" : "+l"(bal_b), "+l"(meta_b), "+l"(shape_b), "+l"(nstate), "+r"(Wu), "+r"(Su), "+r"(bal_writer));
  auto add_dwell = [&](int s, Real L, bool p) {
    if (NS > 0) sts_add_if(p, a_acc + (unsigned)s * (unsigned)(128 * sizeof(Real)), L);
    else if (p && L != (Real)0) atomicAdd(&s_dw[s], (double)L);
  };
  auto flush_dwell = [&]() {
    if (NS > 0) {
#pragma unroll
      for (int j = 0; j < NR; j++) {
        const unsigned a = a_acc + (unsigned)j * (unsigned)(128 * sizeof(Real)), b = a_sum + (unsigned)j * (128u * 8u);
        sts_real(b, lds_real(b, 0.0) + (double)lds_real(a, (Real)0));
        sts_real(a, (Real)0);
      }
    }
  };
  const int nb = e1 - e0;
  struct Ahead { uint32_t mt; int ps, cs; };
  Ahead X = {0, 0, 0}, Y = {0, 0, 0};
  auto fetch = [&](int i, Ahead& a) {
    a.mt = ldg_u32(meta_b + rowf); rowf += Su;
    int par, chi;
    lds_v2s32(a_topo + 8u * (unsigned)i, par, chi);
    a.ps = ldg_u8(nstate + (uint64_t)(uint32_t)par * Su);
    a.cs = ldg_u8(nstate + (uint64_t)(uint32_t)chi * Su);
  };
  uint32_t po[4] = {0, 0, 0, 0};
  const PairBlocks pb(P.rng, iter);
  const uint32_t gsite = P.rng.site0 + (uint32_t)site;
  auto body = [&](int i, auto odd_c, auto newblk_c, auto tail_c, const Ahead cur) {
    constexpr bool ODD = decltype(odd_c)::value, NEWBLK = decltype(newblk_c)::value, TAIL = decltype(tail_c)::value;
    const int e = e0 + i;
    const uint32_t mt = cur.mt; const int ps = cur.ps, cs = cur.cs;
    if (NEWBLK) pb.block(P.rng, (uint32_t)e >> 1, gsite, po);
    const uint32_t wA = ODD ? po[2] : po[0], wB = ODD ? po[3] : po[1];
    const int m = (int)(mt & 0xffffu);
    const uint32_t q = mt >> 16;
    const Real Le = lds_real(a_len + (unsigned)sizeof(Real) * (unsigned)i, (Real)0);
    const bool two = (m == 2) && (ps != cs);
    const Real p1 = pos_dec<Real>(q, Le);
    const Real L0 = two ? p1 : Le;
    const int s0 = two ? ps : cs;
    const Real L1 = two ? PN::sub(Le, p1) : (Real)0;
    const Real lam = PN::add(PN::mul(lds_real(a_rate + (unsigned)sizeof(Real) * (unsigned)s0, (Real)0), L0),
                             PN::mul(lds_real(a_rate + (unsigned)sizeof(Real) * (unsigned)cs, (Real)0), L1));
    const bool hard = (m > 2) || lam > (Real)PM_LAMBDA_INV;
    const bool ok = TAIL ? (!hard && site_raw < S) : !hard;
    const int k = poisson_inv<Real>(lam, wA);
    red_shared_inc_if(ok && m == 2 && (full || two), a_cnt + 4u * (unsigned)(ps * n + cs));
    add_dwell(s0, L0, ok);
    add_dwell(cs, L1, ok && two);
    const uint32_t newq = (!two && k == 1) ? pos_rand(wB) : q;
    stg_u32_if(ok, meta_b + row, (newq << 16) + (uint32_t)((two ? 2 : 1) + k));
    stg_u16_if(ok, shape_b + row, (uint16_t)(((uint32_t)cs << 11) + ((uint32_t)s0 << 6) + (two ? 1u : 0u)));
    row += Su;
    const unsigned bal = __ballot_sync(0xffffffffu, TAIL ? (hard && site_raw < S) : hard);
    stg_u32_if(bal_writer != 0, bal_b + rowb, bal);
    rowb += Wu;
  };
  auto run = [&](auto tail_c) {
    const std::true_type T{}; const std::false_type F{};
    int i = 0;
    if (nb > 0 && (e0 & 1)) {
      fetch(0, X);
      body(0, T, T, tail_c, X);
      i = 1;
    }
    if (i < nb) fetch(i, X);
    if (i + 1 < nb) fetch(i + 1, Y);
    while (i + 3 < nb) {
      const int stop = min(nb - 4, i + 62);
      for (; i <= stop; i += 2) {
        const Ahead cx = X, cy = Y;
        fetch(i + 2, X); fetch(i + 3, Y);
        body(i, F, T, tail_c, cx);
        body(i + 1, T, F, tail_c, cy);
      }
      flush_dwell();
    }
    for (; i + 1 < nb; i += 2) {
      const Ahead cx = X, cy = Y;
      if (i + 2 < nb) fetch(i + 2, X);
      if (i + 3 < nb) fetch(i + 3, Y);
      body(i, F, T, tail_c, cx);
      body(i + 1, T, F, tail_c, cy);
    }
    if (i < nb) body(i, F, T, tail_c, X);
    flush_dwell();
  };
  if ((long long)(blockIdx.x + 1) * blockDim.x <= S) run(std::false_type()); else run(std::true_type());
  if (NS > 0) {
    const int lane = threadIdx.x & 31, warp = threadIdx.x >> 5;
#pragma unroll
    for (int j = 0; j < NR; j++) {
      double v = lds_real(a_sum + (unsigned)j * (128u * 8u), 0.0);
#pragma unroll
      for (int o = 16; o > 0; o >>= 1) v += __shfl_down_sync(0xffffffffu, v, o);
      if (lane == 0) s_dw[warp * n + j] = v;
    }
  }
  __syncthreads();
  const long long blk = (long long)blockIdx.y * gridDim.x + blockIdx.x;
  if ((int)threadIdx.x < n) {
    double v;
    if (NS > 0) { v = 0; for (int w = 0; w < (int)(blockDim.x >> 5); w++) v += s_dw[w * n + threadIdx.x]; }
    else v = s_dw[threadIdx.x];
    P.dw_partial[blk * n + threadIdx.x] = v;
  }
  for (int i = threadIdx.x; i < n * n; i += blockDim.x) if (s_cnt[i]) atomicAdd(&P.cnt[i], (unsigned long long)s_cnt[i]);
}

template <typename Real>
__device__ __forceinline__ Real rate_or_zero(Real r) { return rate_ok(r) ? r : (Real)0; }

template <typename Real>
struct RunPieces {
  Real L, x, rate;
  int left;
  bool gaps;
  bool firstB;
  uint32_t wB;
  WordStream ws;
  bool joint, pend, run0;
  Real v, sc;
  __device__ __forceinline__ void begin(const RngDesc& d, uint32_t site, uint32_t it, uint32_t e, int run, Real len, Real r,
                                       uint32_t cnt_word, bool single_run, uint32_t wordB) {
    L = len; x = 0; rate = r; left = 0; gaps = false; firstB = single_run; wB = wordB; joint = false;
    if (!rate_ok(r)) return;
    const Real lam = Pin<Real>::mul(r, len);
    if (lam > (Real)PM_LAMBDA_INV) { gaps = true; ws.open(d, site, it, K_BRGAP, e, (uint32_t)run); }
    else { left = poisson_inv<Real>(lam, cnt_word); ws.open(d, site, it, K_BRPOS, e, (uint32_t)run); }
  }
  __device__ __forceinline__ void begin_joint(const RngDesc& d, uint32_t site, uint32_t it, uint32_t e, Real len0, int K, Real lam0,
                                             Real lamT, Real r0, uint32_t wordB) {
    typedef Pin<Real> PN;
    L = len0; x = 0; left = K; gaps = false; firstB = true; wB = wordB; joint = true; pend = false; run0 = true;
    v = 0; rate = PN::div(lam0, lamT); sc = PN::div(lamT, r0);
    ws.open(d, site, it, K_BRPOS, e, 0u);
  }
  __device__ __forceinline__ void second_run(Real len1, Real lamT, Real r1) { L = len1; x = 0; run0 = false; sc = Pin<Real>::div(lamT, r1); }
  __device__ __forceinline__ Real next(bool& last) {
    typedef Pin<Real> PN;
    if (joint) {
      if (!pend && left > 0) {
        uint32_t w;
        if (firstB) { w = wB; firstB = false; } else w = ws.next();
        v = next_order_stat<Real>(v, (Real)1, left, w);
        left--; pend = true;
      }
      if (pend && (!run0 || v < rate)) {
        const Real t2 = min(PN::mul(run0 ? v : PN::sub(v, rate), sc), L);
        const Real piece = max(PN::sub(t2, x), (Real)0);
        x = max(t2, x); pend = false; last = false;
        return piece;
      }
      last = true;
      return PN::sub(L, x);
    }
    if (gaps) {
      const Real g = PN::div(PN::neglog(PN::u01(ws.next())), rate);
      const Real t2 = PN::add(x, g);
      if (t2 < L) { x = t2; last = false; return g; }
      last = true;
      return PN::sub(L, x);
    }
    if (left > 0) {
      uint32_t w;
      if (firstB) { w = wB; firstB = false; } else w = ws.next();
      const Real t2 = next_order_stat<Real>(x, L, left, w);
      const Real piece = PN::sub(t2, x);
      x = t2; left--; last = false;
      return piece;
    }
    last = true;
    return PN::sub(L, x);
  }
};

template <typename Real>
__device__ __noinline__ int count_gaps(RngDesc d, uint32_t site, uint32_t it, uint32_t e, uint32_t run, Real L, Real rate, Real* first) {
  typedef Pin<Real> PN;
  WordStream g; g.open(d, site, it, K_BRGAP, e, run);
  Real x = 0; int k = 0;
  for (;;) {
    const Real gp = PN::div(PN::neglog(PN::u01(g.next())), rate);
    const Real t2 = PN::add(x, gp);
    if (!(t2 < L) || k > 70000) break;
    x = t2; k++;
    if (k == 1) *first = gp;
  }
  return k;
}

template <typename Real>
struct HardItem { uint32_t site, e, meta, ends, shape; };

template <typename Real, int NS>
struct PathWorker {
  static constexpr int NC = NS > 0 ? NS : PM_NMAX;
  static constexpr int NR = NS > 0 ? NS : 1;
  typedef typename StreamSel<Real, false>::type Stream;
// ... 489 lines not shown
```

phylomap_b200/csrc/pm_launch.cuh:

```cuda
#pragma once
#include "pm_kernels.cuh"
#include "pm_small.cuh"

namespace pm {

template <typename Real, int NS, bool EXACT>
struct Sweep {
  static void prune(const ChainParams<Real>& P, int grid, size_t smem, cudaStream_t st);
  static void nodes(const ChainParams<Real>& P, int grid, size_t smem, cudaStream_t st, uint32_t iter);
  static int fused_blocks_per_sm(size_t smem_nodes);
  static void prune_nodes(const ChainParams<Real>& P, int grid, size_t smem_nodes, cudaStream_t st, uint32_t iter, long long b0,
                          int phases, int* slot_busy, int slots_per_sm, unsigned long long* phase_ns);
  static void paths(const ChainParams<Real>& P, dim3 grid, size_t smem, cudaStream_t st, uint32_t iter, int first, int chunk,
                    int hard_blocks);
  static size_t small_smem(int T);
  static void small_chain(const ChainParams<Real>& P, int sites, cudaStream_t st, uint32_t iter0, int nsweeps, const SmallOut& out,
                          bool two_per_sm);
};

}
```

phylomap_b200/csrc/pm_launch_impl.cuh:

```cuda
#pragma once
#include "pm_launch.cuh"

namespace pm {

template <typename Real, int NS, bool EXACT>
void Sweep<Real, NS, EXACT>::prune(const ChainParams<Real>& P, int grid, size_t smem, cudaStream_t st) {
  if constexpr (!EXACT && (NS == 2 || NS == 4)) {
    constexpr int D = 8, MB = sizeof(Real) == 8 ? 2 : 3;
    const size_t spow = 2 * PM_SMEM_POW * NS * NS * sizeof(Real);
    const size_t sm = spow + (size_t)PM_CLADE_SLOT * 8 * D;
    auto kern = k_prune_clade<Real, NS, D, MB>;
    cudaFuncSetAttribute(kern, cudaFuncAttributeMaxDynamicSharedMemorySize, (int)sm);
    kern<<<grid, 256, sm, st>>>(P);
  }
  else k_prune<Real, NS, EXACT><<<grid, 256, smem, st>>>(P);
}
template <typename Real, int NS, bool EXACT>
void Sweep<Real, NS, EXACT>::nodes(const ChainParams<Real>& P, int grid, size_t smem, cudaStream_t st, uint32_t iter) {
  if constexpr (!EXACT && (NS == 2 || NS == 4)) {
    constexpr int D = 8, MB = sizeof(Real) == 8 ? 2 : 3;
    const size_t sm = smem + (size_t)(32 * NS * sizeof(Real) + 160) * 8 * D;
    auto kern = k_nodes_clade<Real, NS, D, MB>;
    cudaFuncSetAttribute(kern, cudaFuncAttributeMaxDynamicSharedMemorySize, (int)sm);
    kern<<<grid, 256, sm, st>>>(P, iter);
  }
  else k_nodes<Real, NS, EXACT><<<grid, 256, smem, st>>>(P, iter);
}
template <typename Real, int NS, bool EXACT>
struct FusedCfg {
  static constexpr int D = 8, MB = sizeof(Real) == 8 ? 2 : 3;
  static size_t smem(size_t smem_nodes) {
    const size_t sm_prune = 2 * PM_SMEM_POW * (NS > 0 ? NS : 1) * (NS > 0 ? NS : 1) * sizeof(Real) + (size_t)PM_CLADE_SLOT * 8 * D;
    const size_t sm_nodes = smem_nodes + (size_t)(32 * (NS > 0 ? NS : 1) * sizeof(Real) + 160) * 8 * D;
    return sm_prune > sm_nodes ? sm_prune : sm_nodes;
  }
};
template <typename Real, int NS, bool EXACT>
int Sweep<Real, NS, EXACT>::fused_blocks_per_sm(size_t smem_nodes) {
  if constexpr (!EXACT && (NS == 2 || NS == 4)) {
    typedef FusedCfg<Real, NS, EXACT> C;
    auto kern = k_prune_nodes_clade<Real, NS, C::D, C::MB>;
    const size_t sm = C::smem(smem_nodes);
    cudaFuncSetAttribute(kern, cudaFuncAttributeMaxDynamicSharedMemorySize, (int)sm);
    int nb = 0;
    if (cudaOccupancyMaxActiveBlocksPerMultiprocessor(&nb, kern, 256, sm) != cudaSuccess) return 0;
    return nb;
  }
  return 0;
}
template <typename Real, int NS, bool EXACT>
void Sweep<Real, NS, EXACT>::prune_nodes(const ChainParams<Real>& P, int grid, size_t smem_nodes, cudaStream_t st, uint32_t iter,
                                         long long b0, int phases, int* slot_busy, int slots_per_sm, unsigned long long* phase_ns) {
  if constexpr (!EXACT && (NS == 2 || NS == 4)) {
    typedef FusedCfg<Real, NS, EXACT> C;
    auto kern = k_prune_nodes_clade<Real, NS, C::D, C::MB>;
    const size_t sm = C::smem(smem_nodes);
    cudaFuncSetAttribute(kern, cudaFuncAttributeMaxDynamicSharedMemorySize, (int)sm);
    kern<<<grid, 256, sm, st>>>(P, iter, b0, phases, slot_busy, slots_per_sm, phase_ns);
  }
}
template <typename Real, int NS, bool EXACT>
void Sweep<Real, NS, EXACT>::paths(const ChainParams<Real>& P, dim3 grid, size_t smem, cudaStream_t st, uint32_t iter,
                                   int first, int chunk, int hard_blocks) {
  if constexpr (EXACT) k_paths<Real, NS, true><<<grid, 128, smem, st>>>(P, iter, first, chunk);
  else {
    const size_t smem_easy = EasySmem<Real, NS>(P.n).bytes(chunk);
    k_paths_easy<Real, NS><<<grid, 128, smem_easy, st>>>(P, iter, chunk);
    if (!first) k_paths_hard<Real, NS, 8, 0><<<2 * hard_blocks, 128, smem, st>>>(P, iter, first);
    k_paths_hard<Real, NS, 4, 1><<<hard_blocks, 128, smem, st>>>(P, iter, first);
  }
}
template <typename Real, int NS, bool EXACT>
size_t Sweep<Real, NS, EXACT>::small_smem(int T) {
  if constexpr (!EXACT && (NS == 2 || NS == 4)) return (size_t)SmallSmem<Real, NS>(T).total;
  return (size_t)1 << 40;
}
template <typename Real, int NS, bool EXACT>
void Sweep<Real, NS, EXACT>::small_chain(const ChainParams<Real>& P, int sites, cudaStream_t st, uint32_t iter0, int nsweeps,
                                         const SmallOut& out, bool two_per_sm) {
  if constexpr (!EXACT && (NS == 2 || NS == 4)) {
    const size_t sm = (size_t)SmallSmem<Real, NS>(P.T).total;
    auto kern = two_per_sm ? k_small_chain<Real, NS, 2> : k_small_chain<Real, NS, 1>;
    cudaFuncSetAttribute(kern, cudaFuncAttributeMaxDynamicSharedMemorySize, (int)sm);
    kern<<<sites, 256, sm, st>>>(P, iter0, nsweeps, out);
  }
}

}
```

Before: 71.78 billion.

## Process two 32-site halves per warp in clade prune/node kernels for f32

Widens the clade prune and node-draw blocks to 64 sites per block for float, so each warp handles two 32-lane site halves against the same clade entry metadata and shared power matrices. The ring slot size, cp.async issue roles and host block sizing are generalised to the block width W. It also adds paired-float FMA and multiply helpers (__ffma2_rn, __fmul2_rn) for the matrix-vector and normalisation steps, and lowers min-blocks-per-SM from 3 to 2 for float. The aim is to amortise per-entry header loads and control overhead over more sites and raise FP32 throughput, at the cost of more registers and shared memory per block and fewer resident blocks.

```diff
diff --git a/phylomap_b200/csrc/pm_host.cu b/phylomap_b200/csrc/pm_host.cu
--- a/phylomap_b200/csrc/pm_host.cu
+++ b/phylomap_b200/csrc/pm_host.cu
@@ -642,6 +642,7 @@
     if (NS == 4) return f(std::integral_constant<int, 4>{});
     return f(std::integral_constant<int, 0>{});
   }
+  int clade_block_sites() const { return with_ns([](auto ns) { return pm::Sweep<Real, decltype(ns)::value, false>::block_sites; }); }
   template <typename F>
   auto with_ns_exact(F&& f) const {
     if constexpr (std::is_same_v<Real, double>)
@@ -656,7 +657,8 @@
     {
       pm::ChainParams<Real> P = t.P;
       P.ctl = ctl_d;
-      const int gx = (int)((t.S + 31) / 32);
+      constexpr int bs = pm::Sweep<Real, NSc, EX>::block_sites;
+      const int gx = (int)((t.S + bs - 1) / bs);
       if (t.pl_slots) {
         begin_timed(4);
         pm::Sweep<Real, NSc, EX>::prune_nodes(P, gx, smem_nodes, stream, iter, 0, 3, t.slots_per_sm ? t.slot_busy.template as<int>() : nullptr,
@@ -741,9 +743,10 @@
 
   template <int NSc, bool EX>
   void launch_prune_t(TreeDev<Real>& t, long long only_site) {
-    const long long nb = (t.S + 31) / 32;
+    constexpr int bs = pm::Sweep<Real, NSc, EX>::block_sites;
+    const long long nb = (t.S + bs - 1) / bs;
     if (t.pl_slots) {
-      if (only_site >= 0) pm::Sweep<Real, NSc, EX>::prune_nodes(t.P, 1, smem_nodes, stream, 0u, only_site / 32, 1, nullptr, 0, nullptr);
+      if (only_site >= 0) pm::Sweep<Real, NSc, EX>::prune_nodes(t.P, 1, smem_nodes, stream, 0u, only_site / bs, 1, nullptr, 0, nullptr);
       else pm::Sweep<Real, NSc, EX>::prune_nodes(t.P, (int)nb, smem_nodes, stream, 0u, 0, 1, t.slots_per_sm ? t.slot_busy.template as<int>() : nullptr,
                                                  t.slots_per_sm, nullptr);
     } else pm::Sweep<Real, NSc, EX>::prune(t.P, (int)nb, smem_prune, stream);
@@ -1065,9 +1068,10 @@
     if (per_sm < 1) fail(PM_ERR_CUDA, "cudaOccupancyMaxActiveBlocksPerMultiprocessor failed for the fused prune + node-draw kernel");
     t.slots_per_sm = per_sm;
     t.pl_slots = sm_id_range(opt.device, sms) * per_sm;
-    t.pl_sites = 32LL * t.pl_slots;
-    if (t.pl_sites >= ((t.S + 31) / 32) * 32) {
-      t.pl_slots = (int)((t.S + 31) / 32); t.pl_sites = 32LL * t.pl_slots; t.slots_per_sm = 0;
+    const int bs = clade_block_sites();
+    t.pl_sites = (long long)bs * t.pl_slots;
+    if (t.pl_sites >= ((t.S + bs - 1) / bs) * bs) {
+      t.pl_slots = (int)((t.S + bs - 1) / bs); t.pl_sites = (long long)bs * t.pl_slots; t.slots_per_sm = 0;
     } else {
       t.slot_busy.alloc((size_t)t.pl_slots * sizeof(int));
       CK(cudaMemsetAsync(t.slot_busy.p, 0, t.slot_busy.bytes, stream));
@@ -1550,7 +1554,7 @@
     CK(cudaSetDevice(opt.device));
     launch_prune(t, site);
     CK(cudaStreamSynchronize(stream));
-    const long long col = t.pl_slots ? site % 32 : site;
+    const long long col = t.pl_slots ? site % clade_block_sites() : site;
     std::fill(out, out + (size_t)(2 * T - 1) * n, 0.0);
     std::vector<Real> v(n);
     for (int i = 0; i < T - 1; i++) {
diff --git a/phylomap_b200/csrc/pm_kernels.cuh b/phylomap_b200/csrc/pm_kernels.cuh
--- a/phylomap_b200/csrc/pm_kernels.cuh
+++ b/phylomap_b200/csrc/pm_kernels.cuh
@@ -164,6 +164,9 @@
 __device__ __forceinline__ void cp_async4(unsigned dst, const void* gsrc) {
   asm volatile("cp.async.ca.shared.global [%0], [%1], 4;" ::"r"(dst), "l"(gsrc) : "memory");
 }
+__device__ __forceinline__ void cp_async4_if(bool pred, unsigned dst, const void* gsrc) {
+  asm volatile("{ .reg .pred p; setp.ne.b32 p, %2, 0; @p cp.async.ca.shared.global [%0], [%1], 4; }" ::"r"(dst), "l"(gsrc), "r"((int)pred) : "memory");
+}
 __device__ __forceinline__ void cp_async16(unsigned dst, const void* gsrc) {
   asm volatile("cp.async.ca.shared.global [%0], [%1], 16;" ::"r"(dst), "l"(gsrc) : "memory");
 }
@@ -190,13 +193,56 @@
 }
 __device__ __forceinline__ int lds_s32(unsigned a) { int v; asm volatile("ld.shared.s32 %0, [%1];" : "=r"(v) : "r"(a)); return v; }
 
-#define PM_CLADE_SLOT 384
+__host__ __device__ constexpr int pm_clade_slot(int W) { return 10 * W + 64; }
 #define PM_CLADE_ENTRY_INTS 16
 
-template <typename Real, int NS, int DEPTH>
+template <typename Real, int N>
+__device__ __forceinline__ void mul_elem(const Real* a, const Real* b, Real* d) {
+  if constexpr (std::is_same<Real, float>::value && N % 2 == 0) {
+#pragma unroll
+    for (int j = 0; j < N; j += 2) {
+      const float2 r = __fmul2_rn(make_float2(a[j], a[j + 1]), make_float2(b[j], b[j + 1]));
+      d[j] = r.x; d[j + 1] = r.y;
+    }
+  } else {
+#pragma unroll
+    for (int j = 0; j < N; j++) d[j] = a[j] * b[j];
+  }
+}
+template <typename Real, int N>
+__device__ __forceinline__ void matvec_pairs(const Real* M, const Real* MT, const Real* x, Real* y) {
+  if constexpr (std::is_same<Real, float>::value && N % 2 == 0) {
+    float2 acc[N / 2];
+#pragma unroll
+    for (int c = 0; c < N; c++) {
+      Real col[N];
+      VecIO<Real, N>::load(MT + c * N, N, col);
+      const float2 xc = make_float2(x[c], x[c]);
+#pragma unroll
+      for (int r = 0; r < N / 2; r++)
+        acc[r] = __ffma2_rn(make_float2(col[2 * r], col[2 * r + 1]), xc, c == 0 ? make_float2(0.f, 0.f) : acc[r]);
+    }
+#pragma unroll
+    for (int r = 0; r < N / 2; r++) { y[2 * r] = acc[r].x; y[2 * r + 1] = acc[r].y; }
+  } else {
+#pragma unroll
+    for (int r = 0; r < N; r++) {
+      Real row[N];
+      VecIO<Real, N>::load(M + r * N, N, row);
+      Real acc = 0;
+#pragma unroll
+      for (int c = 0; c < N; c++) acc += row[c] * x[c];
+      y[r] = acc;
+    }
+  }
+}
+
+template <typename Real, int NS, int DEPTH, int W>
 __device__ __forceinline__ void prune_clade_block(const ChainParams<Real>& P, const long long site0, const long long pl0) {
+  constexpr int H = W / 32, SLOT = pm_clade_slot(W);
+  constexpr int TIPA = 256 * H, TIPB = 288 * H, HDR = 320 * H, NXT = HDR + 32;
   extern __shared__ __align__(16) unsigned char smem_raw[];
-  Real* sPow = reinterpret_cast<Real*>(smem_raw + PM_CLADE_SLOT * 8 * DEPTH);
+  Real* sPow = reinterpret_cast<Real*>(smem_raw + SLOT * 8 * DEPTH);
   Real* sPowT = sPow + PM_SMEM_POW * NS * NS;
   const int npow_s = min(PM_SMEM_POW, P.jcap);
   for (int i = threadIdx.x; i < npow_s * NS * NS; i += blockDim.x) {
@@ -208,15 +254,13 @@
   __syncthreads();
   const int lane = threadIdx.x & 31, warp = threadIdx.x >> 5, nw = blockDim.x >> 5;
   const long long S = P.S;
-  const long long site_raw = site0 + lane;
-  const bool active = site_raw < S;
-  const long long site = active ? site_raw : S - 1;
   const bool parity = P.parity_tips != 0;
   const int T = P.T;
-  const uint32_t* __restrict__ meta = P.meta + site;
-  const uint8_t* __restrict__ tip = P.tipcode + site;
-  Real* PLs = P.PL + (pl0 + (site - site0)) * NS;
-  const long long rowPL = P.pl_S * NS;
+  auto site_of = [&](int h, bool& active) {
+    const long long raw = site0 + 32 * h + lane;
+    active = raw < S;
+    return active ? raw : S - 1;
+  };
 
   auto contribution = [&](int k, int code, Real* v) {
     if (code >= 0 && !parity && k < npow_s) {
@@ -227,9 +271,10 @@
     }
   };
   auto product = [&](const Real* va, const Real* vb, Real* out) {
+    mul_elem<Real, NS>(vb, va, out);
     Real sum = 0;
 #pragma unroll
-    for (int j = 0; j < NS; j++) { out[j] = vb[j] * va[j]; sum += out[j]; }
+    for (int j = 0; j < NS; j++) sum += out[j];
     if (sizeof(Real) == 4 && !(sum > (Real)1e-30)) {
       double d[NS], ds = 0;
 #pragma unroll
@@ -240,61 +285,78 @@
       return;
     }
     const Real inv = sum > (Real)0 ? fast_rcp<Real>(sum) : (Real)0;
-#pragma unroll
-    for (int j = 0; j < NS; j++) out[j] *= inv;
+    Real invs[NS];
+#pragma unroll
+    for (int j = 0; j < NS; j++) invs[j] = inv;
+    mul_elem<Real, NS>(out, invs, out);
   };
 
   {
     const int i0 = __ldg(P.cl_warp_off + warp), i1 = __ldg(P.cl_warp_off + warp + 1);
-    unsigned ring = (unsigned)__cvta_generic_to_shared(smem_raw) + warp * (DEPTH * PM_CLADE_SLOT);
+    unsigned ring = (unsigned)__cvta_generic_to_shared(smem_raw) + warp * (DEPTH * SLOT);
     asm volatile("" : "+r"(ring));
-    char* const plb = reinterpret_cast<char*>(PLs);
-    const char* const mtb = reinterpret_cast<const char*>(meta);
-    const char* const tpb = reinterpret_cast<const char*>(P.tipcode) + site0 + 4 * (lane & 7);
-    const bool tip_in = site0 + 4 * (lane & 7) < S;
+    unsigned long long plb_u[H], mtb_u[H];
+    int act[H];
+#pragma unroll
+    for (int h = 0; h < H; h++) {
+      bool a;
+      const long long site = site_of(h, a);
+      plb_u[h] = reinterpret_cast<unsigned long long>(P.PL + (pl0 + (site - site0)) * NS);
+      mtb_u[h] = reinterpret_cast<unsigned long long>(P.meta + site);
+      act[h] = a ? 1 : 0;
+      asm volatile("" : "+l"(plb_u[h]), "+l"(mtb_u[h]), "+r"(act[h]));
+    }
+    const int tq = lane % (8 * H);
+    const char* const tpb = reinterpret_cast<const char*>(P.tipcode) + site0 + 4 * tq;
+    const bool tip_in = site0 + 4 * tq < S;
     const int4* ep = reinterpret_cast<const int4*>(P.cl_entries) + 4 * (long long)i0;
-    unsigned long long plb_u = reinterpret_cast<unsigned long long>(plb), mtb_u = reinterpret_cast<unsigned long long>(mtb),
-                       tpb_u = reinterpret_cast<unsigned long long>(tpb);
-    int act = active ? 1 : 0;
-    asm volatile("" : "+l"(plb_u), "+l"(mtb_u), "+l"(tpb_u), "+r"(act));
+    unsigned long long tpb_u = reinterpret_cast<unsigned long long>(tpb);
+    asm volatile("" : "+l"(tpb_u));
     auto off64 = [](int lo, int hi) { return (long long)(((unsigned long long)(unsigned)hi << 32) | (unsigned)lo); };
-    const bool role_b = (lane >> 3) == 1, role_nxt = lane >= 21, role_ent = lane >= 16;
-    unsigned long long cbase = role_ent ? (unsigned long long)(role_nxt ? (long long)DEPTH * 64 + 16 + 4 * (lane - 21)
-                                                                        : (lane == 20 ? 48 : 4 * (lane - 16)))
-                                        : tpb_u;
-    unsigned dst_off = lane >= 29 ? 340 + 4 * (lane - 29) : role_nxt ? 352 + 4 * (lane - 21) : 256 + 4 * lane;
-    int lrole = ((lane < 29 && (role_ent || tip_in)) ? 1 : 0) | (role_nxt ? 2 : 0) | (role_b ? 4 : 0) | (role_ent ? 8 : 0);
+    const int er = H == 1 ? lane - 16 : lane;
+    const unsigned long long esrc = er < 4 ? (unsigned long long)(4 * er) : er == 4 ? 48 : (unsigned long long)DEPTH * 64 + 16 + 4 * (er - 5);
+    const unsigned edst = er < 5 ? HDR + 4 * er : er < 13 ? NXT + 4 * (er - 5) : HDR + 20 + 4 * (er - 13);
+    const bool role_ent = H == 1 && lane >= 16, role_b = !role_ent && lane >= 8 * H, role_nxt = role_ent && er >= 5;
+    unsigned long long cbase = role_ent ? esrc : tpb_u;
+    unsigned dst_off = role_ent ? edst : TIPA + 4 * lane;
+    int lrole = ((role_ent ? er < 13 : tip_in) ? 1 : 0) | (role_nxt ? 2 : 0) | (role_b ? 4 : 0) | (role_ent ? 8 : 0);
     unsigned lane4 = 4 * lane;
     unsigned fast_pow = ((!parity || NS == 4) && npow_s == PM_SMEM_POW) ? (unsigned)PM_SMEM_POW : 0u;
     int lane_v = lane;
     asm volatile("" : "+l"(cbase), "+r"(dst_off), "+r"(lrole), "+r"(lane4), "+r"(fast_pow), "+r"(lane_v));
     auto issue = [&](unsigned slot, const int4* e, const int4& q1, const int4& q2, bool more) {
-      cp_async4(slot + lane4, reinterpret_cast<const char*>(mtb_u) + off64(q1.x, q1.y));
-      cp_async4(slot + 128 + lane4, reinterpret_cast<const char*>(mtb_u) + off64(q1.z, q1.w));
+#pragma unroll
+      for (int h = 0; h < H; h++) {
+        cp_async4(slot + 128 * h + lane4, reinterpret_cast<const char*>(mtb_u[h]) + off64(q1.x, q1.y));
+        cp_async4(slot + 128 * (H + h) + lane4, reinterpret_cast<const char*>(mtb_u[h]) + off64(q1.z, q1.w));
+      }
       const long long tipoff = (lrole & 4) ? off64(q2.z, q2.w) : off64(q2.x, q2.y);
       const long long X = (lrole & 8) ? reinterpret_cast<long long>(e) : tipoff;
       const bool on = (lrole & 1) && X >= 0 && (more || !(lrole & 2));
       cp_async4(slot + dst_off, reinterpret_cast<const char*>(cbase + (unsigned long long)(X >= 0 ? X : 0LL)), on);
+      if (H > 1) cp_async4_if(er < 5 || (er < 13 && more), slot + edst, reinterpret_cast<const char*>(e) + esrc);
     };
 #pragma unroll 1
     for (int u = 0; u < DEPTH; u++) {
-      if (i0 + u < i1) { issue(ring + u * PM_CLADE_SLOT, ep, __ldg(ep + 1), __ldg(ep + 2), i0 + u + DEPTH < i1); ep += 4; }
+      if (i0 + u < i1) { issue(ring + u * SLOT, ep, __ldg(ep + 1), __ldg(ep + 2), i0 + u + DEPTH < i1); ep += 4; }
       cp_async_commit();
     }
-    Real prev[NS], xA[NS], xB[NS];
-#pragma unroll
-    for (int j = 0; j < NS; j++) { prev[j] = 0; xA[j] = 0; xB[j] = 0; }
+    Real prev[H][NS], xA[H][NS], xB[H][NS];
+#pragma unroll
+    for (int h = 0; h < H; h++)
+#pragma unroll
+      for (int j = 0; j < NS; j++) { prev[h][j] = 0; xA[h][j] = 0; xB[h][j] = 0; }
     long long pnA = 0, pnB = 0;
     int flA = 0, flB = 0;
     if (i0 < i1) {
       cp_async_wait<DEPTH - 1>();
       __syncwarp();
-      const int4 h = lds_v4(ring + 320);
+      const int4 h = lds_v4(ring + HDR);
       pnA = off64(h.x, h.y);
-      flA = lds_s32(ring + 336);
+      flA = lds_s32(ring + HDR + 16);
     }
     unsigned slot = ring;
-    unsigned ring_end = ring + DEPTH * PM_CLADE_SLOT;
+    unsigned ring_end = ring + DEPTH * SLOT;
     asm volatile("" : "+r"(ring_end));
     auto tip_column = [&](int k, int code, Real* v) {
       if (!parity) { VecIO<Real, NS>::load(sPowT + (k * NS + code) * NS, NS, v); return; }
@@ -305,67 +367,62 @@
 #pragma unroll
       for (int j = 0; j < NS; j++) v[j] = c0[j] + c1[j];
     };
-    auto step = [&](int idx, long long pn_off, int fl, const Real* xcur, long long& pn_off_n, int& fl_n, Real* xnext) {
-      const unsigned slot_n = (slot + PM_CLADE_SLOT == ring_end) ? ring : slot + PM_CLADE_SLOT;
+    auto step = [&](int idx, long long pn_off, int fl, Real (*xcur)[NS], long long& pn_off_n, int& fl_n, Real (*xnext)[NS]) {
+      const unsigned slot_n = (slot + SLOT == ring_end) ? ring : slot + SLOT;
       cp_async_wait<DEPTH - 2>();
       __syncwarp();
       if (idx + 1 < i1) {
-        const int4 h = lds_v4(slot_n + 320);
-        fl_n = lds_s32(slot_n + 336);
+        const int4 h = lds_v4(slot_n + HDR);
+        fl_n = lds_s32(slot_n + HDR + 16);
         pn_off_n = off64(h.x, h.y);
-        if (h.w >= 0) VecIO<Real, NS>::load(reinterpret_cast<const Real*>(plb_u + (unsigned long long)off64(h.z, h.w)), NS, xnext);
-      }
-      const int ma = lds_u16(slot + lane4), mb = lds_u16(slot + 128 + lane4);
-      Real va[NS], vb[NS];
-      const bool fast = __all_sync(0xffffffffu, ((unsigned)(ma - 1) | (unsigned)(mb - 1)) < fast_pow);
-      if (fast) {
-        if (fl & 16) tip_column(ma - 1, lds_u8(slot + 256 + lane_v), va);
-        else {
-          const Real* Ma = sPow + (ma - 1) * NS * NS;
-          Real src[NS];
-#pragma unroll
-          for (int j = 0; j < NS; j++) src[j] = (fl & 1) ? prev[j] : xcur[j];
-#pragma unroll
-          for (int r = 0; r < NS; r++) {
-            Real row[NS];
-            VecIO<Real, NS>::load(Ma + r * NS, NS, row);
-            Real acc = 0;
-#pragma unroll
-            for (int c = 0; c < NS; c++) acc += row[c] * src[c];
-            va[r] = acc;
+        if (h.w >= 0) {
+#pragma unroll
+          for (int q = 0; q < H; q++) VecIO<Real, NS>::load(reinterpret_cast<const Real*>(plb_u[q] + (unsigned long long)off64(h.z, h.w)), NS, xnext[q]);
+        }
+      }
+      int ma[H], mb[H];
+      unsigned mm = 0;
+#pragma unroll
+      for (int h = 0; h < H; h++) {
+        ma[h] = lds_u16(slot + 128 * h + lane4);
+        mb[h] = lds_u16(slot + 128 * (H + h) + lane4);
+        mm |= (unsigned)(ma[h] - 1) | (unsigned)(mb[h] - 1);
+      }
+      const bool fast = __all_sync(0xffffffffu, mm < fast_pow);
+#pragma unroll
+      for (int h = 0; h < H; h++) {
+        Real va[NS], vb[NS];
+        if (fast) {
+          if (fl & 16) tip_column(ma[h] - 1, lds_u8(slot + TIPA + 32 * h + lane_v), va);
+          else {
+            Real src[NS];
+#pragma unroll
+            for (int j = 0; j < NS; j++) src[j] = (fl & 1) ? prev[h][j] : xcur[h][j];
+            matvec_pairs<Real, NS>(sPow + (ma[h] - 1) * NS * NS, sPowT + (ma[h] - 1) * NS * NS, src, va);
           }
-        }
-        if (fl & 32) tip_column(mb - 1, lds_u8(slot + 288 + lane_v), vb);
-        else {
-          const Real* Mb = sPow + (mb - 1) * NS * NS;
-          Real src[NS];
-#pragma unroll
-          for (int j = 0; j < NS; j++) src[j] = (fl & 2) ? prev[j] : xcur[j];
-#pragma unroll
-          for (int r = 0; r < NS; r++) {
-            Real row[NS];
-            VecIO<Real, NS>::load(Mb + r * NS, NS, row);
-            Real acc = 0;
-#pragma unroll
-            for (int c = 0; c < NS; c++) acc += row[c] * src[c];
-            vb[r] = acc;
+          if (fl & 32) tip_column(mb[h] - 1, lds_u8(slot + TIPB + 32 * h + lane_v), vb);
+          else {
+            Real src[NS];
+#pragma unroll
+            for (int j = 0; j < NS; j++) src[j] = (fl & 2) ? prev[h][j] : xcur[h][j];
+            matvec_pairs<Real, NS>(sPow + (mb[h] - 1) * NS * NS, sPowT + (mb[h] - 1) * NS * NS, src, vb);
           }
-        }
-      } else {
-        const int ca = (fl & 16) ? lds_u8(slot + 256 + lane_v) : -1, cb = (fl & 32) ? lds_u8(slot + 288 + lane_v) : -1;
-#pragma unroll
-        for (int j = 0; j < NS; j++) {
-          va[j] = (fl & 1) ? prev[j] : xcur[j];
-          vb[j] = (fl & 2) ? prev[j] : xcur[j];
-        }
-        contribution(mb - 1, cb, vb);
-        contribution(ma - 1, ca, va);
-      }
-      product(va, vb, prev);
-      if (act) VecIO<Real, NS>::store(reinterpret_cast<Real*>(plb_u + (unsigned long long)pn_off), NS, prev);
+        } else {
+          const int ca = (fl & 16) ? lds_u8(slot + TIPA + 32 * h + lane_v) : -1, cb = (fl & 32) ? lds_u8(slot + TIPB + 32 * h + lane_v) : -1;
+#pragma unroll
+          for (int j = 0; j < NS; j++) {
+            va[j] = (fl & 1) ? prev[h][j] : xcur[h][j];
+            vb[j] = (fl & 2) ? prev[h][j] : xcur[h][j];
+          }
+          contribution(mb[h] - 1, cb, vb);
+          contribution(ma[h] - 1, ca, va);
+        }
+        product(va, vb, prev[h]);
+        if (act[h]) VecIO<Real, NS>::store(reinterpret_cast<Real*>(plb_u[h] + (unsigned long long)pn_off), NS, prev[h]);
+      }
       __syncwarp();
       if (idx + DEPTH < i1) {
-        const int4 q1 = lds_v4(slot + 352), q2 = lds_v4(slot + 368);
+        const int4 q1 = lds_v4(slot + NXT), q2 = lds_v4(slot + NXT + 16);
         __syncwarp();
         issue(slot, ep, q1, q2, idx + 2 * DEPTH < i1);
         ep += 4;
@@ -383,6 +440,11 @@
   __syncthreads();
 
   const int4* __restrict__ ent = reinterpret_cast<const int4*>(P.cl_top_entries);
+  const long long rowPL = P.pl_S * NS;
+  bool active = false;
+  const uint32_t* meta = nullptr;
+  const uint8_t* tip = nullptr;
+  Real* PLs = nullptr;
   auto load = [&](PruneNode<Real, NS>& nd, int id) {
     const int4 e0 = __ldg(ent + 2 * id), e1 = __ldg(ent + 2 * id + 1);
     nd.pn = e0.x;
@@ -404,24 +466,31 @@
   PruneNode<Real, NS> A, B;
   for (int l = 0; l < P.n_cl_top_levels; l++) {
     const int beg = __ldg(P.cl_top_off + l), end = __ldg(P.cl_top_off + l + 1);
-    int idx = beg + warp;
-    if (idx < end) load(A, idx);
-    while (idx < end) {
-      if (idx + nw < end) load(B, idx + nw);
-      compute(A);
-      idx += nw;
-      if (idx >= end) break;
-      if (idx + nw < end) load(A, idx + nw);
-      compute(B);
-      idx += nw;
+#pragma unroll 1
+    for (int h = 0; h < H; h++) {
+      const long long site = site_of(h, active);
+      meta = P.meta + site;
+      tip = P.tipcode + site;
+      PLs = P.PL + (pl0 + (site - site0)) * NS;
+      int idx = beg + warp;
+      if (idx < end) load(A, idx);
+      while (idx < end) {
+        if (idx + nw < end) load(B, idx + nw);
+        compute(A);
+        idx += nw;
+        if (idx >= end) break;
+        if (idx + nw < end) load(A, idx + nw);
+        compute(B);
+        idx += nw;
+      }
     }
     __syncthreads();
   }
 }
 
-template <typename Real, int NS, int DEPTH, int MINB>
+template <typename Real, int NS, int DEPTH, int MINB, int W>
 __global__ void __launch_bounds__(256, MINB) k_prune_clade(ChainParams<Real> P) {
-  prune_clade_block<Real, NS, DEPTH>(P, P.tile_base + (long long)blockIdx.x * 32, (long long)blockIdx.x * 32);
+  prune_clade_block<Real, NS, DEPTH, W>(P, P.tile_base + (long long)blockIdx.x * W, (long long)blockIdx.x * W);
 }
 
 template <typename Real, int NS, bool EXACT>
@@ -674,8 +743,7 @@
     for (int j = 0; j < NS; j++) w[j] = (Real)(j == ps);
     for (int r = 0; r < k; r++) matvec_t<Real, NS, false>(sBs, NS, w);
   }
-#pragma unroll
-  for (int j = 0; j < NS; j++) w[j] *= pl[j];
+  mul_elem<Real, NS>(w, pl, w);
   Real c[NS];
   c[0] = w[0];
 #pragma unroll
@@ -724,11 +792,15 @@
   return draw_node_state<Real, NS>(P, sBs, sPow, npow_s, k, ps, pl, word);
 }
 
-template <typename Real, int NS, int DEPTH>
+template <typename Real, int NS, int W>
+__host__ __device__ constexpr int pm_nodes_slot() { return W * NS * (int)sizeof(Real) + 4 * W + 32; }
+
+template <typename Real, int NS, int DEPTH, int W>
 __device__ __forceinline__ void nodes_clade_block(const ChainParams<Real>& P, const uint32_t iter, const long long site0, const long long pl0) {
+  constexpr int H = W / 32;
   constexpr int PB = NS * (int)sizeof(Real);
-  constexpr int PLB = 32 * PB;
-  constexpr int SLOT = PLB + 160;
+  constexpr int PLB = W * PB;
+  constexpr int SLOT = pm_nodes_slot<Real, NS, W>(), HDR = PLB + 128 * H;
   extern __shared__ __align__(16) unsigned char smem_raw[];
   Real* sBs = reinterpret_cast<Real*>(smem_raw + SLOT * 8 * DEPTH);
   Real* sVec = sBs + NS * NS;
@@ -738,26 +810,34 @@
   __syncthreads();
   const int lane = threadIdx.x & 31, warp = threadIdx.x >> 5, nw = blockDim.x >> 5;
   const long long S = P.S;
-  const long long site_raw = site0 + lane;
-  const bool active = site_raw < S;
-  const long long site = active ? site_raw : S - 1;
-  const long long lsite = pl0 + (site - site0);
   const bool parity = P.parity_tips != 0;
   const int T = P.T;
-  const uint32_t gsite = P.rng.site0 + (uint32_t)site;
   const uint32_t kslot = make_slot(K_NODEGRP, 0u);
-  uint8_t* const nst = P.node_state + site;
+  struct Half { long long site, lsite; bool active; uint32_t gsite; };
+  auto half = [&](int h) {
+    Half q;
+    const long long raw = site0 + 32 * h + lane;
+    q.active = raw < S;
+    q.site = q.active ? raw : S - 1;
+    q.lsite = pl0 + (q.site - site0);
+    q.gsite = P.rng.site0 + (uint32_t)q.site;
+    return q;
+  };
   if (warp == 0) {
-    Real w[NS], pl[NS];
-    VecIO<Real, NS>::load(P.PL + ((long long)(P.root - T) * P.pl_S + lsite) * NS, NS, pl);
-#pragma unroll
-    for (int j = 0; j < NS; j++) w[j] = sVec[j] * pl[j];
-    uint32_t o[4];
-    philox4x32_10_rk(0xffffffffu, kslot, iter, gsite, P.rng.rk, o);
-    const int s = categorical<Real, NS, false>(w, NS, u01_from_word<Real>(o[0]), P.err_flag);
-    if (active) {
-      nst[(long long)P.root * S] = (uint8_t)s;
-      if (gsite == 0u) *P.root_out = s;
+#pragma unroll 1
+    for (int h = 0; h < H; h++) {
+      const Half q = half(h);
+      Real w[NS], pl[NS];
+      VecIO<Real, NS>::load(P.PL + ((long long)(P.root - T) * P.pl_S + q.lsite) * NS, NS, pl);
+#pragma unroll
+      for (int j = 0; j < NS; j++) w[j] = sVec[j] * pl[j];
+      uint32_t o[4];
+      philox4x32_10_rk(0xffffffffu, kslot, iter, q.gsite, P.rng.rk, o);
+      const int s = categorical<Real, NS, false>(w, NS, u01_from_word<Real>(o[0]), P.err_flag);
+      if (q.active) {
+        P.node_state[(long long)P.root * S + q.site] = (uint8_t)s;
+        if (q.gsite == 0u) *P.root_out = s;
+      }
     }
   }
   __syncthreads();
@@ -765,14 +845,19 @@
     const int beg = __ldg(P.cd_top_off + l), end = __ldg(P.cd_top_off + l + 1);
     for (int idx = beg + warp; idx < end; idx += nw) {
       const int4 en = __ldg(reinterpret_cast<const int4*>(P.cd_top) + idx);
-      const int ps = nst[(long long)en.y * S];
-      const int k = (int)(P.meta[(long long)en.z * S + site] & 0xffffu) - 1;
-      Real pl[NS];
-      VecIO<Real, NS>::load(P.PL + ((long long)(en.x - T) * P.pl_S + lsite) * NS, NS, pl);
-      uint32_t o[4];
-      philox4x32_10_rk(0x80000000u + (uint32_t)idx, kslot, iter, gsite, P.rng.rk, o);
-      const int s = draw_node_state<Real, NS>(P, sBs, sPow, npow_s, k, ps, pl, o[0]);
-      if (active) nst[(long long)en.x * S] = (uint8_t)s;
+#pragma unroll 1
+      for (int h = 0; h < H; h++) {
+        const Half q = half(h);
+        uint8_t* const nst = P.node_state + q.site;
+        const int ps = nst[(long long)en.y * S];
+        const int k = (int)(P.meta[(long long)en.z * S + q.site] & 0xffffu) - 1;
+        Real pl[NS];
+        VecIO<Real, NS>::load(P.PL + ((long long)(en.x - T) * P.pl_S + q.lsite) * NS, NS, pl);
+        uint32_t o[4];
+        philox4x32_10_rk(0x80000000u + (uint32_t)idx, kslot, iter, q.gsite, P.rng.rk, o);
+        const int s = draw_node_state<Real, NS>(P, sBs, sPow, npow_s, k, ps, pl, o[0]);
+        if (q.active) nst[(long long)en.x * S] = (uint8_t)s;
+      }
     }
     __syncthreads();
   }
@@ -780,24 +865,37 @@
     const int i0 = __ldg(P.cd_warp_off + warp), i1 = __ldg(P.cd_warp_off + warp + 1);
     unsigned ring = (unsigned)__cvta_generic_to_shared(smem_raw) + warp * (DEPTH * SLOT);
     asm volatile("" : "+r"(ring));
-    unsigned long long plb_u = reinterpret_cast<unsigned long long>(P.PL + lsite * NS),
-                       mtb_u = reinterpret_cast<unsigned long long>(P.meta + site),
-                       nsb_u = reinterpret_cast<unsigned long long>(nst);
-    int act = active ? 1 : 0;
+    unsigned long long plb_u[H], mtb_u[H], nsb_u[H];
+    int act[H];
+    uint32_t gsite[H];
+#pragma unroll
+    for (int h = 0; h < H; h++) {
+      const Half q = half(h);
+      plb_u[h] = reinterpret_cast<unsigned long long>(P.PL + q.lsite * NS);
+      mtb_u[h] = reinterpret_cast<unsigned long long>(P.meta + q.site);
+      nsb_u[h] = reinterpret_cast<unsigned long long>(P.node_state + q.site);
+      act[h] = q.active ? 1 : 0;
+      gsite[h] = q.gsite;
+      asm volatile("" : "+l"(plb_u[h]), "+l"(mtb_u[h]), "+l"(nsb_u[h]), "+r"(act[h]));
+    }
     unsigned lane4 = 4 * lane, lanePB = PB * lane;
     unsigned long long hsrc = lane < 4 ? 16 + 4 * lane : (unsigned long long)DEPTH * 64 + 4 * (lane - 4);
-    unsigned hdst = PLB + 128 + 4 * lane;
-    asm volatile("" : "+l"(plb_u), "+l"(mtb_u), "+l"(nsb_u), "+r"(act), "+r"(lane4), "+r"(lanePB), "+l"(hsrc), "+r"(hdst));
+    unsigned hdst = HDR + 4 * lane;
+    asm volatile("" : "+r"(lane4), "+r"(lanePB), "+l"(hsrc), "+r"(hdst));
     auto off64 = [](int lo, int hi) { return (long long)(((unsigned long long)(unsigned)hi << 32) | (unsigned)lo); };
     const int4* ep = reinterpret_cast<const int4*>(P.cd_entries) + 4 * (long long)i0;
     auto issue = [&](unsigned slot, const int4* e, const int4& q0, bool more) {
-      const char* src = reinterpret_cast<const char*>(plb_u) + off64(q0.x, q0.y);
-      if (PB == 8) asm volatile("cp.async.ca.shared.global [%0], [%1], 8;" ::"r"(slot + lanePB), "l"(src) : "memory");
-      else {
-        cp_async16(slot + lanePB, src);
-        if (PB == 32) cp_async16(slot + lanePB + 16, src + 16);
-      }
-      cp_async4(slot + PLB + lane4, reinterpret_cast<const char*>(mtb_u) + off64(q0.z, q0.w));
+#pragma unroll
+      for (int h = 0; h < H; h++) {
+        const char* src = reinterpret_cast<const char*>(plb_u[h]) + off64(q0.x, q0.y);
+        const unsigned dst = slot + 32 * PB * h + lanePB;
+        if (PB == 8) asm volatile("cp.async.ca.shared.global [%0], [%1], 8;" ::"r"(dst), "l"(src) : "memory");
+        else {
+          cp_async16(dst, src);
+          if (PB == 32) cp_async16(dst + 16, src + 16);
+        }
+        cp_async4(slot + PLB + 128 * h + lane4, reinterpret_cast<const char*>(mtb_u[h]) + off64(q0.z, q0.w));
+      }
       if (lane < 8) cp_async4(slot + hdst, reinterpret_cast<const char*>(e) + hsrc, lane < 4 || more);
     };
 #pragma unroll 1
@@ -806,40 +904,54 @@
       cp_async_commit();
     }
     long long vA = 0, vB = 0, pA = -1, pB = -1;
-    int psA = 0, psB = 0;
+    int psA[H], psB[H], sprev[H];
+    uint32_t o[H][4];
+#pragma unroll
+    for (int h = 0; h < H; h++) {
+      psA[h] = 0; psB[h] = 0; sprev[h] = 0;
+      o[h][0] = o[h][1] = o[h][2] = o[h][3] = 0;
+    }
     if (i0 < i1) {
       cp_async_wait<DEPTH - 1>();
       __syncwarp();
-      const int4 h = lds_v4(ring + PLB + 128);
-      vA = off64(h.x, h.y); pA = off64(h.z, h.w);
-      if (pA >= 0) psA = *reinterpret_cast<const uint8_t*>(nsb_u + (unsigned long long)pA);
+      const int4 hd = lds_v4(ring + HDR);
+      vA = off64(hd.x, hd.y); pA = off64(hd.z, hd.w);
+      if (pA >= 0) {
+#pragma unroll
+        for (int h = 0; h < H; h++) psA[h] = *reinterpret_cast<const uint8_t*>(nsb_u[h] + (unsigned long long)pA);
+      }
     }
     unsigned slot = ring;
     unsigned ring_end = ring + DEPTH * SLOT;
     asm volatile("" : "+r"(ring_end));
-    int sprev = 0;
-    uint32_t o[4] = {0, 0, 0, 0};
-    auto step = [&](int idx, long long v_off, long long p_off, int ps_mem, long long& v_off_n, long long& p_off_n, int& ps_mem_n) {
+    auto step = [&](int idx, long long v_off, long long p_off, const int* ps_mem, long long& v_off_n, long long& p_off_n, int* ps_mem_n) {
       const unsigned slot_n = (slot + SLOT == ring_end) ? ring : slot + SLOT;
       cp_async_wait<DEPTH - 2>();
       __syncwarp();
       if (idx + 1 < i1) {
-        const int4 h = lds_v4(slot_n + PLB + 128);
-        v_off_n = off64(h.x, h.y); p_off_n = off64(h.z, h.w);
-        if (h.w >= 0) ps_mem_n = *reinterpret_cast<const uint8_t*>(nsb_u + (unsigned long long)p_off_n);
-      }
-      if ((idx & 3) == 0 || idx == i0) philox4x32_10_rk((uint32_t)idx >> 2, kslot, iter, gsite, P.rng.rk, o);
-      const uint32_t word = (idx & 3) == 0 ? o[0] : (idx & 3) == 1 ? o[1] : (idx & 3) == 2 ? o[2] : o[3];
-      Real pl[NS];
-      lds_vec<Real, NS>(slot + lanePB, pl);
-      const int k = lds_u16(slot + PLB + lane4) - 1;
-      const int ps = p_off < 0 ? sprev : ps_mem;
-      const int sn = draw_node_state<Real, NS>(P, sBs, sPow, npow_s, k, ps, pl, word);
-      if (act) *reinterpret_cast<uint8_t*>(nsb_u + (unsigned long long)v_off) = (uint8_t)sn;
-      sprev = sn;
+        const int4 hd = lds_v4(slot_n + HDR);
+        v_off_n = off64(hd.x, hd.y); p_off_n = off64(hd.z, hd.w);
+        if (hd.w >= 0) {
+#pragma unroll
+          for (int h = 0; h < H; h++) ps_mem_n[h] = *reinterpret_cast<const uint8_t*>(nsb_u[h] + (unsigned long long)p_off_n);
+        }
+      }
+      const bool fresh = (idx & 3) == 0 || idx == i0;
+#pragma unroll
+      for (int h = 0; h < H; h++) {
+        if (fresh) philox4x32_10_rk((uint32_t)idx >> 2, kslot, iter, gsite[h], P.rng.rk, o[h]);
+        const uint32_t word = (idx & 3) == 0 ? o[h][0] : (idx & 3) == 1 ? o[h][1] : (idx & 3) == 2 ? o[h][2] : o[h][3];
+        Real pl[NS];
+        lds_vec<Real, NS>(slot + 32 * PB * h + lanePB, pl);
+        const int k = lds_u16(slot + PLB + 128 * h + lane4) - 1;
+        const int ps = p_off < 0 ? sprev[h] : ps_mem[h];
+        const int sn = draw_node_state<Real, NS>(P, sBs, sPow, npow_s, k, ps, pl, word);
+        if (act[h]) *reinterpret_cast<uint8_t*>(nsb_u[h] + (unsigned long long)v_off) = (uint8_t)sn;
+        sprev[h] = sn;
+      }
       __syncwarp();
       if (idx + DEPTH < i1) {
-        const int4 q0 = lds_v4(slot + PLB + 144);
+        const int4 q0 = lds_v4(slot + HDR + 16);
         __syncwarp();
         issue(slot, ep, q0, idx + 2 * DEPTH < i1);
         ep += 4;
@@ -856,57 +968,64 @@
   }
   if (P.n_cd_tips > 0) {
     __syncthreads();
-    const int ntip = P.n_cd_tips, ngrp = (ntip + 3) >> 2;
-    const uint8_t* const tipb = P.tipcode + site;
-    const char* const mtb = reinterpret_cast<const char*>(P.meta + site);
-    struct TipLoad { int ps, k, cd; };
-    auto load = [&](int grp, TipLoad (&L)[4]) {
-#pragma unroll
-      for (int q = 0; q < 4; q++) {
-        const int v = min(4 * grp + q, ntip - 1);
-        const longlong2 en = __ldg(reinterpret_cast<const longlong2*>(P.cd_tips) + v);
-        L[q].ps = nst[en.x];
-        L[q].k = (int)(*reinterpret_cast<const uint32_t*>(mtb + en.y) & 0xffffu) - 1;
-        L[q].cd = tipb[(long long)v * P.TS];
-      }
-    };
-    auto draw = [&](int grp, const TipLoad (&L)[4]) {
-      uint32_t o[4];
-      philox4x32_10_rk(0x40000000u + (uint32_t)grp, kslot, iter, gsite, P.rng.rk, o);
-#pragma unroll
-      for (int q = 0; q < 4; q++) {
-        if (4 * grp + q < ntip) {
-          const uint32_t word = q == 0 ? o[0] : q == 1 ? o[1] : q == 2 ? o[2] : o[3];
-          const int sn = draw_tip_state<Real, NS>(P, sBs, sPow, npow_s, L[q].k, L[q].ps, L[q].cd, parity, word);
-          if (active) nst[(long long)(4 * grp + q) * S] = (uint8_t)sn;
-        }
-      }
-    };
-    TipLoad A[4], B[4];
-    int grp = warp;
-    if (grp < ngrp) load(grp, A);
-    while (grp < ngrp) {
-      if (grp + nw < ngrp) load(grp + nw, B);
-      draw(grp, A);
-      grp += nw;
-      if (grp >= ngrp) break;
-      if (grp + nw < ngrp) load(grp + nw, A);
-      draw(grp, B);
-      grp += nw;
-    }
-  }
-}
-
-template <typename Real, int NS, int DEPTH, int MINB>
+#pragma unroll 1
+    for (int h = 0; h < H; h++) {
+      const Half hs = half(h);
+      const long long site = hs.site;
+      const bool active = hs.active;
+      uint8_t* const nst = P.node_state + site;
+      const int ntip = P.n_cd_tips, ngrp = (ntip + 3) >> 2;
+      const uint8_t* const tipb = P.tipcode + site;
+      const char* const mtb = reinterpret_cast<const char*>(P.meta + site);
+      struct TipLoad { int ps, k, cd; };
+      auto load = [&](int grp, TipLoad (&L)[4]) {
+#pragma unroll
+        for (int q = 0; q < 4; q++) {
+          const int v = min(4 * grp + q, ntip - 1);
+          const longlong2 en = __ldg(reinterpret_cast<const longlong2*>(P.cd_tips) + v);
+          L[q].ps = nst[en.x];
+          L[q].k = (int)(*reinterpret_cast<const uint32_t*>(mtb + en.y) & 0xffffu) - 1;
+          L[q].cd = tipb[(long long)v * P.TS];
+        }
+      };
+      auto draw = [&](int grp, const TipLoad (&L)[4]) {
+        uint32_t o[4];
+        philox4x32_10_rk(0x40000000u + (uint32_t)grp, kslot, iter, hs.gsite, P.rng.rk, o);
+#pragma unroll
+        for (int q = 0; q < 4; q++) {
+          if (4 * grp + q < ntip) {
+            const uint32_t word = q == 0 ? o[0] : q == 1 ? o[1] : q == 2 ? o[2] : o[3];
+            const int sn = draw_tip_state<Real, NS>(P, sBs, sPow, npow_s, L[q].k, L[q].ps, L[q].cd, parity, word);
+            if (active) nst[(long long)(4 * grp + q) * S] = (uint8_t)sn;
+          }
+        }
+      };
+      TipLoad A[4], B[4];
+      int grp = warp;
+      if (grp < ngrp) load(grp, A);
+      while (grp < ngrp) {
+        if (grp + nw < ngrp) load(grp + nw, B);
+        draw(grp, A);
+        grp += nw;
+        if (grp >= ngrp) break;
+        if (grp + nw < ngrp) load(grp + nw, A);
+        draw(grp, B);
+        grp += nw;
+      }
+    }
+  }
+}
+
+template <typename Real, int NS, int DEPTH, int MINB, int W>
 __global__ void __launch_bounds__(256, MINB) k_nodes_clade(ChainParams<Real> P, uint32_t iter) {
   if (P.ctl) iter = P.ctl[0];
-  nodes_clade_block<Real, NS, DEPTH>(P, iter, P.tile_base + (long long)blockIdx.x * 32, (long long)blockIdx.x * 32);
+  nodes_clade_block<Real, NS, DEPTH, W>(P, iter, P.tile_base + (long long)blockIdx.x * W, (long long)blockIdx.x * W);
 }
 
 __device__ __forceinline__ unsigned long long global_ns() { unsigned long long t; asm volatile("mov.u64 %0, %%globaltimer;" : "=l"(t)); return t; }
 __device__ __forceinline__ unsigned sm_id() { unsigned v; asm volatile("mov.u32 %0, %%smid;" : "=r"(v)); return v; }
 
-template <typename Real, int NS, int DEPTH, int MINB>
+template <typename Real, int NS, int DEPTH, int MINB, int W>
 __global__ void __launch_bounds__(256, MINB) k_prune_nodes_clade(ChainParams<Real> P, uint32_t iter, long long b0, int phases, int* slot_busy,
                                                                  int slots_per_sm, unsigned long long* phase_ns) {
   if (P.ctl) iter = P.ctl[0];
@@ -925,12 +1044,12 @@
   }
   __syncthreads();
   const int slot = s_slot;
-  const long long site0 = (b0 + blockIdx.x) * 32, pl0 = (long long)slot * 32;
-  prune_clade_block<Real, NS, DEPTH>(P, site0, pl0);
+  const long long site0 = (b0 + blockIdx.x) * W, pl0 = (long long)slot * W;
+  prune_clade_block<Real, NS, DEPTH, W>(P, site0, pl0);
   __syncthreads();
   if (phases & 2) {
     if (phase_ns && threadIdx.x == 0) s_t[1] = global_ns();
-    nodes_clade_block<Real, NS, DEPTH>(P, iter, site0, pl0);
+    nodes_clade_block<Real, NS, DEPTH, W>(P, iter, site0, pl0);
     __syncthreads();
     if (phase_ns && threadIdx.x == 0) {
       const unsigned long long t2 = global_ns();
diff --git a/phylomap_b200/csrc/pm_launch.cuh b/phylomap_b200/csrc/pm_launch.cuh
--- a/phylomap_b200/csrc/pm_launch.cuh
+++ b/phylomap_b200/csrc/pm_launch.cuh
@@ -5,7 +5,17 @@
 namespace pm {
 
 template <typename Real, int NS, bool EXACT>
+struct FusedCfg {
+  static constexpr int W = sizeof(Real) == 8 ? 32 : 64, D = 8, MB = 2;
+  static constexpr bool clade = !EXACT && (NS == 2 || NS == 4);
+  static size_t smem_prune() { return 2 * PM_SMEM_POW * NS * NS * sizeof(Real) + (size_t)pm_clade_slot(W) * 8 * D; }
+  static size_t smem_nodes(size_t smem_model) { return smem_model + (size_t)pm_nodes_slot<Real, NS, W>() * 8 * D; }
+  static size_t smem(size_t smem_model) { return smem_prune() > smem_nodes(smem_model) ? smem_prune() : smem_nodes(smem_model); }
+};
+
+template <typename Real, int NS, bool EXACT>
 struct Sweep {
+  static constexpr int block_sites = FusedCfg<Real, NS, EXACT>::clade ? FusedCfg<Real, NS, EXACT>::W : 32;
   static void prune(const ChainParams<Real>& P, int grid, size_t smem, cudaStream_t st);
   static void nodes(const ChainParams<Real>& P, int grid, size_t smem, cudaStream_t st, uint32_t iter);
   static int fused_blocks_per_sm(size_t smem_nodes);
diff --git a/phylomap_b200/csrc/pm_launch_impl.cuh b/phylomap_b200/csrc/pm_launch_impl.cuh
--- a/phylomap_b200/csrc/pm_launch_impl.cuh
+++ b/phylomap_b200/csrc/pm_launch_impl.cuh
@@ -5,11 +5,10 @@
 
 template <typename Real, int NS, bool EXACT>
 void Sweep<Real, NS, EXACT>::prune(const ChainParams<Real>& P, int grid, size_t smem, cudaStream_t st) {
-  if constexpr (!EXACT && (NS == 2 || NS == 4)) {
-    constexpr int D = 8, MB = sizeof(Real) == 8 ? 2 : 3;
-    const size_t spow = 2 * PM_SMEM_POW * NS * NS * sizeof(Real);
-    const size_t sm = spow + (size_t)PM_CLADE_SLOT * 8 * D;
-    auto kern = k_prune_clade<Real, NS, D, MB>;
+  if constexpr (FusedCfg<Real, NS, EXACT>::clade) {
+    typedef FusedCfg<Real, NS, EXACT> C;
+    const size_t sm = C::smem_prune();
+    auto kern = k_prune_clade<Real, NS, C::D, C::MB, C::W>;
     cudaFuncSetAttribute(kern, cudaFuncAttributeMaxDynamicSharedMemorySize, (int)sm);
     kern<<<grid, 256, sm, st>>>(P);
   }
@@ -17,29 +16,20 @@
 }
 template <typename Real, int NS, bool EXACT>
 void Sweep<Real, NS, EXACT>::nodes(const ChainParams<Real>& P, int grid, size_t smem, cudaStream_t st, uint32_t iter) {
-  if constexpr (!EXACT && (NS == 2 || NS == 4)) {
-    constexpr int D = 8, MB = sizeof(Real) == 8 ? 2 : 3;
-    const size_t sm = smem + (size_t)(32 * NS * sizeof(Real) + 160) * 8 * D;
-    auto kern = k_nodes_clade<Real, NS, D, MB>;
+  if constexpr (FusedCfg<Real, NS, EXACT>::clade) {
+    typedef FusedCfg<Real, NS, EXACT> C;
+    const size_t sm = C::smem_nodes(smem);
+    auto kern = k_nodes_clade<Real, NS, C::D, C::MB, C::W>;
     cudaFuncSetAttribute(kern, cudaFuncAttributeMaxDynamicSharedMemorySize, (int)sm);
     kern<<<grid, 256, sm, st>>>(P, iter);
   }
   else k_nodes<Real, NS, EXACT><<<grid, 256, smem, st>>>(P, iter);
 }
 template <typename Real, int NS, bool EXACT>
-struct FusedCfg {
-  static constexpr int D = 8, MB = sizeof(Real) == 8 ? 2 : 3;
-  static size_t smem(size_t smem_nodes) {
-    const size_t sm_prune = 2 * PM_SMEM_POW * (NS > 0 ? NS : 1) * (NS > 0 ? NS : 1) * sizeof(Real) + (size_t)PM_CLADE_SLOT * 8 * D;
-    const size_t sm_nodes = smem_nodes + (size_t)(32 * (NS > 0 ? NS : 1) * sizeof(Real) + 160) * 8 * D;
-    return sm_prune > sm_nodes ? sm_prune : sm_nodes;
-  }
-};
-template <typename Real, int NS, bool EXACT>
 int Sweep<Real, NS, EXACT>::fused_blocks_per_sm(size_t smem_nodes) {
-  if constexpr (!EXACT && (NS == 2 || NS == 4)) {
+  if constexpr (FusedCfg<Real, NS, EXACT>::clade) {
     typedef FusedCfg<Real, NS, EXACT> C;
-    auto kern = k_prune_nodes_clade<Real, NS, C::D, C::MB>;
+    auto kern = k_prune_nodes_clade<Real, NS, C::D, C::MB, C::W>;
     const size_t sm = C::smem(smem_nodes);
     cudaFuncSetAttribute(kern, cudaFuncAttributeMaxDynamicSharedMemorySize, (int)sm);
     int nb = 0;
@@ -51,9 +41,9 @@
 template <typename Real, int NS, bool EXACT>
 void Sweep<Real, NS, EXACT>::prune_nodes(const ChainParams<Real>& P, int grid, size_t smem_nodes, cudaStream_t st, uint32_t iter,
                                          long long b0, int phases, int* slot_busy, int slots_per_sm, unsigned long long* phase_ns) {
-  if constexpr (!EXACT && (NS == 2 || NS == 4)) {
+  if constexpr (FusedCfg<Real, NS, EXACT>::clade) {
     typedef FusedCfg<Real, NS, EXACT> C;
-    auto kern = k_prune_nodes_clade<Real, NS, C::D, C::MB>;
+    auto kern = k_prune_nodes_clade<Real, NS, C::D, C::MB, C::W>;
     const size_t sm = C::smem(smem_nodes);
     cudaFuncSetAttribute(kern, cudaFuncAttributeMaxDynamicSharedMemorySize, (int)sm);
     kern<<<grid, 256, sm, st>>>(P, iter, b0, phases, slot_busy, slots_per_sm, phase_ns);
```

Result: no change. 71.13 billion (median of 6 runs) (-0.9%).
